# plainerman/DiffDock-Pocket

Hardware: AMD Instinct MI355X
Metric: ligand poses/sec (40 samples x 20 steps) on 3dpf (higher is better)
Workload: dtype f32 (fc and G products: fp16 hi/lo split of both operands on v_mfma_f32_16x16x32_f16 - the row-stationary conv kernel - and v_mfma_f32_32x32x16_f16, fp32 accumulate; G between its two kernels as fp16 hi + continuation byte = 19 significant bits; the exact fp32 MFMA form is timed in other_workloads)

## Files before the change

diffdock_pocket_amd/_lib.py:

```python
from __future__ import annotations

import ctypes as C
import os

HERE = os.path.dirname(os.path.abspath(__file__))
LIB_PATH = os.environ.get("DDP_HIP_LIB", os.path.join(HERE, "libddp_hip.so"))

DDP_MAX_TASKS, DDP_MAX_BLOCKS, DDP_MAX_SEGS, DDP_MAX_NS, DDP_EDGE_TILE = 9, 4, 3, 64, 64
F_SCALAR_S0, F_DOT, F_SCALAR_S1, F_VEC_S0, F_CROSS = range(5)
FS = 68

DDP_MAX_GEMM_BATCH = 16
DDP_EVAL_MAX_ATOMS = 1024
DDP_MINIMIZE_MAX_ATOMS, DDP_MINIMIZE_MAX_TORSIONS = 512, 4096
DDP_MINIMIZE_FLEX_MAX_MOVING, DDP_MINIMIZE_FLEX_MAX_BONDS, DDP_MINIMIZE_FLEX_MAX_STATE_BYTES = 256, 256, 47040
DDP_PAIRWISE_MAX_SAMPLES, DDP_CLUSTER_MAX_SAMPLES = 32768, 1024
EXPORTS = ["ddp_conv_messages", "ddp_conv_rows", "ddp_stage_a_gh", "ddp_stage_a_gh3", "ddp_segment_reduce", "ddp_edge_featurize", "ddp_edge_featurize_jobs", "ddp_torsion_sh", "ddp_stage_a", "ddp_stage_a_h2",
           "ddp_pose_update", "ddp_sidechain_update", "ddp_sde_update", "ddp_radius_count", "ddp_radius_fill", "ddp_knn", "ddp_group_by_key", "ddp_node_linear", "ddp_scan_jobs", "ddp_mark_jobs", "ddp_rowcopy_jobs", "ddp_select_jobs",
           "ddp_gather_rows", "ddp_clean_pair_maps", "ddp_flex_mark", "ddp_fallback_rowmap", "ddp_step_prologue", "ddp_trrot_head", "ddp_tor_head", "ddp_radius_search_jobs", "ddp_group_by_key_jobs", "ddp_set_occupancy_shaping", "ddp_pose_rmsd", "ddp_pose_contacts", "ddp_pose_pairwise_rmsd", "ddp_pose_cluster", "ddp_traj_record", "ddp_svgd_tau", "ddp_svgd_pairs", "ddp_svgd_rows", "ddp_refine_energy", "ddp_refine_direction", "ddp_refine_accept", "ddp_pose_score", "ddp_pose_minimize", "ddp_pose_minimize_flex", "ddp_pocket_occupancy", "ddp_pocket_buriedness", "ddp_pocket_label", "ddp_abi_version", "ddp_last_error", "ddp_source_hash"]


class Seg(C.Structure):
    _fields_ = [("kind", C.c_int32), ("in_off", C.c_int32), ("count", C.c_int32)]


class Block(C.Structure):
    _fields_ = [("U", C.c_int32), ("n", C.c_int32), ("C", C.c_int32), ("out_off", C.c_int32), ("tile0", C.c_int32),
                ("ntiles", C.c_int32), ("nsub", C.c_int32), ("ups", C.c_int32), ("nseg", C.c_int32),
                ("seg", Seg * DDP_MAX_SEGS), ("g_slot", C.c_int32), ("g_col0", C.c_int32)]


class RoleSeg(C.Structure):
    _fields_ = [("block", C.c_int32), ("tile0", C.c_int32), ("tstride", C.c_int32), ("count", C.c_int32), ("round", C.c_int32)]


DDP_CONV32_WAVES, DDP_MAX_ROLE_SEGS = 4, 2


class ConvShape(C.Structure):
    _fields_ = [("f_in", C.c_int32), ("hid", C.c_int32), ("kp1", C.c_int32), ("hp", C.c_int32), ("hs", C.c_int32),
                ("nct1", C.c_int32), ("d_out", C.c_int32), ("nblocks", C.c_int32), ("fbuf_floats", C.c_int32),
                ("g_cols", C.c_int32 * 2), ("blk", Block * DDP_MAX_BLOCKS), ("nrounds", C.c_int32),
                ("nrole", C.c_int32 * DDP_CONV32_WAVES), ("role", (RoleSeg * DDP_MAX_ROLE_SEGS) * DDP_CONV32_WAVES)]


class ConvTask(C.Structure):
    _fields_ = [("x_src", C.c_void_p), ("ldx_src", C.c_int32), ("n_edges", C.c_int32), ("src", C.c_void_p),
                ("eid", C.c_void_p), ("sh", C.c_void_p), ("seg_ptr", C.c_void_p * DDP_MAX_SEGS),
                ("seg_idx", C.c_void_p * DDP_MAX_SEGS), ("seg_ld", C.c_int32 * DDP_MAX_SEGS),
                ("seg_n", C.c_int32 * DDP_MAX_SEGS), ("w1p", C.c_void_p), ("b1p", C.c_void_p), ("w2p", C.c_void_p),
                ("b2p", C.c_void_p), ("msg", C.c_void_p), ("g", C.c_void_p * 2),
                ("pos", C.c_void_p), ("n_edges_dev", C.c_void_p), ("w1h", C.c_void_p), ("w2h", C.c_void_p), ("h2_range_flag", C.c_void_p),
                ("wsh", C.c_void_p), ("bsp", C.c_void_p), ("gh", C.c_void_p * 2), ("gh_fmt", C.c_int32), ("rows_form", C.c_int32), ("rows_bias_k", C.c_int32), ("rows_seg0", C.c_int32), ("rows_seg1", C.c_int32), ("rows_nts", C.c_int32)]


class ReduceSrc(C.Structure):
    _fields_ = [("msg", C.c_void_p), ("rowptr", C.c_void_p), ("bn_scale", C.c_void_p), ("bn_shift", C.c_void_p),
                ("n_edges", C.c_int32), ("rowmap", C.c_void_p), ("n_edges_dev", C.c_void_p)]


DDP_MAX_NODE_JOBS, DDP_MAX_NODE_CAT = 8, 16
DDP_MAX_LIST_JOBS = 12
_P, _I = C.c_void_p, C.c_int32


class ScanJob(C.Structure):
    _fields_ = [("n", _I), ("n_dev", _P), ("flag", _P), ("val", _P), ("rowptr", _P), ("base", _I), ("excl", _P), ("excl2", _P),
                ("list", _P), ("total", _P)]


class MarkJob(C.Structure):
    _fields_ = [("idx", _P), ("n", _I), ("n_dev", _P), ("mask", _P)]


class RowcopyJob(C.Structure):
    _fields_ = [("n_rows", _I), ("keep", _P), ("old_rowptr", _P), ("new_rowptr", _P), ("inp", _P * 3), ("out", _P * 3)]


class SelectJob(C.Structure):
    _fields_ = [("n", _I), ("n_dev", _P), ("mask_a", _P), ("idx_a", _P), ("mask_b", _P), ("idx_b", _P), ("out_idx", _P),
                ("pay", _P * 4), ("pay_add", _I * 4), ("out", _P * 4), ("total", _P), ("block_count", _P), ("block_off", _P)]


class RadiusJob(C.Structure):
    _fields_ = [("x", _P), ("x_ptr", _P), ("y", _P), ("y_batch", _P), ("ny", _I), ("r", C.c_float), ("max_neighbors", _I),
                ("flags", _I), ("graph_div", _P), ("counts", _P), ("offsets", _P), ("base", _I), ("total", _P), ("out_query", _P),
                ("out_x", _P), ("capacity", _I), ("overflow", _P)]


class SdeArgs(C.Structure):
    _fields_ = [("score", _P * 4), ("z", _P * 4), ("out", _P * 4), ("n", _I * 4)]


class SvgdArgs(C.Structure):
    _fields_ = [("pos", _P), ("n", _I), ("n_lig", _I), ("n_tor", _I), ("dihedrals", _P), ("score", _P * 3), ("upd", _P * 3), ("gdt", _P),
                ("weight", C.c_float), ("w_rep", C.c_float), ("w_rot", C.c_float), ("w_tor", C.c_float), ("svgd_only", _I),
                ("tau", _P), ("tr_diff", _P), ("rot_diff", _P), ("tor_diff", _P), ("dist", _P)]


class RefineArgs(C.Structure):
    _fields_ = [("n_samples", _I), ("n", _I), ("m", _I), ("rec_stride", _I), ("n_tor", _I), ("pos", _P), ("anchor", _P), ("lig_radii", _P),
                ("rec", _P), ("rec_radii", _P), ("self_pairs", _P), ("overlap", C.c_double), ("restraint", C.c_double), ("energy", _P),
                ("grad", _P), ("bonds", _P), ("mask_rotate", _P), ("step", _P), ("tr", _P), ("rot", _P), ("tor", _P), ("trial", _P),
                ("trial_energy", _P), ("trial_grad", _P), ("accepted", _P), ("grow", C.c_double), ("shrink", C.c_double),
                ("step_max", C.c_double)]


class ScoreArgs(C.Structure):
    _fields_ = [("n_samples", _I), ("n", _I), ("m", _I), ("rec_stride", _I), ("pos", _P), ("lig_radii", _P), ("lig_flags", _P), ("rec", _P),
                ("rec_radii", _P), ("rec_flags", _P), ("self_pairs", _P), ("cutoff", C.c_double), ("gauss_offset", C.c_double),
                ("gauss_width", C.c_double), ("hydrophobic_good", C.c_double), ("hydrophobic_bad", C.c_double), ("hbond_good", C.c_double),
                ("hbond_bad", C.c_double), ("w_gauss", C.c_double), ("w_repulsion", C.c_double), ("w_hydrophobic", C.c_double),
                ("w_hbond", C.c_double), ("tor_divisor", C.c_double), ("energy", _P), ("grad", _P)]


class MinimizeArgs(C.Structure):
    _fields_ = [("n_samples", _I), ("n", _I), ("m", _I), ("rec_stride", _I), ("n_tor", _I), ("iterations", _I), ("pos", _P), ("anchor", _P),
                ("lig_radii", _P), ("lig_flags", _P), ("rec", _P), ("rec_radii", _P), ("rec_flags", _P), ("self_pairs", _P), ("bonds", _P),
                ("mask_rotate", _P), ("cutoff", C.c_double), ("gauss_offset", C.c_double), ("gauss_width", C.c_double),
                ("hydrophobic_good", C.c_double), ("hydrophobic_bad", C.c_double), ("hbond_good", C.c_double), ("hbond_bad", C.c_double),
                ("w_gauss", C.c_double), ("w_repulsion", C.c_double), ("w_hydrophobic", C.c_double), ("w_hbond", C.c_double),
                ("restraint", C.c_double), ("grow", C.c_double), ("shrink", C.c_double), ("step_max", C.c_double), ("step", _P),
                ("accepted", _P), ("energy_in", _P), ("energy_out", _P), ("history", _P), ("grad", _P)]


class MinimizeFlexArgs(C.Structure):
    _fields_ = MinimizeArgs._fields_ + [("rec_anchor", _P), ("n_mov", _I), ("n_sc", _I), ("n_sub", _I), ("reserved", _I), ("mov", _P),
                                        ("sc_edge_idx", _P), ("sc_sub", _P), ("sc_map", _P), ("sc_pairs", _P),
                                        ("restraint_sc", C.c_double), ("grad_mov", _P)]


def flex_state_bytes(n: int, n_mov: int, n_sc: int) -> int:
    return 89 * n + 81 * n_mov + 4 * n_sc


class GroupJob(C.Structure):
    _fields_ = [("key", _P), ("n_items", _I), ("n_items_dev", _P), ("n_keys", _I), ("pay", _P * 3), ("rowptr", _P), ("perm", _P),
                ("out_key", _P), ("out", _P * 3), ("key_map", _P), ("scratch", _P)]



DDP_MAX_FEATURIZE_JOBS = 8


class FeaturizeJob(C.Structure):
    _fields_ = [("pos_a", _P), ("ia", _P), ("pos_b", _P), ("ib", _P), ("n_edges", _I), ("n_edges_dev", _P), ("offset", _P), ("k_rbf", _I),
                ("coeff", C.c_float), ("pre", _P), ("pre_idx", _P), ("ld_pre", _I), ("pre2", _P), ("n_pre2", _I), ("ld_pre2", _I),
                ("w1d", _P), ("w2", _P), ("b2", _P), ("ns", _I), ("out", _P), ("sh", _P)]


class _BondJob(C.Structure):
    _fields_ = [("pos", _P), ("b0", _P), ("b1", _P), ("n", _I), ("mid", _P), ("vec", _P)]


class _CopyJob(C.Structure):
    _fields_ = [("src", _P), ("dst", _P), ("n", _I)]


class PrologueArgs(C.Structure):
    _fields_ = [("t", _P * 4), ("t_stride", _I * 4), ("sig_min", C.c_float * 4), ("sig_max", C.c_float * 4), ("sigma", _P * 4),
                ("n_graphs", _I), ("cut", _P), ("cut_mul", C.c_float), ("cut_add", C.c_float), ("graph_emb", _P), ("sd", _I),
                ("emb_scale", C.c_float), ("freq", _P), ("lig_pos", _P), ("graph_ptr", _P), ("center", _P),
                ("bonds", _BondJob * 2), ("copy", _CopyJob * 2)]


class TrRotArgs(C.Structure):
    _fields_ = [("gp", _P), ("ld_gp", _I), ("n_graphs", _I), ("ns", _I), ("sd", _I), ("graph_emb", _P), ("w1", _P * 2), ("b1", _P * 2),
                ("w2", _P * 2), ("b2", _P * 2), ("sigma", _P * 2), ("so3_table", _P), ("so3_n", _I), ("so3_lo", C.c_float),
                ("so3_span", C.c_float), ("out", _P * 2)]


class TorArgs(C.Structure):
    _fields_ = [("h", _P), ("ld_h", _I), ("n_bonds", _I), ("ns", _I), ("w1", _P), ("w2", _P), ("sigma", _P), ("graph_of_bond", _P),
                ("torus_table", _P), ("torus_n", _I), ("torus_lo", C.c_float), ("torus_span", C.c_float), ("out", _P)]


class NodeJob(C.Structure):
    _fields_ = [("n_rows", C.c_int32), ("cat", C.c_void_p), ("ld_cat", C.c_int32), ("n_cat", C.c_int32), ("table", C.c_void_p),
                ("feat_off", C.c_int32 * DDP_MAX_NODE_CAT), ("emb_dim", C.c_int32), ("emb_mode", C.c_int32),
                ("dense", C.c_void_p * 2), ("ld_dense", C.c_int32 * 2), ("n_dense", C.c_int32 * 2),
                ("t", C.c_void_p), ("t_stride", C.c_int32), ("scale", C.c_float), ("freq", C.c_void_p),
                ("sig_emb", C.c_void_p), ("ld_sig", C.c_int32), ("sd", C.c_int32), ("sig_out", C.c_void_p), ("ld_sig_out", C.c_int32),
                ("w", C.c_void_p), ("bias", C.c_void_p),
                ("out", C.c_void_p), ("ld_out", C.c_int32), ("ncols", C.c_int32), ("zero_to", C.c_int32),
                ("add", C.c_void_p), ("ld_add", C.c_int32)]


def g_ld(hid: int, gcols: int) -> int:
    return (((hid + 3) // 4 * 4 + 1) * gcols + 31) // 32 * 32


class DdpError(RuntimeError):
    pass


_lib = None


def load():
    global _lib
    if _lib is not None:
        return _lib
    if not os.path.exists(LIB_PATH):
        raise DdpError(f"{LIB_PATH} not found: build it with `python -m diffdock_pocket_amd.build` "
                       f"(hipcc --offload-arch=gfx950); there is no fallback path")
    lib = C.CDLL(LIB_PATH)
    for name in EXPORTS:
        if not hasattr(lib, name):
            raise DdpError(f"{LIB_PATH} does not export {name}")
    lib.ddp_abi_version.restype = C.c_int
    lib.ddp_last_error.restype = C.c_char_p
    lib.ddp_conv_messages.argtypes = [C.POINTER(ConvShape), C.POINTER(ConvTask), C.c_int, C.c_void_p]
    lib.ddp_conv_messages.restype = C.c_int
    lib.ddp_conv_rows.argtypes = lib.ddp_conv_messages.argtypes
    lib.ddp_conv_rows.restype = C.c_int
    lib.ddp_segment_reduce.argtypes = [C.c_void_p, C.c_int, C.c_int, C.c_int, C.POINTER(ReduceSrc), C.c_int, C.c_int,
                                       C.c_int, C.c_int, C.c_void_p]
    lib.ddp_segment_reduce.restype = C.c_int
    lib.ddp_edge_featurize.argtypes = [C.c_void_p, C.c_void_p, C.c_void_p, C.c_void_p, C.c_int, C.c_void_p, C.c_void_p, C.c_int,
                                       C.c_float, C.c_void_p, C.c_void_p, C.c_int, C.c_void_p, C.c_int, C.c_int, C.c_void_p,
                                       C.c_void_p, C.c_void_p, C.c_int, C.c_void_p, C.c_void_p, C.c_void_p]
    lib.ddp_edge_featurize.restype = C.c_int
    lib.ddp_edge_featurize_jobs.argtypes = [C.POINTER(FeaturizeJob), C.c_int, C.c_void_p]
    lib.ddp_edge_featurize_jobs.restype = C.c_int
    lib.ddp_torsion_sh.argtypes = [C.c_void_p, C.c_void_p, C.c_void_p, C.c_int, C.c_void_p, C.c_void_p, C.c_void_p, C.c_int, C.c_int,
                                   C.c_void_p, C.c_void_p, C.c_int, C.c_void_p, C.c_void_p]
    lib.ddp_torsion_sh.restype = C.c_int
    lib.ddp_stage_a.argtypes = [C.c_void_p, C.c_int, C.c_int, C.c_void_p, C.c_void_p, C.c_int, C.POINTER(C.c_int32), C.c_int,
                                C.c_void_p, C.c_void_p, C.c_int, C.c_int, C.c_void_p, C.c_int, C.c_void_p]
    lib.ddp_stage_a.restype = C.c_int
    lib.ddp_stage_a_h2.argtypes = lib.ddp_stage_a.argtypes[:-1] + [C.c_void_p, C.c_void_p]
    lib.ddp_stage_a_h2.restype = C.c_int
    lib.ddp_stage_a_gh.argtypes = lib.ddp_stage_a_h2.argtypes[:-1] + [C.c_void_p, C.c_void_p]
    lib.ddp_stage_a_gh.restype = C.c_int
    lib.ddp_stage_a_gh3.argtypes = lib.ddp_stage_a_gh.argtypes
    lib.ddp_stage_a_gh3.restype = C.c_int
    lib.ddp_set_occupancy_shaping.argtypes = [C.c_int, C.c_int]
    lib.ddp_set_occupancy_shaping.restype = C.c_int
    lib.ddp_pose_update.argtypes = [C.c_void_p, C.c_int, C.c_int, C.c_void_p, C.c_void_p, C.c_void_p, C.c_int, C.c_void_p,
                                    C.c_void_p, C.c_void_p, C.c_void_p]
    lib.ddp_pose_update.restype = C.c_int
    lib.ddp_sidechain_update.argtypes = [C.c_void_p, C.c_int, C.c_int, C.c_void_p, C.c_int, C.c_void_p, C.c_void_p, C.c_void_p,
                                         C.c_void_p, C.c_void_p]
    lib.ddp_sidechain_update.restype = C.c_int
    lib.ddp_radius_count.argtypes = [C.c_void_p, C.c_void_p, C.c_void_p, C.c_void_p, C.c_int, C.c_float, C.c_int, C.c_int,
                                     C.c_void_p, C.c_void_p]
    lib.ddp_radius_count.restype = C.c_int
    lib.ddp_radius_fill.argtypes = [C.c_void_p, C.c_void_p, C.c_void_p, C.c_void_p, C.c_int, C.c_float, C.c_int, C.c_int,
                                    C.c_void_p, C.c_void_p, C.c_void_p, C.c_void_p]
    lib.ddp_radius_fill.restype = C.c_int
    lib.ddp_knn.argtypes = [C.c_void_p, C.c_void_p, C.c_void_p, C.c_int, C.c_int, C.c_void_p, C.c_void_p]
    lib.ddp_knn.restype = C.c_int
    lib.ddp_group_by_key.argtypes = [C.c_void_p, C.c_int, C.c_int] + [C.c_void_p] * 11
    lib.ddp_group_by_key.restype = C.c_int
    for name, job in (("ddp_scan_jobs", ScanJob), ("ddp_mark_jobs", MarkJob), ("ddp_rowcopy_jobs", RowcopyJob),
                      ("ddp_select_jobs", SelectJob), ("ddp_radius_search_jobs", RadiusJob), ("ddp_group_by_key_jobs", GroupJob)):
        getattr(lib, name).argtypes = [C.POINTER(job), C.c_int, C.c_void_p]
        getattr(lib, name).restype = C.c_int
    lib.ddp_sde_update.argtypes = [C.c_void_p, C.POINTER(SdeArgs), C.c_void_p]
    lib.ddp_sde_update.restype = C.c_int
    lib.ddp_gather_rows.argtypes = [C.c_void_p, C.c_int, C.c_void_p, C.c_int, C.c_void_p, C.c_void_p, C.c_int, C.c_int, C.c_void_p]
    lib.ddp_gather_rows.restype = C.c_int
    lib.ddp_clean_pair_maps.argtypes = [C.c_void_p, C.c_void_p, C.c_void_p, C.c_void_p, C.c_int, C.c_int, C.c_int, C.c_int, C.c_void_p,
                                        C.c_void_p, C.c_void_p]
    lib.ddp_clean_pair_maps.restype = C.c_int
    lib.ddp_flex_mark.argtypes = [C.c_void_p, C.c_void_p, C.c_int, C.c_void_p, C.c_void_p, C.c_int, C.c_int, C.c_int, C.c_int, C.c_int,
                                  C.c_void_p, C.c_void_p]
    lib.ddp_flex_mark.restype = C.c_int
    lib.ddp_fallback_rowmap.argtypes = [C.c_void_p, C.c_void_p, C.c_void_p, C.c_void_p, C.c_int, C.c_int, C.c_void_p, C.c_void_p]
    lib.ddp_fallback_rowmap.restype = C.c_int
    for name, st in (("ddp_step_prologue", PrologueArgs), ("ddp_trrot_head", TrRotArgs), ("ddp_tor_head", TorArgs)):
        getattr(lib, name).argtypes = [C.POINTER(st), C.c_void_p]
        getattr(lib, name).restype = C.c_int
    lib.ddp_node_linear.argtypes = [C.POINTER(NodeJob), C.c_int, C.c_void_p]
    lib.ddp_node_linear.restype = C.c_int
    lib.ddp_pose_rmsd.argtypes = [C.c_void_p, C.c_int, C.c_int, C.c_void_p, C.c_int, C.c_void_p, C.c_int, C.c_void_p, C.c_int,
                                  C.c_void_p, C.c_void_p, C.c_void_p]
    lib.ddp_pose_rmsd.restype = C.c_int
    lib.ddp_pose_contacts.argtypes = [C.c_void_p, C.c_int, C.c_int, C.c_void_p, C.c_void_p, C.c_int, C.c_int, C.c_void_p, C.c_float,
                                      C.c_void_p, C.c_void_p, C.c_void_p]
    lib.ddp_pose_contacts.restype = C.c_int
    lib.ddp_pose_pairwise_rmsd.argtypes = [C.c_void_p, C.c_int, C.c_int, C.c_void_p, C.c_int, C.c_void_p, C.c_int, C.c_void_p, C.c_void_p]
    lib.ddp_pose_pairwise_rmsd.restype = C.c_int
    lib.ddp_pose_cluster.argtypes = [C.c_void_p, C.c_int, C.c_void_p, C.c_float, C.c_void_p, C.c_void_p, C.c_void_p, C.c_void_p, C.c_void_p]
    lib.ddp_pose_cluster.restype = C.c_int
    lib.ddp_traj_record.argtypes = [C.c_void_p, C.c_int, C.c_int, C.c_void_p, C.c_void_p, C.c_int, C.c_void_p, C.c_int, C.c_void_p,
                                    C.c_int, C.c_void_p, C.c_void_p]
    lib.ddp_traj_record.restype = C.c_int
    for name in ("ddp_svgd_tau", "ddp_svgd_pairs", "ddp_svgd_rows"):
        getattr(lib, name).argtypes = [C.POINTER(SvgdArgs), C.c_void_p]
        getattr(lib, name).restype = C.c_int
    for name in ("ddp_refine_energy", "ddp_refine_direction", "ddp_refine_accept"):
        getattr(lib, name).argtypes = [C.POINTER(RefineArgs), C.c_void_p]
        getattr(lib, name).restype = C.c_int
    lib.ddp_pose_score.argtypes = [C.POINTER(ScoreArgs), C.c_void_p]
    lib.ddp_pose_score.restype = C.c_int
    lib.ddp_pose_minimize.argtypes = [C.POINTER(MinimizeArgs), C.c_void_p]
    lib.ddp_pose_minimize.restype = C.c_int
    lib.ddp_pose_minimize_flex.argtypes = [C.POINTER(MinimizeFlexArgs), C.c_void_p]
    lib.ddp_pose_minimize_flex.restype = C.c_int
    lib.ddp_pocket_occupancy.argtypes = [C.c_void_p, C.c_void_p, C.c_int, C.c_float, C.c_float, C.c_float, C.c_float, C.c_int, C.c_int, C.c_int,
                                         C.c_void_p, C.c_void_p]
    lib.ddp_pocket_occupancy.restype = C.c_int
    lib.ddp_pocket_buriedness.argtypes = [C.c_void_p, C.c_int, C.c_int, C.c_int, C.c_double, C.c_double, C.c_int, C.c_void_p, C.c_void_p,
                                          C.c_void_p]
    lib.ddp_pocket_buriedness.restype = C.c_int
    lib.ddp_pocket_label.argtypes = [C.c_void_p, C.c_int, C.c_int, C.c_int, C.c_void_p, C.c_void_p]
    lib.ddp_pocket_label.restype = C.c_int
    if lib.ddp_abi_version() != 17:
        raise DdpError("libddp_hip.so ABI version mismatch")
    lib.ddp_source_hash.restype = C.c_char_p
    if "DDP_HIP_LIB" not in os.environ:
        from .build import source_hash
        have, want = lib.ddp_source_hash().decode(), source_hash()
        if have != want:
            raise DdpError(f"{LIB_PATH} was built from other sources (library {have}, tree {want}): rebuild it with "
                           f"`python -m diffdock_pocket_amd.build`")
    _lib = lib
    return lib


def check(rc, what):
    if rc != 0:
        raise DdpError(f"{what} failed (rc={rc}): {load().ddp_last_error().decode()}")
```

diffdock_pocket_amd/csrc/ddp_gemm.hip:

```cpp
#include <hip/hip_runtime.h>
#include <stdint.h>
#include <type_traits>
#include <stdlib.h>

#include "ddp_hip.h"
#include "ddp_internal.h"

typedef float f32x2 __attribute__((ext_vector_type(2)));
typedef float f32x4 __attribute__((ext_vector_type(4)));

#define DDP_GEMM_THREADS 256
#define DDP_GEMM_ROWS 128

struct GemmOffs {
  int off[DDP_MAX_GEMM_BATCH];
};

template <int KT, int CPL>
__global__ __launch_bounds__(DDP_GEMM_THREADS, 2) void ddp_stage_a_kernel(const float* __restrict__ x, int ldx, int nrows,
                                                                           const int32_t* __restrict__ rows,
                                                                           const int32_t* __restrict__ nrows_dev, int out_rows,
                                                                           const GemmOffs offs, const float* __restrict__ w,
                                                                           int k, int ncols, float* __restrict__ out, int ldo) {
  constexpr int KP = (KT > 0) ? KT / 2 : 32;
// ... 225 lines not shown

template <int KT>
__global__ __launch_bounds__(DDP_GEMM_THREADS, 2) void ddp_stage_a_x3_kernel(const float* __restrict__ x, int ldx, int nrows,
                                                                              const int32_t* __restrict__ rows,
                                                                              const int32_t* __restrict__ nrows_dev, int out_rows,
                                                                              int mrows, const GemmOffs offs,
                                                                              const __bf16* __restrict__ w3, int ncols,
                                                                              float* __restrict__ out, int ldo) {
  if (nrows_dev) nrows = min(nrows, *nrows_dev);
  if ((int)blockIdx.y * mrows >= nrows) return;
  constexpr int KP = (KT + 15) / 16 * 16, NS = KP / 16, CT = DDP_SA3_CT;
  constexpr int XS = KP + 8;
  constexpr int NV = (32 * KT / 4 + DDP_GEMM_THREADS - 1) / DDP_GEMM_THREADS;
  constexpr int TS = 36;
  constexpr int NM = NS * 6;
  __shared__ __attribute__((aligned(16))) __bf16 xt[2][3][32 * XS];
  __shared__ __attribute__((aligned(16))) float st[4][2][32 * TS];
  const int z = (int)blockIdx.z, tid = (int)threadIdx.x;
  const int wave = tid >> 6, lane = tid & 63, r = lane & 31, hh = lane >> 5;
  const int col0 = ((int)blockIdx.x * 4 + wave) * (32 * CT);
  bf16x8 wr[CT][3][NS];
#pragma unroll
  for (int t = 0; t < CT; ++t) {
    const int c = min(col0 + 32 * t + r, ncols - 1);
#pragma unroll
    for (int p = 0; p < 3; ++p)
#pragma unroll
      for (int s2 = 0; s2 < NS; ++s2)
        wr[t][p][s2] = *reinterpret_cast<const bf16x8*>(w3 + (((((size_t)z * 3 + p) * NS + s2) * 2 + hh) * ncols + c) * 8);
  }
  if constexpr (KP > KT) {
    for (int i = tid; i < 2 * 3 * 32 * (KP - KT); i += DDP_GEMM_THREADS) {
      const int kk = i % (KP - KT), rr = (i / (KP - KT)) % 32, bp = i / ((KP - KT) * 32);
      xt[bp / 3][bp % 3][rr * XS + KT + kk] = (__bf16)0.f;
    }
  }
  const float* __restrict__ xb = x + offs.off[z];
  for (int R0 = (int)blockIdx.y * mrows; R0 < nrows; R0 += (int)gridDim.y * mrows) {
  const int R1 = min(nrows, R0 + mrows);
  const bool al4 = ((ldx | offs.off[z]) & 3) == 0 && (reinterpret_cast<size_t>(x) & 15) == 0;
  f32x4 xv[NV];
  auto fetch = [&](int row0) {
#pragma unroll
    for (int v = 0; v < NV; ++v) {
      const int i = tid + v * DDP_GEMM_THREADS;
      const int rr = min(i / (KT / 4), 31), q = i % (KT / 4);
      const int ri = min(row0 + rr, nrows - 1);
      const float* __restrict__ p = xb + (size_t)(rows ? rows[ri] : ri) * ldx + 4 * q;
      if (al4)
        xv[v] = *reinterpret_cast<const f32x4*>(p);
      else
        xv[v] = f32x4{p[0], p[1], p[2], p[3]};
    }
  };
  auto park = [&](int buf) {
#pragma unroll
    for (int v = 0; v < NV; ++v) {
      const int i = tid + v * DDP_GEMM_THREADS;
      if (i < 32 * (KT / 4)) {
        const int rr = i / (KT / 4), q = i % (KT / 4);
        bf16x4 h, m, l;
#pragma unroll
        for (int e = 0; e < 4; ++e) {
          const float f = xv[v][e];
          h[e] = (__bf16)f;
          const float r1 = f - (float)h[e];
          m[e] = (__bf16)r1;
          l[e] = (__bf16)(r1 - (float)m[e]);
        }
        *reinterpret_cast<bf16x4*>(&xt[buf][0][rr * XS + 4 * q]) = h;
        *reinterpret_cast<bf16x4*>(&xt[buf][1][rr * XS + 4 * q]) = m;
        *reinterpret_cast<bf16x4*>(&xt[buf][2][rr * XS + 4 * q]) = l;
      }
    }
  };
  float* pend_ob = nullptr;
  int pend_c0 = 0, pend_rows = 0, pend_buf = 0, pbuf = 0;
  int pend_ri[4] = {0, 0, 0, 0};
  f32x4 dv = {0.f, 0.f, 0.f, 0.f};
  auto drain_read = [&](int p) {
    if (pend_ob) dv = *reinterpret_cast<const f32x4*>(&st[wave][pend_buf][(8 * p + (lane >> 3)) * TS + 4 * (lane & 7)]);
  };
  auto drain_store = [&](int p) {
    if (pend_ob) {
      const int rr = 8 * p + (lane >> 3), c = pend_c0 + 4 * (lane & 7);
      if (rr < pend_rows && c < ncols) *reinterpret_cast<f32x4*>(&pend_ob[(size_t)pend_ri[p] * ldo + c]) = dv;
    }
  };
  fetch(R0);
  park(0);
  __syncthreads();
  int buf = 0;
  for (int row0 = R0; row0 < R1; row0 += 32, buf ^= 1) {
    const bool more = row0 + 32 < R1;
    if (more) fetch(row0 + 32);
    bf16x8 a[3][NS];
#pragma unroll
    for (int p = 0; p < 3; ++p)
#pragma unroll
      for (int s2 = 0; s2 < NS; ++s2) a[p][s2] = *reinterpret_cast<const bf16x8*>(&xt[buf][p][r * XS + 16 * s2 + 8 * hh]);
    float* __restrict__ ob = out + (size_t)z * out_rows * ldo;
    int blk_ri[4];
#pragma unroll
    for (int p = 0; p < 4; ++p) {
      const int ri = min(row0 + 8 * p + (lane >> 3), R1 - 1);
      blk_ri[p] = rows ? rows[ri] : ri;
    }
#pragma unroll
    for (int t = 0; t < CT; ++t) {
      f32x16 acc;
#pragma unroll
      for (int i = 0; i < 16; ++i) acc[i] = 0.f;
#pragma unroll
      for (int m = 0; m < NM; ++m) {
        constexpr int PA[6] = {2, 0, 1, 1, 0, 0}, PB[6] = {0, 2, 1, 0, 1, 0};
        const int pr = m / NS, s2 = m % NS;
        acc = __builtin_amdgcn_mfma_f32_32x32x16_bf16(a[PA[pr]][s2], wr[t][PB[pr]][s2], acc, 0, 0, 0);
        static_assert(NM / 4 >= 3 && NM % 4 == 0, "quarter schedule");
        if (m % (NM / 4) == 0) drain_read(m / (NM / 4));
        if (m % (NM / 4) == 2) drain_store(m / (NM / 4));
      }
      float* tl = st[wave][pbuf];
#pragma unroll
      for (int i = 0; i < 16; ++i) tl[((i & 3) + 8 * (i >> 2) + 4 * hh) * TS + r] = acc[i];
      pend_ob = ob;
#pragma unroll
      for (int p = 0; p < 4; ++p) pend_ri[p] = blk_ri[p];
      pend_c0 = col0 + 32 * t;
      pend_rows = R1 - row0;
      pend_buf = pbuf;
      pbuf ^= 1;
    }
    if (more) park(buf ^ 1);
    __syncthreads();
  }
#pragma unroll
  for (int p = 0; p < 4; ++p) {
    drain_read(p);
    drain_store(p);
  }
  __syncthreads();
  }
}

typedef _Float16 h8 __attribute__((ext_vector_type(8)));
typedef _Float16 h4 __attribute__((ext_vector_type(4)));
#ifndef DDP_SAH_CT_GH
#define DDP_SAH_CT_GH 4
#endif
#ifndef DDP_SAH_CT
#define DDP_SAH_CT 4
#endif

template <int KT, bool GH = false, bool G3 = false>
__global__ __launch_bounds__(DDP_GEMM_THREADS, 2) void ddp_stage_a_h2_kernel(const float* __restrict__ x, int ldx, int nrows,
                                                                              const int32_t* __restrict__ rows,
                                                                              const int32_t* __restrict__ nrows_dev, int out_rows,
                                                                              int mrows, const GemmOffs offs,
                                                                              const _Float16* __restrict__ wh, int ncols,
                                                                              float* __restrict__ out, int ldo, int32_t* range_flag,
                                                                              const int32_t* __restrict__ gh_dest = nullptr) {
  if (nrows_dev) nrows = min(nrows, *nrows_dev);
  if ((int)blockIdx.y * mrows >= nrows) return;
  constexpr int KP = (KT + 15) / 16 * 16, NS = KP / 16, CT = GH ? DDP_SAH_CT_GH : DDP_SAH_CT;
  constexpr int XS = KP + 8;
  constexpr int NV = (32 * KT / 4 + DDP_GEMM_THREADS - 1) / DDP_GEMM_THREADS;
  constexpr int TS = 36;
  constexpr int RS3 = 392;
  __shared__ __attribute__((aligned(16))) _Float16 xt[2][2][32 * XS];
  __shared__ __attribute__((aligned(16))) float st[G3 ? 1 : 4][2][G3 ? 4 : 32 * TS];
  __shared__ __attribute__((aligned(16))) char g3t[G3 ? 4 : 1][G3 ? 32 * RS3 : 16];
  const int z = (int)blockIdx.z, tid = (int)threadIdx.x;
  const int wave = tid >> 6, lane = tid & 63, r = lane & 31, hh = lane >> 5;
  const int col0 = ((int)blockIdx.x * 4 + wave) * (32 * CT);
  h8 wr[CT][2][NS];
#pragma unroll
  for (int t = 0; t < CT; ++t) {
    const int c = min(col0 + 32 * t + r, ncols - 1);
#pragma unroll
    for (int p = 0; p < 2; ++p)
#pragma unroll
      for (int s2 = 0; s2 < NS; ++s2)
        wr[t][p][s2] = *reinterpret_cast<const h8*>(wh + (((((size_t)z * 2 + p) * NS + s2) * 2 + hh) * ncols + c) * 8);
  }
  if constexpr (KP > KT) {
    for (int i = tid; i < 2 * 2 * 32 * (KP - KT); i += DDP_GEMM_THREADS) {
      const int kk = i % (KP - KT), rr = (i / (KP - KT)) % 32, bp = i / ((KP - KT) * 32);
      xt[bp / 2][bp % 2][rr * XS + KT + kk] = (_Float16)0.f;
    }
  }
  const float* __restrict__ xb = x + offs.off[z];
  float* __restrict__ ob = out + (size_t)z * out_rows * ldo;
  int cq[CT];
#pragma unroll
  for (int t = 0; t < CT; ++t) cq[t] = max(0, min(4 * (lane & 7), ncols - 4 - (col0 + 32 * t)));
  int gh_o[CT][2];
  bool gh_sp[CT];
  float gh_max = 0.f;
#pragma unroll
  for (int t = 0; t < CT; ++t) {
    gh_o[t][0] = gh_o[t][1] = 0;
    gh_sp[t] = false;
    if constexpr (GH) {
      const int g = min(col0 + 32 * t + 8 * (lane & 3), ncols - 8) >> 3;
      const int32_t* __restrict__ d = gh_dest + ((size_t)z * (ncols >> 3) + g) * 2;
      gh_o[t][0] = d[0] & ~3;
      gh_o[t][1] = d[1];
      gh_sp[t] = (d[0] & 1) != 0;
    }
  }
  unsigned sp3 = 0u;
  int g3_rr[3] = {0, 0, 0}, g3_pc[3] = {0, 0, 0};
  if constexpr (G3) {
    const int g = min(col0 + 8 * (lane & 15), ncols - 8) >> 3;
    sp3 = (unsigned)__ballot((gh_dest[((size_t)z * (ncols >> 3) + g) * 2] & 1) != 0) & 0xffffu;
#pragma unroll
    for (int j = 0; j < 3; ++j) {
      g3_rr[j] = (64 * j + lane) / 24;
      g3_pc[j] = (64 * j + lane) % 24;
    }
  }
  for (int R0 = (int)blockIdx.y * mrows; R0 < nrows; R0 += (int)gridDim.y * mrows) {
  const int R1 = min(nrows, R0 + mrows);
  const bool al4 = ((ldx | offs.off[z]) & 3) == 0 && (reinterpret_cast<size_t>(x) & 15) == 0;
  f32x4 xv[NV];
  auto fetch = [&](int row0) {
#pragma unroll
    for (int v = 0; v < NV; ++v) {
      const int i = tid + v * DDP_GEMM_THREADS;
      const int rr = min(i / (KT / 4), 31), q = i % (KT / 4);
      const int ri = min(row0 + rr, nrows - 1);
      const float* __restrict__ p = xb + (size_t)(rows ? rows[ri] : ri) * ldx + 4 * q;
      if (al4)
        xv[v] = *reinterpret_cast<const f32x4*>(p);
      else
        xv[v] = f32x4{p[0], p[1], p[2], p[3]};
    }
  };
  auto park = [&](int buf) {
#pragma unroll
    for (int v = 0; v < NV; ++v) {
      const int i = tid + v * DDP_GEMM_THREADS;
      if (i < 32 * (KT / 4)) {
        const int rr = i / (KT / 4), q = i % (KT / 4);
        h4 h, l;
#pragma unroll
        for (int e = 0; e < 4; ++e) {
          const float f = GH ? xv[v][e] * (float)DDP_GH_SX : xv[v][e];
          if (!(fabsf(f) <= 65504.f) && range_flag) *range_flag = 1;
          h[e] = (_Float16)f;
          l[e] = (_Float16)(GH ? f - (float)h[e] : (f - (float)h[e]) * 2048.f);
        }
        *reinterpret_cast<h4*>(&xt[buf][0][rr * XS + 4 * q]) = h;
        *reinterpret_cast<h4*>(&xt[buf][1][rr * XS + 4 * q]) = l;
      }
    }
  };
  size_t pend_off[4] = {0, 0, 0, 0};
  int pend_lds[4] = {0, 0, 0, 0};
  bool pend_sp = false;
  int pbuf = 0;
  f32x4 dv = {0.f, 0.f, 0.f, 0.f};
  f32x4 dv2 = {0.f, 0.f, 0.f, 0.f};
  auto gh_read = [&](const float* pt, int p) {
    if (p & 1) {
      dv = dv2;
      return;
    }
    typedef float f32x8 __attribute__((ext_vector_type(8)));
    const f32x4 a = *reinterpret_cast<const f32x4*>(&pt[pend_lds[p]]), b = *reinterpret_cast<const f32x4*>(&pt[pend_lds[p] + 4]);
    const f32x8 f = {a[0], a[1], a[2], a[3], b[0], b[1], b[2], b[3]};
    const h8 hi = __builtin_convertvector(f, h8);
    const f32x8 rest = f - __builtin_convertvector(hi, f32x8);
    const h8 lo = __builtin_convertvector(rest, h8);
    const float m8 = fmaxf(fmaxf(fmaxf(fabsf(f[0]), fabsf(f[1])), fmaxf(fabsf(f[2]), fabsf(f[3]))), fmaxf(fmaxf(fabsf(f[4]), fabsf(f[5])), fmaxf(fabsf(f[6]), fabsf(f[7]))));
    gh_max = fmaxf(gh_max, pend_sp ? m8 : 0.f);
    const f32x4 vh = __builtin_bit_cast(f32x4, hi), vl = __builtin_bit_cast(f32x4, lo);
#pragma unroll
    for (int e = 0; e < 4; ++e) {
      dv[e] = pend_sp ? vh[e] : a[e];
      dv2[e] = pend_sp ? vl[e] : b[e];
    }
  };
  auto block = [&](auto drain_tag, int t, const h8 (&a)[2][NS], const int (&blk_ri)[4], int nr) {
    constexpr bool DRAIN = decltype(drain_tag)::value;
    f32x16 am, ac;
#pragma unroll
    for (int i = 0; i < 16; ++i) { am[i] = 0.f; ac[i] = 0.f; }
    const float* pt = st[wave][pbuf ^ 1];
#pragma unroll
    for (int s2 = 0; s2 < NS; ++s2) {
      if constexpr (DRAIN && NS == 4) {
        if constexpr (GH)
          gh_read(pt, s2);
        else
          dv = *reinterpret_cast<const f32x4*>(&pt[pend_lds[s2]]);
      }
      if constexpr (GH) {
        am = __builtin_amdgcn_mfma_f32_32x32x16_f16(wr[t][0][s2], a[0][s2], am, 0, 0, 0);
        am = __builtin_amdgcn_mfma_f32_32x32x16_f16(wr[t][1][s2], a[0][s2], am, 0, 0, 0);
        am = __builtin_amdgcn_mfma_f32_32x32x16_f16(wr[t][0][s2], a[1][s2], am, 0, 0, 0);
      } else {
        am = __builtin_amdgcn_mfma_f32_32x32x16_f16(a[0][s2], wr[t][0][s2], am, 0, 0, 0);
        ac = __builtin_amdgcn_mfma_f32_32x32x16_f16(a[0][s2], wr[t][1][s2], ac, 0, 0, 0);
        ac = __builtin_amdgcn_mfma_f32_32x32x16_f16(a[1][s2], wr[t][0][s2], ac, 0, 0, 0);
      }
      if constexpr (DRAIN && NS == 4) {
        {
          *reinterpret_cast<f32x4*>(&ob[pend_off[s2]]) = dv;
        }
      }
    }
    if constexpr (DRAIN && NS != 4) {
#pragma unroll
      for (int p = 0; p < 4; ++p) {
        if constexpr (GH)
          gh_read(pt, p);
        else
          dv = *reinterpret_cast<const f32x4*>(&pt[pend_lds[p]]);
        *reinterpret_cast<f32x4*>(&ob[pend_off[p]]) = dv;
      }
    }
    float* tl = st[wave][pbuf];
    if constexpr (GH) {
#pragma unroll
      for (int q4 = 0; q4 < 4; ++q4)
        *reinterpret_cast<f32x4*>(&tl[r * TS + 8 * q4 + 4 * hh]) = f32x4{am[4 * q4], am[4 * q4 + 1], am[4 * q4 + 2], am[4 * q4 + 3]};
    } else {
#pragma unroll
      for (int i = 0; i < 16; ++i) tl[((i & 3) + 8 * (i >> 2) + 4 * hh) * TS + r] = am[i] + ac[i] * (1.f / 2048.f);
    }
    if constexpr (GH) {
#if defined(DDP_GH_ABL) && DDP_GH_ABL == 1
      pend_sp = false;
#else
      pend_sp = gh_sp[t];
#endif
#pragma unroll
      for (int p = 0; p < 4; ++p) {
        const int rr = min(16 * (p >> 1) + (lane >> 2), nr - 1);
        pend_lds[p] = rr * TS + 8 * (lane & 3);
        pend_off[p] = (size_t)blk_ri[p >> 1] * ldo + gh_o[t][p & 1];
      }
    } else {
#pragma unroll
      for (int p = 0; p < 4; ++p) {
        const int rr = min(8 * p + (lane >> 3), nr - 1);
        pend_lds[p] = rr * TS + cq[t];
        pend_off[p] = (size_t)blk_ri[p] * ldo + (col0 + 32 * t + cq[t]);
      }
    }
    pbuf ^= 1;
  };
  auto block3 = [&](int t, const h8 (&a)[2][NS]) {
    f32x16 am;
#pragma unroll
    for (int i = 0; i < 16; ++i) am[i] = 0.f;
#pragma unroll
    for (int s2 = 0; s2 < NS; ++s2) {
      am = __builtin_amdgcn_mfma_f32_32x32x16_f16(wr[t][0][s2], a[0][s2], am, 0, 0, 0);
      am = __builtin_amdgcn_mfma_f32_32x32x16_f16(wr[t][1][s2], a[0][s2], am, 0, 0, 0);
      am = __builtin_amdgcn_mfma_f32_32x32x16_f16(wr[t][0][s2], a[1][s2], am, 0, 0, 0);
    }
    char* tl = g3t[G3 ? wave : 0] + r * RS3 + 96 * t;
#pragma unroll
    for (int q = 0; q < 4; ++q) {
      const bool sp = ((sp3 >> (4 * t + q)) & 1u) != 0u;
      const float v0 = am[4 * q], v1 = am[4 * q + 1], v2 = am[4 * q + 2], v3 = am[4 * q + 3];
      gh_max = fmaxf(gh_max, sp ? fmaxf(fmaxf(fabsf(v0), fabsf(v1)), fmaxf(fabsf(v2), fabsf(v3))) : 0.f);
      const uint32_t b0 = __builtin_bit_cast(uint32_t, v0) + 0x10u, b1 = __builtin_bit_cast(uint32_t, v1) + 0x10u;
      const uint32_t b2 = __builtin_bit_cast(uint32_t, v2) + 0x10u, b3 = __builtin_bit_cast(uint32_t, v3) + 0x10u;
      typedef __fp16 pk2 __attribute__((ext_vector_type(2)));
      const pk2 h01 = __builtin_amdgcn_cvt_pkrtz(__builtin_bit_cast(float, b0), __builtin_bit_cast(float, b1));
      const pk2 h23 = __builtin_amdgcn_cvt_pkrtz(__builtin_bit_cast(float, b2), __builtin_bit_cast(float, b3));
      const uint32_t lo = ((b0 >> 5) & 0xffu) | (((b1 >> 5) & 0xffu) << 8) | (((b2 >> 5) & 0xffu) << 16) | ((b3 >> 5) << 24);
      typedef uint32_t u32x2 __attribute__((ext_vector_type(2)));
      u32x2 w8;
      w8[0] = sp ? __builtin_bit_cast(uint32_t, h01) : __builtin_bit_cast(uint32_t, v0);
      w8[1] = sp ? __builtin_bit_cast(uint32_t, h23) : __builtin_bit_cast(uint32_t, v1);
      *reinterpret_cast<u32x2*>(tl + 24 * q + 8 * hh) = w8;
      *reinterpret_cast<uint32_t*>(tl + 24 * q + 16 + 4 * hh) = sp ? lo : __builtin_bit_cast(uint32_t, v2);
    }
  };
  auto drain3 = [&](int myrow, int nr) {
    __builtin_amdgcn_fence(__ATOMIC_RELEASE, "wavefront");
    __builtin_amdgcn_wave_barrier();
    const char* img = g3t[G3 ? wave : 0];
    float* __restrict__ oc = ob + 6 * (col0 >> 3);
#pragma unroll
    for (int p = 0; p < 4; ++p)
#pragma unroll
      for (int j = 0; j < 3; ++j) {
        const int rl = min(8 * p + g3_rr[j], nr - 1);
        typedef uint32_t u32x2 __attribute__((ext_vector_type(2)));
        const u32x2 lo8 = *reinterpret_cast<const u32x2*>(img + rl * RS3 + 16 * g3_pc[j]);
        const u32x2 hi8 = *reinterpret_cast<const u32x2*>(img + rl * RS3 + 16 * g3_pc[j] + 8);
        const int ri = __shfl(myrow, rl);
        typedef uint32_t u32x4 __attribute__((ext_vector_type(4)));
        *reinterpret_cast<u32x4*>(oc + (size_t)ri * ldo + 4 * g3_pc[j]) = u32x4{lo8[0], lo8[1], hi8[0], hi8[1]};
      }
    __builtin_amdgcn_wave_barrier();
  };
  fetch(R0);
  park(0);
  __syncthreads();
  int buf = 0;
  bool first = true;
  for (int row0 = R0; row0 < R1; row0 += 32, buf ^= 1) {
    const bool more = row0 + 32 < R1;
    if (more) fetch(row0 + 32);
    h8 a[2][NS];
#pragma unroll
    for (int p = 0; p < 2; ++p)
#pragma unroll
      for (int s2 = 0; s2 < NS; ++s2) a[p][s2] = *reinterpret_cast<const h8*>(&xt[buf][p][r * XS + 16 * s2 + 8 * hh]);
    int blk_ri[4];
#pragma unroll
    for (int p = 0; p < 4; ++p) {
      const int ri = min(row0 + (GH ? 16 * (p & 1) + (lane >> 2) : 8 * p + (lane >> 3)), R1 - 1);
      blk_ri[p] = rows ? rows[ri] : ri;
    }
    const int nr = R1 - row0;
    if constexpr (G3) {
      if (col0 < ncols) {
        const int ri = min(row0 + r, R1 - 1);
        const int myrow = rows ? rows[ri] : ri;
#pragma unroll
        for (int t = 0; t < CT; ++t) block3(t, a);
        drain3(myrow, nr);
      }
      if (more) park(buf ^ 1);
      __syncthreads();
      continue;
    }
#pragma unroll
    for (int t = 0; t < CT; ++t) {
      if (col0 + 32 * t >= ncols) continue;
      if (t == 0 && first)
        block(std::false_type{}, t, a, blk_ri, nr);
      else
        block(std::true_type{}, t, a, blk_ri, nr);
      first = false;
    }
    if (more) park(buf ^ 1);
    __syncthreads();
  }
  if (!first) {
    const float* pt = st[wave][pbuf ^ 1];
#pragma unroll
    for (int p = 0; p < 4; ++p) {
      if constexpr (GH)
        gh_read(pt, p);
      else
        dv = *reinterpret_cast<const f32x4*>(&pt[pend_lds[p]]);
      *reinterpret_cast<f32x4*>(&ob[pend_off[p]]) = dv;
    }
  }
  __syncthreads();
  }
  if constexpr (GH) {
    if (!(gh_max <= 65504.f) && range_flag) *range_flag = 1;
  }
}

static int stage_a_impl(const float* x, int ldx, int nrows, const int32_t* rows, const int32_t* nrows_dev, int out_rows,
                        const int32_t* offs, int nbatch, const float* w, const void* w_bf16x3, const void* w_h2, int k, int ncols, float* out,
                        int ldo, int32_t* range_flag, void* stream, const int32_t* gh_dest = nullptr, int gh_fmt = 0) {
  if (!rows) out_rows = nrows;
  if (out_rows < 1 && nrows > 0) return ddp_fail(DDP_EINVAL, "ddp_stage_a: out_rows");
  if (nbatch < 0 || nbatch > DDP_MAX_GEMM_BATCH) return ddp_fail(DDP_ELIMIT, "ddp_stage_a: nbatch > DDP_MAX_GEMM_BATCH");
  if (k < 2 || k > 64 || (k & 1)) return ddp_fail(DDP_ELIMIT, "ddp_stage_a: K must be even and in [2, 64]");
  if (ncols < 1 || nrows < 0 || (ldo < ncols && !(gh_dest && gh_fmt == 1 && ldo >= (ncols / 8) * 6)))
    return ddp_fail(DDP_EINVAL, "ddp_stage_a: ncols / nrows / ldo");
  if (gh_dest && gh_fmt == 1 && ((ncols & 127) != 0 || (ldo & 31) != 0))
    return ddp_fail(DDP_EINVAL, "ddp_stage_a_gh3: ncols % 128 == 0 (a wave's four column blocks), ldo % 32 == 0 (whole 128-byte lines)");
  if (nbatch == 0 || nrows == 0) return 0;
  if (!x || !offs || !w || !out) return ddp_fail(DDP_EINVAL, "ddp_stage_a: null argument");
  if ((reinterpret_cast<size_t>(x) & 3) || (reinterpret_cast<size_t>(out) & 7))
    return ddp_fail(DDP_EINVAL, "ddp_stage_a: x must be 4-byte aligned, out 8-byte aligned");
  GemmOffs O;
  for (int i = 0; i < DDP_MAX_GEMM_BATCH; ++i) O.off[i] = (i < nbatch) ? offs[i] : 0;
  hipStream_t s = (hipStream_t)stream;
  const int nry = (nrows + DDP_GEMM_ROWS - 1) / DDP_GEMM_ROWS;
#define DDP_GEMM_LAUNCH(KT, CPL)                                                                                 \
  hipLaunchKernelGGL((ddp_stage_a_kernel<KT, CPL>), dim3((ncols + CPL * DDP_GEMM_THREADS - 1) / (CPL * DDP_GEMM_THREADS), nry, nbatch), \
                     dim3(DDP_GEMM_THREADS), 0, s, x, ldx, nrows, rows, nrows_dev, out_rows, O, w, k, ncols, out, ldo)
  const bool wide = ((ncols | ldo) & 3) == 0 && ncols >= 4 * DDP_GEMM_THREADS && (reinterpret_cast<size_t>(out) & 15) == 0;
#define DDP_GEMM_MFMA(KT)                                                                                        \
  hipLaunchKernelGGL((ddp_stage_a_mfma_kernel<KT>), dim3((ncols + 128 * DDP_SA_CT - 1) / (128 * DDP_SA_CT), gy, nbatch), \
                     dim3(DDP_GEMM_THREADS), 0, s, x, ldx, nrows, rows, nrows_dev, out_rows, mrows, O, w, ncols, out, ldo)
  const bool listed = rows && nrows_dev;
  int mrows = listed ? (nrows >= 16384 ? 256 : 128) : (nrows >= 8192 ? DDP_GEMM_MROWS : nrows >= 384 ? 256 : 64);
  int gy = (nrows + mrows - 1) / mrows;
  if (listed && gy > 96) gy = 96;
#ifdef DDP_SA_TUNE
  if (nrows < 8192 || listed) {
    if (const char* e = getenv("DDP_SA_MROWS")) mrows = atoi(e);
    gy = (nrows + mrows - 1) / mrows;
    const char* c = getenv("DDP_SA_GYCAP");
    const int cap = c ? atoi(c) : 96;
    if (listed && gy > cap) gy = cap;
  }
#endif
  static const bool no_mfma = getenv("DDP_STAGE_A_VALU") != nullptr;
  if (gh_dest) {
    if (!(w_h2 && wide && (k == 60 || k == 32 || k == 24 || k == 16) && (reinterpret_cast<size_t>(w_h2) & 15) == 0 && (ncols & 31) == 0 &&
          (reinterpret_cast<size_t>(gh_dest) & 7) == 0))
      return ddp_fail(DDP_EINVAL, "ddp_stage_a_gh: plane output needs the h2 path (w_h2, k in {60, 32, 24, 16}) and ncols % 32 == 0");
    const dim3 grid((ncols + 128 * DDP_SAH_CT_GH - 1) / (128 * DDP_SAH_CT_GH), gy, nbatch);
    const int pad = ddp_shape_stage_a_pad;
    static int pad_have[8] = {0, 0, 0, 0, 0, 0, 0, 0};
#define DDP_GEMM_GH(KT, I)                                                                                       \
    {                                                                                                            \
      if (pad > 0) {                                                                                             \
        const hipError_t ep = (gh_fmt == 1) ? ddp_need_lds(reinterpret_cast<const void*>(ddp_stage_a_h2_kernel<KT, true, true>), pad, &pad_have[4 + I]) \
                                            : ddp_need_lds(reinterpret_cast<const void*>(ddp_stage_a_h2_kernel<KT, true>), pad, &pad_have[I]); \
        if (ep != hipSuccess) return ddp_fail_hip(ep, "hipFuncSetAttribute(stage A)");                           \
      }                                                                                                          \
      if (gh_fmt == 1)                                                                                           \
        hipLaunchKernelGGL((ddp_stage_a_h2_kernel<KT, true, true>), grid, dim3(DDP_GEMM_THREADS), pad, s, x, ldx, nrows, rows, nrows_dev, out_rows, mrows, O, \
                           reinterpret_cast<const _Float16*>(w_h2), ncols, out, ldo, range_flag, gh_dest);       \
      else                                                                                                       \
        hipLaunchKernelGGL((ddp_stage_a_h2_kernel<KT, true>), grid, dim3(DDP_GEMM_THREADS), pad, s, x, ldx, nrows, rows, nrows_dev, out_rows, mrows, O, \
                           reinterpret_cast<const _Float16*>(w_h2), ncols, out, ldo, range_flag, gh_dest);       \
    }
    switch (k) {
      case 60: DDP_GEMM_GH(60, 0); break;
      case 32: DDP_GEMM_GH(32, 1); break;
      case 24: DDP_GEMM_GH(24, 2); break;
      default: DDP_GEMM_GH(16, 3); break;
    }
#undef DDP_GEMM_GH
    const hipError_t eg = hipGetLastError();
    if (eg != hipSuccess) return ddp_fail_hip(eg, "ddp_stage_a_gh launch");
    return 0;
  }
  if (w_h2 && wide && (k == 60 || k == 32 || k == 24 || k == 16) && !no_mfma && (reinterpret_cast<size_t>(w_h2) & 15) == 0) {
    const dim3 grid((ncols + 128 * DDP_SAH_CT - 1) / (128 * DDP_SAH_CT), gy, nbatch);
#define DDP_GEMM_H2(KT)                                                                                          \
    hipLaunchKernelGGL((ddp_stage_a_h2_kernel<KT>), grid, dim3(DDP_GEMM_THREADS), 0, s, x, ldx, nrows, rows, nrows_dev, out_rows, mrows, O, \
                       reinterpret_cast<const _Float16*>(w_h2), ncols, out, ldo, range_flag)
    switch (k) {
      case 60: DDP_GEMM_H2(60); break;
      case 32: DDP_GEMM_H2(32); break;
      case 24: DDP_GEMM_H2(24); break;
      default: DDP_GEMM_H2(16); break;
    }
#undef DDP_GEMM_H2
    const hipError_t eh = hipGetLastError();
    if (eh != hipSuccess) return ddp_fail_hip(eh, "ddp_stage_a (h2) launch");
    return 0;
  }
  if (w_bf16x3 && wide && (k == 60 || k == 32) && !no_mfma && (reinterpret_cast<size_t>(w_bf16x3) & 15) == 0) {
    const dim3 grid((ncols + 128 * DDP_SA3_CT - 1) / (128 * DDP_SA3_CT), gy, nbatch);
    if (k == 60)
      hipLaunchKernelGGL((ddp_stage_a_x3_kernel<60>), grid, dim3(DDP_GEMM_THREADS), 0, s, x, ldx, nrows, rows, nrows_dev, out_rows, mrows, O,
                         reinterpret_cast<const __bf16*>(w_bf16x3), ncols, out, ldo);
    else
      hipLaunchKernelGGL((ddp_stage_a_x3_kernel<32>), grid, dim3(DDP_GEMM_THREADS), 0, s, x, ldx, nrows, rows, nrows_dev, out_rows, mrows, O,
                         reinterpret_cast<const __bf16*>(w_bf16x3), ncols, out, ldo);
    const hipError_t e3 = hipGetLastError();
    if (e3 != hipSuccess) return ddp_fail_hip(e3, "ddp_stage_a (bf16x3) launch");
    return 0;
  }
  if (ncols >= 512 && !no_mfma && (k == 60 || k == 64 || k == 32 || k == 24 || k == 16)) {
    switch (k) {
      case 60: DDP_GEMM_MFMA(60); break;
      case 64: DDP_GEMM_MFMA(64); break;
      case 32: DDP_GEMM_MFMA(32); break;
      case 24: DDP_GEMM_MFMA(24); break;
      default: DDP_GEMM_MFMA(16); break;
    }
  } else
  switch (k) {
    case 60: if (wide) DDP_GEMM_LAUNCH(60, 4); else DDP_GEMM_LAUNCH(60, 2); break;
    case 32: DDP_GEMM_LAUNCH(32, 2); break;
    case 24: DDP_GEMM_LAUNCH(24, 2); break;
    case 16: DDP_GEMM_LAUNCH(16, 2); break;
    default: DDP_GEMM_LAUNCH(0, 2); break;
  }
#undef DDP_GEMM_LAUNCH
#undef DDP_GEMM_MFMA
  const hipError_t err = hipGetLastError();
  if (err != hipSuccess) return ddp_fail_hip(err, "ddp_stage_a launch");
  return 0;
}

extern "C" int ddp_stage_a(const float* x, int ldx, int nrows, const int32_t* rows, const int32_t* nrows_dev, int out_rows,
                           const int32_t* offs, int nbatch, const float* w, const void* w_bf16x3, int k, int ncols, float* out, int ldo,
                           void* stream) {
  return stage_a_impl(x, ldx, nrows, rows, nrows_dev, out_rows, offs, nbatch, w, w_bf16x3, nullptr, k, ncols, out, ldo, nullptr, stream);
}

extern "C" int ddp_stage_a_h2(const float* x, int ldx, int nrows, const int32_t* rows, const int32_t* nrows_dev, int out_rows,
                              const int32_t* offs, int nbatch, const float* w, const void* w_h2, int k, int ncols, float* out, int ldo,
                              int32_t* range_flag, void* stream) {
  return stage_a_impl(x, ldx, nrows, rows, nrows_dev, out_rows, offs, nbatch, w, nullptr, w_h2, k, ncols, out, ldo, range_flag, stream);
}

extern "C" int ddp_stage_a_gh(const float* x, int ldx, int nrows, const int32_t* rows, const int32_t* nrows_dev, int out_rows,
                              const int32_t* offs, int nbatch, const float* w, const void* w_h2, int k, int ncols, float* out, int ldo,
                              int32_t* range_flag, const int32_t* dest, void* stream) {
  if (!dest) return ddp_fail(DDP_EINVAL, "ddp_stage_a_gh: dest");
  return stage_a_impl(x, ldx, nrows, rows, nrows_dev, out_rows, offs, nbatch, w, nullptr, w_h2, k, ncols, out, ldo, range_flag, stream, dest);
}

extern "C" int ddp_stage_a_gh3(const float* x, int ldx, int nrows, const int32_t* rows, const int32_t* nrows_dev, int out_rows,
                               const int32_t* offs, int nbatch, const float* w, const void* w_h2, int k, int ncols, float* out, int ldo,
                               int32_t* range_flag, const int32_t* dest, void* stream) {
  if (!dest) return ddp_fail(DDP_EINVAL, "ddp_stage_a_gh3: dest");
  return stage_a_impl(x, ldx, nrows, rows, nrows_dev, out_rows, offs, nbatch, w, nullptr, w_h2, k, ncols, out, ldo, range_flag, stream, dest, 1);
}
```

diffdock_pocket_amd/csrc/ddp_misc.hip:

```cpp
#include <hip/hip_runtime.h>
#include <stdlib.h>
#include <stdint.h>

#include "ddp_hip.h"
#include "ddp_internal.h"

typedef float f32x4 __attribute__((ext_vector_type(4)));

struct ReduceLaunch {
  ddp_reduce_src_t src[3];
  int nsrc;
};

__global__ void ddp_segment_reduce_kernel(float* __restrict__ x, int ldx, int n_nodes, int d_out, ReduceLaunch L,
                                          int accumulate, int n_rep, int rep_stride) {
  const int node = blockIdx.x;
  const int ch = threadIdx.x;
  if (ch >= d_out) return;
  float* dst = x + (size_t)node * ldx + ch;
  float total = (accumulate && n_rep <= 1) ? *dst : 0.f;
  int p0[3], p1[3];
#pragma unroll
  for (int k = 0; k < 3; ++k) {
    const bool on = k < L.nsrc;
    p0[k] = on ? L.src[k].rowptr[node] : 0;
    p1[k] = on ? L.src[k].rowptr[node + 1] : 0;
  }
#pragma unroll
  for (int k = 0; k < 3; ++k) {
    if (k < L.nsrc && !(L.src[k].n_edges_dev && *L.src[k].n_edges_dev <= 0)) {
      const ddp_reduce_src_t& s = L.src[k];
      const float* __restrict__ m = s.msg + ch;
      const int32_t* __restrict__ rm = s.rowmap;
      float sum = 0.f;
      for (int p = p0[k]; p < p1[k]; p += 8) {
        float v[8];
        int row[8];
#pragma unroll
        for (int i = 0; i < 8; ++i) {
          const int q = min(p + i, p1[k] - 1);
          row[i] = rm ? rm[q] : q;
        }
#pragma unroll
        for (int i = 0; i < 8; ++i) v[i] = m[(size_t)row[i] * d_out];
#pragma unroll
        for (int i = 0; i < 8; ++i)
          if (p + i < p1[k]) sum += v[i];
      }
      const int cnt = p1[k] - p0[k];
      const float mean = sum / (float)(cnt > 1 ? cnt : 1);
      total += mean * s.bn_scale[ch] + s.bn_shift[ch];
    }
  }
  if (n_rep <= 1) {
    *dst = total;
  } else {
    for (int g = 0; g < n_rep; ++g) {
      float* d = dst + (size_t)g * rep_stride * ldx;
      *d = *d + total;
    }
  }
}

typedef float red4 __attribute__((ext_vector_type(4)));
__global__ __launch_bounds__(256) void ddp_segment_reduce4_kernel(float* __restrict__ x, int ldx, int n_nodes, int d_out, ReduceLaunch L,
                                                                  int accumulate, int n_rep, int rep_stride) {
  const int nq = d_out >> 2;
  const long long item = (long long)blockIdx.x * 256 + threadIdx.x;
  const int node = (int)(item / nq), ch = 4 * (int)(item - (long long)node * nq);
  if (node >= n_nodes) return;
  float* dst = x + (size_t)node * ldx + ch;
  red4 total = (accumulate && n_rep <= 1) ? *reinterpret_cast<const red4*>(dst) : red4{0.f, 0.f, 0.f, 0.f};
  int p0[3], p1[3];
#pragma unroll
  for (int k = 0; k < 3; ++k) {
    const bool on = k < L.nsrc;
    p0[k] = on ? L.src[k].rowptr[node] : 0;
    p1[k] = on ? L.src[k].rowptr[node + 1] : 0;
  }
#pragma unroll
  for (int k = 0; k < 3; ++k) {
    if (k < L.nsrc && !(L.src[k].n_edges_dev && *L.src[k].n_edges_dev <= 0)) {
      const ddp_reduce_src_t& s = L.src[k];
      const float* __restrict__ m = s.msg + ch;
      const int32_t* __restrict__ rm = s.rowmap;
      red4 sum = {0.f, 0.f, 0.f, 0.f};
      for (int p = p0[k]; p < p1[k]; p += 8) {
        red4 v[8];
        int row[8];
#pragma unroll
        for (int i = 0; i < 8; ++i) {
          const int q = min(p + i, p1[k] - 1);
          row[i] = rm ? rm[q] : q;
        }
#pragma unroll
        for (int i = 0; i < 8; ++i) v[i] = *reinterpret_cast<const red4*>(m + (size_t)row[i] * d_out);
#pragma unroll
        for (int i = 0; i < 8; ++i)
          if (p + i < p1[k]) sum += v[i];
      }
      const int cnt = p1[k] - p0[k];
      const float den = (float)(cnt > 1 ? cnt : 1);
      const red4 sc = *reinterpret_cast<const red4*>(s.bn_scale + ch), sh = *reinterpret_cast<const red4*>(s.bn_shift + ch);
#pragma unroll
      for (int c = 0; c < 4; ++c) total[c] += (sum[c] / den) * sc[c] + sh[c];
    }
  }
  if (n_rep <= 1) {
    *reinterpret_cast<red4*>(dst) = total;
  } else {
    for (int g = 0; g < n_rep; ++g) {
      red4* d = reinterpret_cast<red4*>(dst + (size_t)g * rep_stride * ldx);
      *d = *d + total;
    }
  }
}

extern "C" int ddp_segment_reduce(float* x, int ldx, int n_nodes, int d_out, const ddp_reduce_src_t* srcs, int nsrc,
                                  int accumulate, int n_rep, int rep_stride, void* stream) {
  if (!x || (!srcs && nsrc > 0)) return ddp_fail(DDP_EINVAL, "ddp_segment_reduce: null argument");
  if (nsrc < 0 || nsrc > 3) return ddp_fail(DDP_ELIMIT, "ddp_segment_reduce: nsrc > 3");
  if (d_out < 1 || d_out > 1024) return ddp_fail(DDP_ELIMIT, "ddp_segment_reduce: d_out");
  if (n_nodes <= 0) return 0;
  ReduceLaunch L;
  L.nsrc = 0;
  for (int i = 0; i < nsrc; ++i)
    if (srcs[i].n_edges > 0) L.src[L.nsrc++] = srcs[i];
  if (L.nsrc == 0 && (accumulate || n_rep > 1)) return 0;
  if (n_rep > 1 && rep_stride < n_nodes) return ddp_fail(DDP_EINVAL, "ddp_segment_reduce: rep_stride < n_nodes");
  bool wide = ((d_out | ldx) & 3) == 0 && (reinterpret_cast<size_t>(x) & 15) == 0;
  for (int i = 0; i < L.nsrc; ++i)
    wide = wide && ((reinterpret_cast<size_t>(L.src[i].msg) | reinterpret_cast<size_t>(L.src[i].bn_scale) | reinterpret_cast<size_t>(L.src[i].bn_shift)) & 15) == 0;
  static const bool narrow_only = getenv("DDP_REDUCE_NARROW") != nullptr;
  if (wide && !narrow_only) {
    const long long items = (long long)n_nodes * (d_out >> 2);
    hipLaunchKernelGGL(ddp_segment_reduce4_kernel, dim3((unsigned)((items + 255) / 256)), dim3(256), 0, (hipStream_t)stream, x, ldx, n_nodes,
                       d_out, L, accumulate, n_rep, rep_stride);
  } else {
    const int threads = ((d_out + 63) / 64) * 64;
    hipLaunchKernelGGL(ddp_segment_reduce_kernel, dim3(n_nodes), dim3(threads), 0, (hipStream_t)stream, x, ldx, n_nodes,
                       d_out, L, accumulate, n_rep, rep_stride);
  }
  hipError_t err = hipGetLastError();
  if (err != hipSuccess) return ddp_fail_hip(err, "ddp_segment_reduce launch");
  return 0;
}

#define EF_NS 64
__global__ __launch_bounds__(256) void ddp_edge_featurize_kernel(
    const float* __restrict__ pos_a, const int* __restrict__ ia, const float* __restrict__ pos_b,
    const int* __restrict__ ib, int n_edges, const int* __restrict__ n_edges_dev, const float* __restrict__ offset, int k_rbf,
    float coeff, const float* __restrict__ pre, const int* __restrict__ pre_idx, int ld_pre, const float* __restrict__ pre2,
    int n_pre2, int ld_pre2, const float* __restrict__ w1d, const float* __restrict__ w2, const float* __restrict__ b2, int ns,
    float* __restrict__ out, float* __restrict__ sh) {
  if (n_edges_dev) n_edges = min(n_edges, *n_edges_dev);
  extern __shared__ __attribute__((aligned(16))) float smem[];
  float* s_w1 = smem;
  float* s_w2 = s_w1 + k_rbf * EF_NS;
  float* s_b2 = s_w2 + EF_NS * EF_NS;
  float* s_off = s_b2 + EF_NS;
  float* s_out = s_off + ((k_rbf + 3) & ~3);
  const int tid = threadIdx.x;
  for (int i = tid; i < k_rbf * EF_NS; i += 256) s_w1[i] = w1d[i];
  for (int i = tid; i < EF_NS * EF_NS; i += 256) s_w2[i] = w2[i];
  if (tid < EF_NS) s_b2[tid] = b2[tid];
  for (int i = tid; i < k_rbf; i += 256) s_off[i] = offset[i];
  __syncthreads();

  const int wave = tid >> 6, lane = tid & 63;
  float* my_out = s_out + wave * 64 * 65;
  for (int base = blockIdx.x * 256; base < n_edges; base += gridDim.x * 256) {
    const int e = base + tid;
    const bool live = e < n_edges;
    const int ec = live ? e : n_edges - 1;
    const int a = ia[ec], b = ib[ec];
    const float vx = pos_b[3 * b] - pos_a[3 * a], vy = pos_b[3 * b + 1] - pos_a[3 * a + 1],
                vz = pos_b[3 * b + 2] - pos_a[3 * a + 2];
    const float d = sqrtf(vx * vx + vy * vy + vz * vz);
    const float inv = 1.7320508075688772f / fmaxf(d, 1e-12f);
    if (live) reinterpret_cast<f32x4*>(sh)[e] = f32x4{1.0f, vx * inv, vy * inv, vz * inv};

    float hid[EF_NS];
    const float* prow = pre + (size_t)pre_idx[ec] * ld_pre;
#pragma unroll
    for (int j = 0; j < EF_NS; ++j) hid[j] = (j < ns) ? prow[j] : 0.f;
    if (ec < n_pre2) {
      const float* p2 = pre2 + (size_t)ec * ld_pre2;
#pragma unroll
      for (int j = 0; j < EF_NS; ++j)
        if (j < ns) hid[j] = hid[j] + p2[j];
    }
    for (int k = 0; k < k_rbf; ++k) {
      const float t = d - s_off[k];
      const float rb = expf(coeff * (t * t));
      const f32x4* wrow = reinterpret_cast<const f32x4*>(s_w1 + k * EF_NS);
#pragma unroll
      for (int j4 = 0; j4 < EF_NS / 4; ++j4) {
        const f32x4 w = wrow[j4];
        hid[4 * j4 + 0] += rb * w[0];
        hid[4 * j4 + 1] += rb * w[1];
        hid[4 * j4 + 2] += rb * w[2];
        hid[4 * j4 + 3] += rb * w[3];
      }
    }
#pragma unroll
    for (int oc = 0; oc < EF_NS / 16; ++oc) {
      float o[16];
#pragma unroll
      for (int q = 0; q < 16; ++q) o[q] = s_b2[16 * oc + q];
#pragma unroll
      for (int j = 0; j < EF_NS; ++j) {
        const float hj = fmaxf(hid[j], 0.f);
        const f32x4* wrow = reinterpret_cast<const f32x4*>(s_w2 + j * EF_NS + 16 * oc);
#pragma unroll
        for (int q4 = 0; q4 < 4; ++q4) {
          const f32x4 w = wrow[q4];
          o[4 * q4 + 0] += hj * w[0];
          o[4 * q4 + 1] += hj * w[1];
          o[4 * q4 + 2] += hj * w[2];
          o[4 * q4 + 3] += hj * w[3];
        }
      }
#pragma unroll
      for (int q = 0; q < 16; ++q) my_out[lane * 65 + 16 * oc + q] = o[q];
    }
    __builtin_amdgcn_wave_barrier();
    const int ebase = base + wave * 64;
    for (int i = lane; i < 64 * ns; i += 64) {
      const int row = i / ns, col = i - row * ns;
      if (ebase + row < n_edges) out[(size_t)(ebase + row) * ns + col] = my_out[row * 65 + col];
    }
    __builtin_amdgcn_wave_barrier();
  }
}

typedef float ef_f32x16 __attribute__((ext_vector_type(16)));
#define EF_HS 68
struct FeatLaunch {
  int njobs;
  int blk_start[DDP_MAX_FEATURIZE_JOBS + 1];
  ddp_featurize_job_t job[DDP_MAX_FEATURIZE_JOBS];
};

__global__ __launch_bounds__(256) void ddp_edge_featurize_mfma_kernel(const FeatLaunch L) {
  int j = 0;
  while (j + 1 < L.njobs && (int)blockIdx.x >= L.blk_start[j + 1]) ++j;
  const ddp_featurize_job_t& J = L.job[j];
  const int blk = (int)blockIdx.x - L.blk_start[j], nblk = L.blk_start[j + 1] - L.blk_start[j];
  const float* __restrict__ pos_a = J.pos_a;
  const int* __restrict__ ia = J.ia;
  const float* __restrict__ pos_b = J.pos_b;
  const int* __restrict__ ib = J.ib;
  const float* __restrict__ offset = J.offset;
  const float* __restrict__ pre = J.pre;
  const int* __restrict__ pre_idx = J.pre_idx;
  const float* __restrict__ pre2 = J.pre2;
  const float* __restrict__ w1d = J.w1d;
  const float* __restrict__ w2 = J.w2;
  const float* __restrict__ b2 = J.b2;
  float* __restrict__ out = J.out;
  float* __restrict__ sh = J.sh;
  const int k_rbf = J.k_rbf, ld_pre = J.ld_pre, n_pre2 = J.n_pre2, ld_pre2 = J.ld_pre2, ns = J.ns;
  const float coeff = J.coeff;
  int n_edges = J.n_edges;
  if (J.n_edges_dev) n_edges = min(n_edges, *J.n_edges_dev);
  if (blk * 128 >= n_edges) return;
  extern __shared__ __attribute__((aligned(16))) float smem[];
  float* s_w1 = smem;
  float* s_w2 = s_w1 + k_rbf * EF_NS;
  float* s_b2 = s_w2 + EF_NS * EF_NS;
  float* s_off = s_b2 + EF_NS;
  float* s_h = s_off + 64;
  const int tid = threadIdx.x;
  for (int i = tid; i < k_rbf * EF_NS; i += 256) {
    const int k = i / EF_NS, c = i - k * EF_NS;
    s_w1[(((k >> 3) * 2 + ((k >> 2) & 1)) * EF_NS + c) * 4 + (k & 3)] = w1d[i];
  }
  for (int i = tid; i < EF_NS * EF_NS; i += 256) {
    const int k = i / EF_NS, c = i - k * EF_NS;
    s_w2[(((k >> 3) * 2 + ((k >> 2) & 1)) * EF_NS + c) * 4 + (k & 3)] = w2[i];
  }
  if (tid < EF_NS) s_b2[tid] = b2[tid];
  for (int i = tid; i < k_rbf; i += 256) s_off[i] = offset[i];
  __syncthreads();

  const int wave = tid >> 6, lane = tid & 63, r = lane & 31, hh = lane >> 5;
  float* my_h = s_h + wave * 32 * EF_HS;
  const f32x4* w1q = reinterpret_cast<const f32x4*>(s_w1);
  const f32x4* w2q = reinterpret_cast<const f32x4*>(s_w2);
  const int nm1 = k_rbf >> 3;
  for (int base = (blk * 4 + wave) * 32; base < n_edges; base += nblk * 128) {
    const int e = base + r;
    const int ec = min(e, n_edges - 1);
// ... 185 lines not shown
```

diffdock_pocket_amd/engine.py:

```python
from __future__ import annotations

import ctypes as C
from collections.abc import Mapping
from types import SimpleNamespace
from typing import Dict, List, Optional

import math

import torch

from . import _lib as L
from . import graph as G
from . import launch as K
from . import packing as P
from . import packing as P_
from .graph import EdgeView

SRC_TYPE = {0: "l", 1: "r", 2: "a", 3: "a", 4: "l", 5: "r", 6: "r", 7: "l", 8: "a"}
RECV_TYPE = {0: "l", 1: "l", 2: "l", 3: "a", 4: "a", 5: "a", 6: "r", 7: "r", 8: "r"}
RECV_OF = {"a": (3, 4, 5), "r": (6, 7, 8)}
ORDER = {"l": [0, 2, 1], "a": [3, 4, 5], "r": [6, 8, 7]}
_DROP_SELF = 1


# ... 480 lines not shown
                    K.rowcopy_jobs(copies)
                    F.pruned[l] = pl
                    rows_mask = {"a": i32z(Na), "r": i32z(Nr)}
                    marks = []
                    for k in range(9):
                        rt, st_ = RECV_TYPE[k], SRC_TYPE[k]
                        if st_ == "l" or k == 2 or k not in F.fact or (rt != "l" and not act[rt]):
                            continue
                        vw = pl.get(k, c[k])
                        if vw.n_edges > 0:
                            marks.append(K.mark_job(rows_mask[st_], vw.src, vw.n_edges, vw.cnt))
                    nxt = None
                    if l != layers[-1]:
                        nxt = {"a": need["a"].clone(), "r": need["r"].clone()}
                        for k in range(9):
                            rt, st_ = RECV_TYPE[k], SRC_TYPE[k]
                            if st_ == "l" or (rt != "l" and not act[rt]):
                                continue
                            vw = pl.get(k, c[k])
                            if vw.n_edges > 0:
                                marks.append(K.mark_job(nxt[st_], vw.src, vw.n_edges, vw.cnt))
                    K.mark_jobs(marks)
                    lists = {}
                    scans = []
                    for t in ("a", "r"):
                        rows = i32e(n_of[t])
                        scans.append(K.scan_job(n_of[t], flag=rows_mask[t], lst=rows, total=cnt[f"rows{l}_{t}"]))
                        lists[t] = (rows, cnt[f"rows{l}_{t}"])
                    K.scan_jobs(scans)
                    F.rows_a[l] = lists
                    if nxt is not None:
                        need = nxt
                gj = []
                for l, pl in F.pruned.items():
                    for k, v in pl.items():
                        if k in F.fact:
                            n_keys = n_of[SRC_TYPE[k]]
                            w = SimpleNamespace(rp=i32e(n_keys + 1), perm=i32e(v.n_edges), key=i32e(v.n_edges), o0=i32e(v.n_edges), o1=i32e(v.n_edges))
                            gj.append(K.group_job(v.src, v.n_edges, n_keys, [v.recv, v.eid], w.rp, w.perm, w.key, [w.o0, w.o1],
                                                  i32e(n_keys + v.n_edges), n_dev=v.cnt))
                            F.pruned_so.setdefault(l, {})[k] = EdgeView(v.n_edges, w.o0, w.key, w.o1, pos=w.perm, cnt=v.cnt)
                K.group_jobs(gj)
                F.keep.append(gj)

        def flex0():
            F.flex0 = None
            fx = getattr(F, "flex_static", None)
            kk = m.atom_max_neighbors if m.atom_max_neighbors else 32
            if (fx is not None and m.share_flex_layer0 and S.num_flex > 0 and not dbg and 0 not in F.pruned and L_ >= 2
                    and 3 in F.fact and 5 in F.fact and E_aa == Na * kk and E_aa % B == 0 and E_aa >= m.plan_min_edges
                    and E_aa * m.ns >= m.flex_share_min_work):
                na, e_ar, nr = fx
                e0 = E_aa // B
                qdirty, dirty, need_r = i32z(Na), i32z(Na), i32z(Nr)
                K.flex_mark(c[3].src, c[3].recv, E_aa, e0, na, na, qdirty, pos=F.apos, a_too=True, ref_list=True)
                K.flex_mark(c[3].recv, c[3].src, E_aa, e0, na, na, dirty, flag=qdirty, a_too=True, ref_list=True)
                K.flex_mark(c[8].recv, c[8].src, c[8].n_edges, e_ar, nr, na, need_r, pos=F.apos)
                scans, copies, pl, rowmaps = [], [], {}, {}
                for k, need, n in ((3, dirty, Na), (5, dirty, Na), (8, need_r, Nr)):
                    full = c[k]
                    v = EdgeView(full.n_edges, i32e(full.n_edges), i32e(full.n_edges), i32e(full.n_edges), rowptr=i32e(n + 1), cnt=cnt[f"fx_{k}"])
                    scans.append(K.scan_job(n, flag=need, rowptr=full.rowptr, excl=v.rowptr, total=cnt[f"fx_{k}"]))
                    copies.append(K.rowcopy_job(n, need, full.rowptr, v.rowptr, [full.recv, full.src, full.eid], [v.recv, v.src, v.eid]))
                    pl[k] = v
                K.scan_jobs(scans)
                K.rowcopy_jobs(copies)
                for k, need, n_per in ((3, dirty, na), (5, dirty, na), (8, need_r, nr)):
                    rowmaps[k] = i32e(c[k].n_edges)
                    K.fallback_rowmap(need, c[k].recv, c[k].rowptr, pl[k].rowptr, c[k].n_edges, n_per, rowmaps[k])
                rows_mask = {"a": i32z(Na), "r": i32z(Nr)}
                marks = [K.mark_job(rows_mask["a"], pl[3].src, pl[3].n_edges, pl[3].cnt),
                         K.mark_job(rows_mask["r"], pl[5].src, pl[5].n_edges, pl[5].cnt)]
                if 1 in F.fact and c[1].n_edges > 0:
                    marks.append(K.mark_job(rows_mask["r"], c[1].src, c[1].n_edges, c[1].cnt))
                K.mark_jobs(marks)
                lists, scans = {}, []
                for t in ("a", "r"):
                    rows = i32e(n_of[t])
                    scans.append(K.scan_job(n_of[t], flag=rows_mask[t], lst=rows, total=cnt[f"rows0_{t}"]))
                    lists[t] = (rows, cnt[f"rows0_{t}"])
                K.scan_jobs(scans)
                gj, pso = [], {}
                for k in (3, 5):
                    v = pl[k]
                    n_keys = n_of[SRC_TYPE[k]]
                    w = SimpleNamespace(rp=i32e(n_keys + 1), perm=i32e(v.n_edges), key=i32e(v.n_edges), o0=i32e(v.n_edges), o1=i32e(v.n_edges))
                    gj.append(K.group_job(v.src, v.n_edges, n_keys, [v.recv, v.eid], w.rp, w.perm, w.key, [w.o0, w.o1],
                                          i32e(n_keys + v.n_edges), n_dev=v.cnt))
                    pso[k] = EdgeView(v.n_edges, w.o0, w.key, w.o1, pos=w.perm, cnt=v.cnt)
                K.group_jobs(gj)
                F.keep.append(gj)
                F.pruned[0], F.pruned_so[0], F.rows_a[0] = pl, pso, lists
                F.flex0 = SimpleNamespace(dirty=dirty, need_r=need_r, rowmaps=rowmaps, na=na, e0=e0)

        def clean1():
            if (m.share_clean_layer1 and (3 in F.shared0 or F.flex0 is not None) and 3 in so and L_ >= 4 and E_aa > 0
                    and E_aa >= m.plan_min_edges and not dbg and 1 not in F.pruned):
                if F.flex0 is not None:
                    n0, e0 = F.flex0.na, F.flex0.e0
                    F.touched_l1 = F.touched + F.flex0.dirty
                else:
                    n0, e0, _ = F.shared0[3]
                    F.touched_l1 = F.touched
                so3 = so[3]
                d = SimpleNamespace(recv=i32e(E_aa), src=i32e(E_aa), eid=i32e(E_aa), pos=i32e(E_aa))
                K.select_jobs([K.select_job(E_aa, F.touched_l1, so3.recv, F.touched_l1, so3.src, [so3.recv, so3.src, so3.eid, so3.pos],
                                            [d.recv, d.src, d.eid, d.pos], cnt["dirty"], i32e(2 * ((E_aa + 2047) // 2048) + 1))])
                so_d = EdgeView(E_aa, d.recv, d.src, d.eid, pos=d.pos, cnt=cnt["dirty"])
                mask, rows_d = i32z(Na), i32e(Na)
                K.mark_jobs([K.mark_job(mask, d.src, E_aa, cnt["dirty"])])
                K.scan_jobs([K.scan_job(Na, flag=mask, lst=rows_d, total=cnt["rows_dirty"])])
                rowmap, rows_v = i32e(E_aa), i32e(n0)
                K.clean_pair_maps(F.touched_l1, c[3].recv, c[3].src, E_aa, e0, B, n0, rowmap, rows_v, rowptr=c[3].rowptr if F.flex0 is not None else None)
                so_v = m._cached(f"so_v{e0}", (so3.pos,), lambda: G.SourceOrder(e0, so3.recv[:e0], so3.src[:e0], so3.eid[:e0], (so3.pos[:e0] + E_aa).contiguous()))
                F.clean1 = SimpleNamespace(so_d=so_d, rows_d=rows_d, rows_d_cnt=cnt["rows_dirty"], rowmap=rowmap, so_v=so_v, rows_v=rows_v,
                                           E=E_aa, e0=e0, n0=n0)

        if side is not None and S.num_flex > 0 and m.fork_lists_flex:
            side(prune)
            flex0()
            clean1()
        elif side is not None and S.num_flex == 0:
            side(lambda: (prune(), flex0(), clean1()))
        else:
            prune()
            flex0()
            clean1()

    def _exact(self, F):
        vals = F.cnt.values()
        by_ptr = {F.cnt.block[i:i + 1].data_ptr(): vals[k] for k, i in F.cnt.index.items()}

        def cut(v):
            if v is None or v.cnt is None:
                return v
            n = by_ptr[v.cnt.data_ptr()]
            return EdgeView(n, v.recv[:n], v.src[:n], v.eid[:n], v.rowptr, v.pos[:n] if v.pos is not None else None, None)

        F.c = {k: cut(v) for k, v in F.c.items()}
        F.so = {k: cut(v) for k, v in F.so.items()}
        F.pruned = {l: {k: cut(v) for k, v in pl.items()} for l, pl in F.pruned.items()}
        F.pruned_so = {l: {k: cut(v) for k, v in pl.items()} for l, pl in F.pruned_so.items()}
        for h in (F.tor, F.sc):
            if h is not None:
                h.csr = cut(h.csr)
        if F.clean1 is not None:
            F.clean1.so_d = cut(F.clean1.so_d)
        F.exact = by_ptr

    def _conv_path(self, conv, dev) -> K.ConvPath:
        return K.conv_path(conv.packed_g(dev), self.m.rows_all_or_none(dev))

    def _stage_a(self, l, convs, x, n_rows, rows=None, rows_cnt=None, dense_rows=None):
        m = self.m
        paths = {self._conv_path(conv, x.device) for _, conv in convs}
        if len(paths) != 1:
            raise L.DdpError("the convs of one stage-A launch run through different conv paths")
        path = paths.pop()
        key = (l, tuple(k for k, _ in convs), path.rows)
        st = m._stage_a_stacks.get(key)
        if st is None or st.W.device != x.device:
            st = m._stage_a_stacks[key] = K.stage_a_stack([(k, conv.packed_g(x.device)) for k, conv in convs], convs[0][1].spec_g.hid, path)
        h2 = m.stage_a_h2 and K.CONV_H2 and not m.stage_a_bf16x3
        st.prepare(m.stage_a_h2, m.stage_a_bf16x3)
        Gall = torch.empty((len(st.meta), n_rows, st.ld), device=x.device, dtype=torch.float32)
        prof = K.profiler(hbm=True)
        if prof is not None:
            e0, e1 = torch.cuda.Event(enable_timing=True), torch.cuda.Event(enable_timing=True)
            e0.record()
        n_list = n_rows if rows is None else int(rows.shape[0])
        K.stage_a(x, n_list, st, Gall, rows=rows, rows_cnt=rows_cnt, out_rows=n_rows, h2=h2, x3=m.stage_a_bf16x3)
        if prof is not None:
            e1.record()
            row_bytes = 4.0 * len(st.meta) * (st.ld + st.W.shape[1])

            def nbytes(n_list=n_list, rows_cnt=rows_cnt, row_bytes=row_bytes, wn=st.W.numel()):
                n = n_list if rows_cnt is None else min(n_list, int(rows_cnt.item()))
                return row_bytes * n + 4.0 * wn
            prof.hbm.setdefault("ddp_stage_a_h2_kernel" if (st.path.rows or h2) else "ddp_stage_a_mfma_kernel", []).append((e0, e1, nbytes))
        return {(k, slot): Gall[i] for i, (k, slot, _) in enumerate(st.meta)}

    def _layers(self, S, F, dev, mark):
        m = self.m
        ns, L_, B, ldx = m.ns, m.num_conv_layers, S.B, m._ldx
        Nl, Nr, Na = S.Nl, S.Nr, S.Na
        c, so = F.c, F.so
        xl, xr, xa = F.xl, F.xr, F.xa
        e, sh = F.e, F.sh
        arr = {0: (xl, xl, "ll"), 1: (xl, xr, "lr"), 2: (xl, xa, "la"), 3: (xa, xa, "aa"), 4: (xa, xl, "la"), 5: (xa, xr, "ar"),
               6: (xr, xr, "rr"), 7: (xr, xl, "lr"), 8: (xr, xa, "ar")}
        nodes = {"l": (xl, Nl), "a": (xa, Na), "r": (xr, Nr)}
        dbg = m.debug_conv_outputs
        exact = getattr(F, "exact", None)
        prof_on = K.profiler() is not None
        plain = m.before_layers is not None
        fork = self._fork(dev) if (m.concurrent_small_batches and Na <= m.concurrent_max_atoms and not plain) else None
        pipelined = (fork is None and m.overlap_direct_conv and not plain and dbg is None and m.section_timer is None and L_ >= 2
                     and F.fact == {0, 1, 2, 3, 4, 5, 6, 7})
        side = self._fork(dev) if pipelined else None
        lists_fork = getattr(F, "lists_fork", None)

        def join_lists():
            nonlocal lists_fork
            if lists_fork is not None:
                lists_fork.join(only=4)
                lists_fork = None
        if not pipelined and fork is None:
            join_lists()

        def plan(l):
            P = SimpleNamespace(l=l, spec=m._layer_specs[l], spec_g=m._layer_specs_g[l], gmap={}, keep=[], msgs={})
            do_atom = m.flexible_sidechains or l != L_ - 1
            P.active = active = {"l": True, "a": do_atom, "r": do_atom and l != L_ - 1}
            P.shared = shared = F.shared0 if l == 0 else {}
            pl, pl_so = F.pruned.get(l, {}), F.pruned_so.get(l, {})
            P.c1 = c1 = F.clean1 if (l == 1 and F.clean1 is not None and active["a"]) else None
            P.per, P.groups = per, groups = {}, {}
            for k in range(9):
                rt, st_ = RECV_TYPE[k], SRC_TYPE[k]
                if not active[rt]:
                    continue
                csr, so_k = c[k], so.get(k) if k in F.fact else None
                x_src = arr[k][1]
                rows = ("all", None, None, nodes[st_][1])
                if k in pl:
                    csr, so_k = pl[k], pl_so.get(k)
                    if st_ != "l":
                        r_, rc = F.rows_a[l][st_]
                        rows = (f"pr{l}", r_, rc, nodes[st_][1])
                elif k in shared:
                    n0, e0, ns0 = shared[k]
                    csr = csr.prefix(e0, n0)
                    so_k = so_k.prefix(e0) if so_k is not None else None
                    x_src = x_src[:ns0]
                    rows = ("g0", None, None, ns0)
                elif k == 2 and so_k is not None:
                    rows = ("near", F.near_rows, F.cnt["near"], Na)
                    if exact is not None:
                        rows = ("near", F.near_rows[:exact[F.cnt["near"].data_ptr()]], None, Na)
                elif l in F.pruned and st_ != "l" and so_k is not None:
                    r_, rc = F.rows_a[l][st_]
                    rows = (f"pr{l}", r_, rc, nodes[st_][1])
                if exact is not None and rows[2] is not None:
                    rows = (rows[0], rows[1][:exact[rows[2].data_ptr()]], None, rows[3])
                per[k] = (csr, so_k, x_src)
                if so_k is not None and csr.n_edges > 0 and not (k == 3 and c1 is not None):
                    groups.setdefault((st_, rows[0]), (x_src, rows, []))[2].append((k, m.conv_layers[9 * l + k]))
            return P

        def node_bytes(l, k):
            d_in = P_.irreps_dim(P_.irreps_muls(ns, m.nv, l))
            return 4.0 * (nodes[SRC_TYPE[k]][1] * d_in + nodes[RECV_TYPE[k]][1] * m._layer_specs[l].d_out)

        def stage_a(P, which, forked=None):
            l = P.l
            for gi, ((st_, gid), (x_src, rows, convs)) in enumerate(P.groups.items()):
                if st_ not in which:
                    continue
                if forked is not None and gi > 0:
                    P.gmap.update(forked.run((gi - 1) % 3, lambda: self._stage_a(l, convs, x_src, rows[3], rows=rows[1], rows_cnt=rows[2])))
                else:
                    P.gmap.update(self._stage_a(l, convs, x_src, rows[3], rows=rows[1], rows_cnt=rows[2]))
            if forked is not None:
                for i_ in range(3):
                    forked.join(only=i_)
            c1 = P.c1
            if c1 is not None and "a" in which:
                conv3 = m.conv_layers[9 * l + 3]
                rows_d, rows_dc = c1.rows_d, c1.rows_d_cnt
                if exact is not None:
                    rows_d, rows_dc = rows_d[:exact[rows_dc.data_ptr()]], None
                P.g_d = self._stage_a(l, [(3, conv3)], xa, Na, rows=rows_d, rows_cnt=rows_dc)
                P.x_clean = torch.empty((c1.n0, ldx), device=dev)
                K.gather_rows(xa, c1.rows_v, c1.n0, P.x_clean, ldx)
                P.g_v = self._stage_a(l, [(3, conv3)], P.x_clean, c1.n0)
                P.keep += [P.g_d, P.g_v, P.x_clean]

        def direct_tasks(P):
            l, spec = P.l, P.spec
            direct = [(k, csr, x_src) for k, (csr, so_k, x_src) in P.per.items() if not (so_k is not None or (k == 3 and P.c1 is not None))]
            live = [(k, csr, x_src) for k, csr, x_src in direct if csr.n_edges > 0]
            split_cap = max(1, L.DDP_MAX_TASKS // max(1, len(live)))
            packs = direct_packs([(m.conv_layers[9 * l + k], max(1, min(m.direct_rows_max_split, split_cap, -(-256 // max(1, -(-csr.n_edges // 128))))))
                                  for k, csr, _ in live], dev)
            tasks, nb_d = [], 0.0
            for k, csr, x_src in direct:
                P.msgs[k] = (torch.empty((csr.n_edges, spec.d_out), device=dev), csr, m.conv_layers[9 * l + k].packed(dev))
            for (k, csr, x_src), pks in zip(live, packs):
                x_recv, _, ek = arr[k]
                if prof_on:
                    nb_d += node_bytes(l, k)
                segs = [(e[ek], csr.eid, ns, ns), (x_recv, csr.recv, ldx, ns), (x_src, csr.src, ldx, ns)]
                for i_, pk in enumerate(pks):
                    t_ = K.make_task(pk, K.conv_path(pk), x_src, ldx, csr, sh[ek], segs, P.msgs[k][0])
                    if i_:
                        t_._count = (0, None)
                    tasks.append(t_)
            P.tasks, P.nb_d = tasks, nb_d
            return tasks

        def launch_direct(P):
            K.launch_convs(P.spec, P.tasks, node_bytes=P.nb_d, tag=f"layer{P.l}")

        def launch_factorised(P, which="lar"):
            l, spec, c1 = P.l, P.spec, P.c1
            tasks_g, nb_g = [], 0.0
            for k, (csr, so_k, x_src) in P.per.items():
                if k in P.msgs or SRC_TYPE[k] not in which:
                    continue
                x_recv, _, ek = arr[k]
                conv = m.conv_layers[9 * l + k]
                pkc = conv.packed(dev)
                e_base, sh_k = e[ek], sh[ek]
                if k == 3 and c1 is not None:
                    msg = torch.empty((c1.E + c1.e0, spec.d_out), device=dev)
                    P.msgs[k] = (msg, csr, pkc, c1.rowmap)
                    pkg, path = conv.packed_g(dev), self._conv_path(conv, dev)
                    sd_ = c1.so_d
                    if sd_.n_edges > 0:
                        segs = [(e_base, sd_.eid, ns, ns), (x_recv, sd_.recv, ldx, ns), (xa, sd_.src, ldx, ns)]
                        tasks_g.append(K.make_task(pkg, path, xa, ldx, sd_, sh_k, segs, msg, g=[P.g_d.get((3, s_)) for s_ in (0, 1)]))
                    sv = c1.so_v
                    segs = [(e_base, sv.eid, ns, ns), (P.x_clean, sv.recv, ldx, ns), (P.x_clean, sv.src, ldx, ns)]
                    tasks_g.append(K.make_task(pkg, path, P.x_clean, ldx, sv, sh_k, segs, msg, g=[P.g_v.get((3, s_)) for s_ in (0, 1)]))
                    continue
                msg = torch.empty((csr.n_edges, spec.d_out), device=dev)
                P.msgs[k] = (msg, csr, pkc)
                if csr.n_edges == 0:
                    continue
                if prof_on:
                    nb_g += node_bytes(l, k)
                segs = [(e_base, so_k.eid, ns, ns), (x_recv, so_k.recv, ldx, ns), (x_src, so_k.src, ldx, ns)]
                tasks_g.append(K.make_task(conv.packed_g(dev), self._conv_path(conv, dev), x_src, ldx, so_k, sh_k, segs, msg,
                                           g=[P.gmap.get((k, s_)) for s_ in (0, 1)]))
            P.tasks_g = getattr(P, "tasks_g", []) + tasks_g
            if tasks_g:
                K.launch_convs(P.spec_g, tasks_g, flops_spec=spec, node_bytes=nb_g, tag=f"layer{l}")

        def fix_rowmaps(P):
            if P.l == 0 and F.flex0 is not None:
                for k, rm in F.flex0.rowmaps.items():
                    if k in P.msgs:
                        P.msgs[k] = (P.msgs[k][0], c[k], P.msgs[k][2], rm)

        def means(P, types):
            spec, shared = P.spec, P.shared
            for rt in types:
                if not P.active[rt]:
                    continue
                x, n = nodes[rt]
                own = [P.msgs[k] for k in ORDER[rt] if k not in shared]
                if own:
                    K.launch_reduce(x, ldx, n, spec.d_out, own, accumulate=True)
                com = [P.msgs[k] for k in ORDER[rt] if k in shared]
                if com:
                    n0 = shared[[k for k in ORDER[rt] if k in shared][0]][0]
                    K.launch_reduce(x, ldx, n0, spec.d_out, com, accumulate=True, n_rep=B, rep_stride=n0)

        if pipelined:
            P = plan(0)
            direct_tasks(P)
            if P.tasks:
                side.run(1, lambda P=P: launch_direct(P))
            stage_a(P, "lar")
            def atom_g_bytes(Pn):
                tot = 0
                for (st_, _gid), (_x, rows_, convs_) in (Pn.groups.items() if m.rows_all_or_none(dev) else ()):
                    if st_ != "a":
                        continue
                    for _k, conv_ in convs_:
                        tot += rows_[3] * 4 * sum(ld_ for ld_ in (conv_.packed_g(dev).gh_ld or []) if ld_ is not None)
                return tot
            for l in range(L_):
                nxt = plan(l + 1) if l + 1 < L_ else None
                launch_factorised(P)
                join_lists()
                fix_rowmaps(P)
                side.join(only=1)
                side.join(only=0)
                ev_r, ev_l, ev_sr, ev_sl = (torch.cuda.Event() for _ in range(4))

                def rec_chain(P=P, nxt=nxt, ev_r=ev_r, ev_sr=ev_sr):
                    means(P, "r")
                    ev_r.record()
                    if nxt is not None:
                        stage_a(nxt, "r")
                        ev_sr.record()

                def lig_chain(P=P, nxt=nxt, ev_l=ev_l, ev_sl=ev_sl):
                    means(P, "l")
                    ev_l.record()
                    if nxt is not None:
                        stage_a(nxt, "l")
                        ev_sl.record()
                side.run(3, rec_chain)
                side.run(2, lig_chain)
                means(P, "a")
                if nxt is not None:
                    direct_tasks(nxt)
                    if nxt.tasks:
                        def direct_next(nxt=nxt, ev_r=ev_r):
                            torch.cuda.current_stream(dev).wait_event(ev_r)
                            launch_direct(nxt)
                        side.run(1, direct_next)
                    if bool(getattr(m, "split_rows_launch", False)) and atom_g_bytes(nxt) >= m.split_rows_min_g_bytes:
                        def early(nxt=nxt, evs=(ev_r, ev_l, ev_sr, ev_sl)):
                            st_ = torch.cuda.current_stream(dev)
                            for ev in evs:
                                st_.wait_event(ev)
                            if getattr(m, "shape_early_rows", False):
                                K.occupancy_shaping(82 * 1024, 0)
                                try:
                                    launch_factorised(nxt, "rl")
                                finally:
                                    K.occupancy_shaping(0, 0)
                                return
                            launch_factorised(nxt, "rl")
                        side.run(0, early)
                    stage_a(nxt, "a")
                side.join(only=2)
                side.join(only=3)
                F.keep.append((P.keep, P.per, P.msgs, P.tasks, P.tasks_g, P.gmap, ev_r))
                P = nxt
            side.join()
            mark("reduce")
# ... 149 lines not shown
```

diffdock_pocket_amd/launch.py:

```python
from __future__ import annotations

import ctypes as C
import os
from dataclasses import dataclass
from typing import Dict, List, NamedTuple, Optional, Sequence

import torch
from torch import nn

from . import _lib as L
from . import packing as P
from .graph import EdgeView


def require_hip(t: torch.Tensor):
    if not t.is_cuda:
        raise L.DdpError("the MI355X score model runs on a HIP device only (no CPU/eager fallback); "
                         "move the batch to cuda:<n>")
    L.load()


def stream():
    return C.c_void_p(torch._C._cuda_getCurrentRawStream(torch._C._cuda_getDevice()))

# ... 227 lines not shown
        L.check(lib.ddp_conv_rows(C.byref(shape), arr, len(tasks), stream()), "ddp_conv_rows")
    else:
        L.check(lib.ddp_conv_messages(C.byref(shape), arr, len(tasks), stream()), "ddp_conv_messages")
    if prof is not None:
        e1.record()
        h2 = P.h2_steps(spec) > 0 and all(t._path.h2 for t in tasks)
        prof.record_conv(e0, e1, spec, flops_spec, [t._count for t in tasks], node_bytes, tag, h2,
                         rows=(2 if path.rows_form == 1 else 1) if path.rows else 0)


def launch_reduce(x, ldx, n_nodes, d_out, sources, accumulate=True, n_rep=1, rep_stride=0):
    lib = L.load()
    arr = (L.ReduceSrc * max(len(sources), 1))()
    for i, src_ in enumerate(sources):
        msg, view, pk = src_[:3]
        arr[i].msg, arr[i].rowptr = msg.data_ptr(), view.rowptr.data_ptr()
        arr[i].bn_scale, arr[i].bn_shift, arr[i].n_edges = pk.bn_scale.data_ptr(), pk.bn_shift.data_ptr(), view.n_edges
        arr[i].rowmap = src_[3].data_ptr() if (len(src_) > 3 and src_[3] is not None) else 0
        arr[i].n_edges_dev = _p(view.cnt)
    prof = profiler(hbm=True)
    if prof is not None:
        e0, e1 = torch.cuda.Event(enable_timing=True), torch.cuda.Event(enable_timing=True)
        e0.record()
    L.check(lib.ddp_segment_reduce(ptr(x), ldx, n_nodes, d_out, arr, len(sources), 1 if accumulate else 0, n_rep, rep_stride,
                                   stream()), "ddp_segment_reduce")
    if prof is not None:
        e1.record()
        views = [s_[1] for s_ in sources]

        def nbytes(views=views, d_out=d_out, n_nodes=n_nodes, n_rep=n_rep):
            ne = sum(v.n_edges if v.cnt is None else min(v.n_edges, int(v.cnt.item())) for v in views)
            return 4.0 * d_out * (ne + 2 * n_nodes * max(n_rep, 1))
        wide = (d_out % 4 == 0 and ldx % 4 == 0 and x.data_ptr() % 16 == 0 and not os.environ.get("DDP_REDUCE_NARROW")
                and all(s_[0].data_ptr() % 16 == 0 and s_[2].bn_scale.data_ptr() % 16 == 0 and s_[2].bn_shift.data_ptr() % 16 == 0 for s_ in sources))
        prof.hbm.setdefault("ddp_segment_reduce4_kernel" if wide else "ddp_segment_reduce_kernel", []).append((e0, e1, nbytes))


class EdgeMLPPack:

    def __init__(self, seq: nn.Sequential, rbf_slice: slice, device):
        W1, b1, W2, b2 = seq[0].weight.detach(), seq[0].bias.detach(), seq[3].weight.detach(), seq[3].bias.detach()
        ns = W1.shape[0]
        k = rbf_slice.stop - rbf_slice.start
        w1d = torch.zeros(k, 64, device=device)
        w1d[:, :ns] = W1[:, rbf_slice].t()
        w2 = torch.zeros(64, 64, device=device)
        w2[:ns, :ns] = W2.t()
        b2p = torch.zeros(64, device=device)
        b2p[:ns] = b2
        self.w1d, self.w2, self.b2, self.ns, self.k = w1d.contiguous(), w2.contiguous(), b2p, ns, k
        self.W1, self.b1 = W1, b1


def edge_featurize(pack: EdgeMLPPack, dist, pos_a, ia, pos_b, ib, pre, pre_idx, pre2=None, n_edges=None, cnt=None):
    lib = L.load()
    E = int(ia.shape[0]) if n_edges is None else int(n_edges)
    dev = pos_a.device
    out = torch.empty((E, pack.ns), device=dev, dtype=torch.float32)
    sh = torch.empty((E, 4), device=dev, dtype=torch.float32)
    if E == 0:
        return out, sh
    if pre.stride(1) != 1:
        pre = pre.contiguous()
    n2 = 0 if pre2 is None else int(pre2.shape[0])
    L.check(lib.ddp_edge_featurize(ptr(pos_a), ptr(ia), ptr(pos_b), ptr(ib), E, ptr(cnt), ptr(dist.offset), pack.k,
                                   C.c_float(dist.coeff), ptr(pre), ptr(pre_idx), pre.stride(0),
                                   ptr(pre2) if n2 else None, n2, pre2.stride(0) if n2 else 0, ptr(pack.w1d),
                                   ptr(pack.w2), ptr(pack.b2), pack.ns, ptr(out), ptr(sh), stream()),
            "ddp_edge_featurize")
    return out, sh


def edge_featurize_jobs(calls):
    if any(a[0].k % 8 or not 8 <= a[0].k <= 64 for a, _ in calls) or len(calls) > L.DDP_MAX_FEATURIZE_JOBS:
        return [edge_featurize(*a, **kw) for a, kw in calls]
    jobs, outs, keep = [], [], []
    for (pack, dist, pos_a, ia, pos_b, ib, pre, pre_idx), kw in calls:
        pre2, n_edges, cnt = kw.get("pre2"), kw.get("n_edges"), kw.get("cnt")
        E = int(ia.shape[0]) if n_edges is None else int(n_edges)
        out = torch.empty((E, pack.ns), device=pos_a.device, dtype=torch.float32)
        sh = torch.empty((E, 4), device=pos_a.device, dtype=torch.float32)
        outs.append((out, sh))
        if E == 0:
            continue
        if pre.stride(1) != 1:
            pre = pre.contiguous()
        n2 = 0 if pre2 is None else int(pre2.shape[0])
        j = L.FeaturizeJob()
        j.pos_a, j.ia, j.pos_b, j.ib, j.n_edges, j.n_edges_dev = _p(pos_a), _p(ia), _p(pos_b), _p(ib), E, _p(cnt)
        j.offset, j.k_rbf, j.coeff = _p(dist.offset), pack.k, float(dist.coeff)
        j.pre, j.pre_idx, j.ld_pre = _p(pre), _p(pre_idx), pre.stride(0)
        j.pre2, j.n_pre2, j.ld_pre2 = (_p(pre2) if n2 else 0), n2, (pre2.stride(0) if n2 else 0)
        j.w1d, j.w2, j.b2, j.ns, j.out, j.sh = _p(pack.w1d), _p(pack.w2), _p(pack.b2), pack.ns, _p(out), _p(sh)
        jobs.append(j)
        keep.append((pre, pre2, ia, ib, pre_idx))
    if jobs:
        arr = (L.FeaturizeJob * len(jobs))(*jobs)
        L.check(L.load().ddp_edge_featurize_jobs(arr, len(jobs), stream()), "ddp_edge_featurize_jobs")
    return outs


@dataclass
class StageAStack:
    W: torch.Tensor
    meta: list
    offs: object
    path: ConvPath
    gh: Optional[torch.Tensor]
    ld: int
    Wh: Optional[torch.Tensor] = None
    W3: Optional[torch.Tensor] = None

    def prepare(self, h2: bool, x3: bool) -> "StageAStack":
        if (h2 or self.path.rows) and self.Wh is None:
            self.Wh = P.split_h2(self.W, unified_scale=P.GH_SW) if self.path.rows else P.split_h2(self.W)
        if x3 and not self.path.rows and self.W3 is None:
            self.W3 = P.split_bf16x3(self.W)
        return self


def stage_a_stack(packs, hid: int, path: ConvPath) -> StageAStack:
    Ws, meta, ghs, lds = [], [], [], set()
    for key, pk in packs:
        for slot in (0, 1):
            if pk.wg[slot] is None:
                continue
            meta.append((key, slot, pk.g_in_off[slot]))
            Ws.append(pk.wgh[slot] if path.rows else pk.wg[slot])
            if path.rows:
                ghs.append(pk.gh_groups[slot])
                lds.add(pk.gh_ld[slot])
    assert len(lds) <= 1, "the convs of one stage-A launch write G rows of one length"
    W = torch.stack(Ws).contiguous()
    gh = torch.stack([P.gh_dest_table(ws, (hid + 7) // 8, W.shape[2], fmt=path.gh_fmt) for ws in ghs]).contiguous().to(W.device) if path.rows else None
    return StageAStack(W, meta, (C.c_int32 * len(meta))(*[mm[2] for mm in meta]), path, gh, lds.pop() if lds else W.shape[2])


def stage_a(x, n_rows, st: StageAStack, out, rows=None, rows_cnt=None, out_rows=None, h2=False, x3=False):
    lib = L.load()
    nb, n_in, ncols = st.W.shape
    if nb > L.DDP_MAX_GEMM_BATCH:
        raise L.DdpError("more (conv, slot) pairs per source array than DDP_MAX_GEMM_BATCH")
    if n_rows == 0:
        return
    args = (x.data_ptr(), x.stride(0), n_rows, ptr(rows), ptr(rows_cnt), out_rows if out_rows is not None else n_rows, st.offs, nb,
            st.W.data_ptr())
    if st.path.rows:
        fn, name = (lib.ddp_stage_a_gh3, "ddp_stage_a_gh3") if st.path.gh_fmt == 1 else (lib.ddp_stage_a_gh, "ddp_stage_a_gh")
        L.check(fn(*args, ptr(st.Wh), n_in, ncols, out.data_ptr(), st.ld, ptr(_RANGE_FLAG), st.gh.data_ptr(), stream()), name)
    elif h2:
        L.check(lib.ddp_stage_a_h2(*args, ptr(st.Wh), n_in, ncols, out.data_ptr(), ncols, ptr(_RANGE_FLAG), stream()), "ddp_stage_a_h2")
    else:
        L.check(lib.ddp_stage_a(*args, ptr(st.W3 if x3 else None), n_in, ncols, out.data_ptr(), ncols, stream()), "ddp_stage_a")


def _hold(j, *objs):
    j._keep = objs
    return j


def _run_jobs(fn, cls, jobs, what):
    lib = L.load()
    for i in range(0, len(jobs), L.DDP_MAX_LIST_JOBS):
        part = jobs[i:i + L.DDP_MAX_LIST_JOBS]
        arr = (cls * len(part))(*part)
        L.check(getattr(lib, fn)(arr, len(part), stream()), what)


def scan_job(n, flag=None, val=None, rowptr=None, base=0, excl=None, excl2=None, lst=None, total=None, n_dev=None) -> L.ScanJob:
    j = L.ScanJob()
    j.n, j.n_dev, j.flag, j.val, j.rowptr, j.base = n, _p(n_dev), _p(flag), _p(val), _p(rowptr), base
    j.excl, j.excl2, j.list, j.total = _p(excl), _p(excl2), _p(lst), _p(total)
    return _hold(j, flag, val, rowptr, excl, excl2, lst, total, n_dev)


def scan_jobs(jobs: Sequence[L.ScanJob]):
    _run_jobs("ddp_scan_jobs", L.ScanJob, list(jobs), "ddp_scan_jobs")


def mark_job(mask, idx, n, n_dev=None) -> L.MarkJob:
    j = L.MarkJob()
    j.idx, j.n, j.n_dev, j.mask = _p(idx), n, _p(n_dev), _p(mask)
    return _hold(j, idx, n_dev, mask)


def mark_jobs(jobs: Sequence[L.MarkJob]):
    _run_jobs("ddp_mark_jobs", L.MarkJob, list(jobs), "ddp_mark_jobs")


def rowcopy_job(n_rows, keep, old_rowptr, new_rowptr, ins, outs) -> L.RowcopyJob:
    j = L.RowcopyJob()
    j.n_rows, j.keep, j.old_rowptr, j.new_rowptr = n_rows, _p(keep), _p(old_rowptr), _p(new_rowptr)
    for k, (a, b) in enumerate(zip(ins, outs)):
        j.inp[k], j.out[k] = _p(a), _p(b)
    return _hold(j, keep, old_rowptr, new_rowptr, list(ins), list(outs))


def rowcopy_jobs(jobs: Sequence[L.RowcopyJob]):
    _run_jobs("ddp_rowcopy_jobs", L.RowcopyJob, list(jobs), "ddp_rowcopy_jobs")


def select_job(n, mask_a, idx_a, mask_b, idx_b, pays, outs, total, scratch, out_idx=None, n_dev=None, pay_add=None) -> L.SelectJob:
    j = L.SelectJob()
    nb = (n + 2047) // 2048
    j.n, j.n_dev, j.mask_a, j.idx_a, j.mask_b, j.idx_b, j.out_idx = n, _p(n_dev), _p(mask_a), _p(idx_a), _p(mask_b), _p(idx_b), _p(out_idx)
    for k, (a, b) in enumerate(zip(pays, outs)):
        j.pay[k], j.out[k] = _p(a), _p(b)
        j.pay_add[k] = 0 if pay_add is None else pay_add[k]
    j.total = _p(total)
    j.block_count, j.block_off = scratch.data_ptr(), scratch.data_ptr() + 4 * nb
    return _hold(j, n_dev, mask_a, idx_a, mask_b, idx_b, out_idx, list(pays), list(outs), total, scratch)


def select_jobs(jobs: Sequence[L.SelectJob]):
    _run_jobs("ddp_select_jobs", L.SelectJob, list(jobs), "ddp_select_jobs")


def radius_job(x, x_ptr, y, y_batch, r, cap, flags, counts, offsets=None, base=0, total=None, out_query=None, out_x=None,
               capacity=0, graph_div=None, overflow=None) -> L.RadiusJob:
    j = L.RadiusJob()
    j.x, j.x_ptr, j.y, j.y_batch, j.ny = x.data_ptr(), x_ptr.data_ptr(), y.data_ptr(), y_batch.data_ptr(), int(y.shape[0])
    j.r, j.max_neighbors, j.flags, j.graph_div = float(r), int(cap), int(flags), _p(graph_div)
    j.counts, j.offsets, j.base, j.total = _p(counts), _p(offsets), int(base), _p(total)
    j.out_query, j.out_x, j.capacity, j.overflow = _p(out_query), _p(out_x), int(capacity), _p(overflow)
    return _hold(j, x, x_ptr, y, y_batch, graph_div, counts, offsets, total, out_query, out_x, overflow)


def radius_search_jobs(jobs: Sequence[L.RadiusJob]):
    _run_jobs("ddp_radius_search_jobs", L.RadiusJob, list(jobs), "ddp_radius_search_jobs")


def group_job(key, n_items, n_keys, pays, rowptr, perm=None, out_key=None, outs=(), scratch=None, n_dev=None, key_map=None) -> L.GroupJob:
    j = L.GroupJob()
    j.key, j.n_items, j.n_items_dev, j.n_keys = _p(key), n_items, _p(n_dev), n_keys
    for k, a in enumerate(pays):
        j.pay[k] = _p(a)
    j.rowptr, j.perm, j.out_key, j.key_map, j.scratch = _p(rowptr), _p(perm), _p(out_key), _p(key_map), _p(scratch)
    for k, a in enumerate(outs):
        j.out[k] = _p(a)
    return _hold(j, key, n_dev, list(pays), rowptr, perm, out_key, list(outs), key_map, scratch)


def group_jobs(jobs: Sequence[L.GroupJob]):
    _run_jobs("ddp_group_by_key_jobs", L.GroupJob, list(jobs), "ddp_group_by_key_jobs")


def gather_rows(x, idx, n, out, ncols, n_dev=None):
    lib = L.load()
    if n > 0:
        L.check(lib.ddp_gather_rows(x.data_ptr(), x.stride(0), idx.data_ptr(), n, ptr(n_dev), out.data_ptr(), out.stride(0), ncols,
                                    stream()), "ddp_gather_rows")


def flex_mark(a, b, n_edges, e0, n_a_per_graph, n_b_per_graph, mark, pos=None, flag=None, a_too=False, ref_list=False):
    L.check(L.load().ddp_flex_mark(ptr(pos), ptr(flag), n_b_per_graph, ptr(a), ptr(b), n_edges, e0, n_a_per_graph, int(a_too), int(ref_list),
                                   ptr(mark), stream()), "ddp_flex_mark")


def fallback_rowmap(mark, recv, old_rowptr, new_rowptr, n_edges, n_recv_per_graph, rowmap):
    L.check(L.load().ddp_fallback_rowmap(ptr(mark), ptr(recv), ptr(old_rowptr), ptr(new_rowptr), n_edges, n_recv_per_graph, ptr(rowmap),
                                         stream()), "ddp_fallback_rowmap")


def clean_pair_maps(touched, recv, src, n_edges, e0, n_graphs, n0, rowmap, rows_v, rowptr=None):
    lib = L.load()
    L.check(lib.ddp_clean_pair_maps(touched.data_ptr(), recv.data_ptr(), src.data_ptr(), ptr(rowptr), n_edges, e0, n_graphs, n0,
                                    rowmap.data_ptr(), rows_v.data_ptr(), stream()), "ddp_clean_pair_maps")


def _eval_arg(t, dtype, dev, what):
    if t.device != dev or t.dtype != dtype or not t.is_contiguous():
        raise L.DdpError(f"{what}: expected a contiguous {dtype} tensor on {dev}, got {t.dtype} on {t.device}")


def pose_rmsd(pred, ref, perms, sel=None, rmsd=None, best=None):
    dev = pred.device
    S, n, P = pred.shape[0], perms.shape[0], perms.shape[1]
    for t, dt, w in ((pred, torch.float32, "pred"), (ref, torch.float32, "ref"), (perms, torch.int32, "perms")):
        _eval_arg(t, dt, dev, f"pose_rmsd {w}")
    if sel is not None:
        _eval_arg(sel, torch.int32, dev, "pose_rmsd sel")
        if sel.shape != (n,):
            raise L.DdpError("pose_rmsd: sel must have one entry per perms row")
    elif n > pred.shape[1]:
        raise L.DdpError("pose_rmsd: more perms rows than pred rows")
    if pred.dim() != 3 or pred.shape[2] != 3 or ref.dim() != 2 or ref.shape[1] != 3 or perms.dim() != 2:
        raise L.DdpError("pose_rmsd: pred [S, rows, 3], ref [n_ref, 3], perms [n, P]")
    rmsd = torch.empty(S, dtype=torch.float32, device=dev) if rmsd is None else rmsd
    best = torch.empty(S, dtype=torch.int32, device=dev) if best is None else best
    if S == 0:
        return rmsd, best
    L.check(L.load().ddp_pose_rmsd(pred.data_ptr(), S, pred.shape[1] * 3, _p(sel), n, ref.data_ptr(), ref.shape[0], perms.data_ptr(), P,
                                   rmsd.data_ptr(), best.data_ptr(), stream()), "ddp_pose_rmsd")
    return rmsd, best


def pose_contacts(lig, lig_radii, rec, rec_radii, ref_centroid, overlap=0.4, out=None):
    dev = lig.device
    S, n = lig.shape[0], lig.shape[1]
    for t, w in ((lig, "lig"), (lig_radii, "lig_radii"), (rec, "rec"), (rec_radii, "rec_radii"), (ref_centroid, "ref_centroid")):
        _eval_arg(t, torch.float32, dev, f"pose_contacts {w}")
    if lig.dim() != 3 or lig.shape[2] != 3 or rec.dim() not in (2, 3) or rec.shape[-1] != 3:
        raise L.DdpError("pose_contacts: lig [S, n, 3], rec [m, 3] or [S, m, 3]")
    m = rec.shape[-2]
    if rec.dim() == 3 and rec.shape[0] != S:
        raise L.DdpError("pose_contacts: a per-sample receptor needs one row block per sample")
# ... 320 lines not shown
```

diffdock_pocket_amd/score_model.py:

```python
from __future__ import annotations

import math
import os
from typing import Dict, List, Optional

import numpy as np
import torch
from torch import nn

from . import _lib as L
from . import graph as G
from . import launch as K
from . import packing as P
from .synthetic import LIG_FEATURE_DIMS, REC_ATOM_FEATURE_DIMS, REC_RESIDUE_FEATURE_DIMS

ASSETS = os.path.join(os.path.dirname(os.path.abspath(__file__)), "assets")


class GaussianSmearing(nn.Module):

    def __init__(self, start=0.0, stop=5.0, num_gaussians=50):
        super().__init__()
        offset = torch.linspace(start, stop, num_gaussians)
        self.coeff = -0.5 / (offset[1] - offset[0]).item() ** 2
# ... 267 lines not shown
_EdgeMLPPack, _edge_featurize = K.EdgeMLPPack, K.edge_featurize
_make_task, _launch_convs, _launch_reduce = K.make_task, K.launch_convs, K.launch_reduce


class _EncoderPack:

    def __init__(self, enc, dev):
        tabs = [e.weight.detach().float() for e in enc.atom_embedding_list]
        self.table = torch.cat(tabs, 0).contiguous().to(dev)
        self.feat_off = [0]
        for t in tabs[:-1]:
            self.feat_off.append(self.feat_off[-1] + t.shape[0])
        self.n_cat, self.emb_dim = len(tabs), tabs[0].shape[1]
        self.old = isinstance(enc, OldAtomEncoder)
        if self.old:
            self.has_lm = enc.lm_embedding_type is not None
            self.n_scalar = enc.num_scalar_features
            if self.n_scalar > 0:
                self.w1, self.b1 = enc.linear.weight.detach().float().t().contiguous().to(dev), enc.linear.bias.detach().float().to(dev)
            if self.has_lm:
                lin = enc.lm_embedding_layer
                self.w2, self.b2 = lin.weight.detach().float().t().contiguous().to(dev), lin.bias.detach().float().to(dev)
        else:
            self.has_extra = enc.additional_features_dim > 0
            if self.has_extra:
                lin = enc.additional_features_embedder
                self.w, self.b = lin.weight.detach().float().t().contiguous().to(dev), lin.bias.detach().float().to(dev)


def _node_job(n_rows, out, ncols, w, bias, zero_to=0, cat=None, pack=None, emb_mode=0, dense=(), sigma=None, sig_out=None, add=None):
    j = L.NodeJob()
    j.n_rows, j.out, j.ld_out, j.ncols, j.zero_to = n_rows, out.data_ptr(), out.stride(0), ncols, zero_to
    j.w, j.bias = w.data_ptr(), (bias.data_ptr() if bias is not None else 0)
    if cat is not None and emb_mode:
        j.cat, j.ld_cat, j.n_cat, j.table, j.emb_dim, j.emb_mode = cat.data_ptr(), cat.stride(0), pack.n_cat, pack.table.data_ptr(), pack.emb_dim, emb_mode
        for f, o in enumerate(pack.feat_off):
            j.feat_off[f] = o
    for d, (ten, c0, n) in enumerate(dense):
        j.dense[d], j.ld_dense[d], j.n_dense[d] = ten.data_ptr() + 4 * c0, ten.stride(0), n
    if sigma is not None and sigma[0] == "t":
        _, t, scale, freq, sd = sigma
        j.t, j.t_stride, j.scale, j.freq, j.sd = t.data_ptr(), (t.stride(0) if t.numel() > 1 else 0), scale, freq.data_ptr(), sd
    elif sigma is not None:
        j.sig_emb, j.ld_sig, j.sd = sigma[1].data_ptr(), sigma[1].stride(0), sigma[1].shape[1]
    if sig_out is not None:
        j.sig_out, j.ld_sig_out = sig_out.data_ptr(), sig_out.stride(0)
    if add is not None:
        j.add, j.ld_add = add.data_ptr(), add.stride(0)
    return j


def _launch_node_jobs(jobs):
    lib = L.load()
    for i in range(0, len(jobs), L.DDP_MAX_NODE_JOBS):
        part = jobs[i:i + L.DDP_MAX_NODE_JOBS]
        arr = (L.NodeJob * len(part))(*part)
        L.check(lib.ddp_node_linear(arr, len(part), _stream()), "ddp_node_linear")


class TensorProductScoreModel(nn.Module):
    def __init__(self, t_to_sigma, device, timestep_emb_func, in_lig_edge_features=4, sigma_embed_dim=32, sh_lmax=2,
                 ns=16, nv=4, num_conv_layers=2, lig_max_radius=5, rec_max_radius=30, cross_max_distance=250,
                 center_max_distance=30, distance_embed_dim=32, cross_distance_embed_dim=32, no_torsion=False,
                 scale_by_sigma=True, norm_by_sigma=True, use_second_order_repr=False, batch_norm=True,
                 dynamic_max_cross=False, dropout=0.0, smooth_edges=False, odd_parity=False,
                 separate_noise_schedule=False, lm_embedding_type=False, confidence_mode=False,
                 confidence_dropout=0, confidence_no_batchnorm=False,
                 asyncronous_noise_schedule=False, affinity_prediction=False, parallel=1,
                 parallel_aggregators="mean max min std", num_confidence_outputs=1, fixed_center_conv=False,
                 atom_max_neighbors=None,
                 no_aminoacid_identities=False, flexible_sidechains=False, include_miscellaneous_atoms=False,
                 use_old_atom_encoder=False):
        super().__init__()
        unsupported = {"sh_lmax != 1": sh_lmax != 1, "use_second_order_repr": use_second_order_repr,
                       "odd_parity": odd_parity,
                       "separate_noise_schedule": separate_noise_schedule,
                       "asyncronous_noise_schedule": asyncronous_noise_schedule,
                       "affinity_prediction": affinity_prediction, "parallel > 1": parallel != 1,
                       "include_miscellaneous_atoms": include_miscellaneous_atoms}
        bad = [k for k, v in unsupported.items() if v]
        if bad:
            raise NotImplementedError("MI355X score model: unsupported configuration: " + ", ".join(bad))
        assert (not no_aminoacid_identities) or (lm_embedding_type is None), "no language model emb without identities"
        if num_conv_layers < 1:
            raise NotImplementedError("num_conv_layers >= 1 required")
        self.t_to_sigma = t_to_sigma
        self.device = device
        self.timestep_emb_func = timestep_emb_func
        self.in_lig_edge_features = in_lig_edge_features
        self.sigma_embed_dim = sigma_embed_dim
        self.lig_max_radius, self.rec_max_radius = lig_max_radius, rec_max_radius
        self.cross_max_distance, self.dynamic_max_cross = cross_max_distance, dynamic_max_cross
        self.center_max_distance = center_max_distance
        self.distance_embed_dim, self.cross_distance_embed_dim = distance_embed_dim, cross_distance_embed_dim
        self.ns, self.nv = ns, nv
        self.scale_by_sigma, self.norm_by_sigma = scale_by_sigma, norm_by_sigma
        self.no_torsion = no_torsion
        self.num_conv_layers = num_conv_layers
        self.fixed_center_conv = fixed_center_conv
        self.atom_max_neighbors = atom_max_neighbors
        self.no_aminoacid_identities = no_aminoacid_identities
        self.flexible_sidechains = flexible_sidechains
        self.confidence_mode = bool(confidence_mode)
        self.smooth_edges = bool(smooth_edges)

        enc = OldAtomEncoder if use_old_atom_encoder else AtomEncoder
        sd, dd, cd = sigma_embed_dim, distance_embed_dim, cross_distance_embed_dim
        self.lig_node_embedding = enc(ns, LIG_FEATURE_DIMS, sd)
        self.lig_edge_embedding = _mlp(in_lig_edge_features + sd + dd, ns, ns, dropout)
        self.rec_node_embedding = enc(ns, REC_RESIDUE_FEATURE_DIMS, sd, lm_embedding_type=lm_embedding_type)
        self.rec_edge_embedding = _mlp(sd + dd, ns, ns, dropout)
        self.atom_node_embedding = enc(ns, REC_ATOM_FEATURE_DIMS, sd)
        self.atom_edge_embedding = _mlp(sd + dd, ns, ns, dropout)
        self.lr_edge_embedding = _mlp(sd + cd, ns, ns, dropout)
        self.ar_edge_embedding = _mlp(sd + dd, ns, ns, dropout)
        self.la_edge_embedding = _mlp(sd + cd, ns, ns, dropout)
        self.lig_distance_expansion = GaussianSmearing(0.0, lig_max_radius, dd)
        self.rec_distance_expansion = GaussianSmearing(0.0, rec_max_radius, dd)
        self.cross_distance_expansion = GaussianSmearing(0.0, cross_max_distance, cd)

        def out_blocks(m):
            return [(mul, dim, s) for mul, dim, s in ((m[0], 1, True), (m[1], 3, False), (m[2], 3, False), (m[3], 1, False))
                    if mul > 0]

        convs = []
        self._layer_specs, self._layer_specs_g = [], []
        self.factorize_min_degree = 3.0
        self.prune_last_receptor_layer = True
        self.share_layer0 = True
        self.share_clean_layer1 = True
        self.share_flex_layer0 = True
        self.flex_share_min_work = 2_000_000
        self.plan_min_edges = 0
        self._static_cache = {}
        self.before_layers = None
        self.cache_slot = 0
        self._stage_a_stacks = {}
        self.section_timer = None
        self.check_weight_values = True
        self.range_check_in_forward = True
        self.la_capacity_per_atom = 128
        self.concurrent_small_batches = True
        self.concurrent_max_atoms = 16000
        self.fork_small_means = True
        self.overlap_direct_conv = True
        self.split_rows_launch = True
        self.shape_early_rows = False
        self.split_rows_min_g_bytes = 3.0e9
        self.fork_front = True
        self.fork_lists_flex = True
        self.concurrent_heads = True
        self.stage_a_bf16x3 = False
        self.stage_a_h2 = True
        self._overflow_flag = None
        self.exact_sizes = False
        self.debug_conv_outputs = None
        for i in range(num_conv_layers):
            mi, mo = P.irreps_muls(ns, nv, i), P.irreps_muls(ns, nv, i + 1)
            spec = P.faster_tp_spec(mi, mo, 3 * ns)
            spec_g = P.faster_tp_spec(mi, mo, 3 * ns, factorized=True)
            self._layer_specs.append(spec)
            self._layer_specs_g.append(spec_g)
            for _ in range(9):
                convs.append(TensorProductConvLayer(spec, out_blocks(mo), batch_norm=batch_norm, dropout=dropout,
                                                    spec_g=spec_g))
        self.conv_layers = nn.ModuleList(convs)
        m_final = P.irreps_muls(ns, nv, num_conv_layers)
        self._d_final = P.irreps_dim(m_final)
        self._ldx = (P.irreps_dim(P.irreps_muls(ns, nv, num_conv_layers)) + 3) // 4 * 4

        if self.confidence_mode:
            conf_in = (2 * ns if num_conv_layers >= 3 else ns) * (2 if flexible_sidechains else 1)
            bn = (lambda: nn.Identity()) if confidence_no_batchnorm else (lambda: nn.BatchNorm1d(ns))
            self.confidence_predictor = nn.Sequential(
                nn.Linear(conf_in, ns), bn(), nn.ReLU(), nn.Dropout(confidence_dropout),
                nn.Linear(ns, ns), bn(), nn.ReLU(), nn.Dropout(confidence_dropout),
                nn.Linear(ns, num_confidence_outputs))
        else:
            self.center_distance_expansion = GaussianSmearing(0.0, center_max_distance, dd)
            self.center_edge_embedding = _mlp(dd + sd, ns, ns, dropout)
            self.final_conv = TensorProductConvLayer(P.faster_tp_spec(m_final, (0, 2, 2, 0), 2 * ns),
                                                     [(2, 3, False), (2, 3, False)], batch_norm=batch_norm, dropout=dropout)
            self.tr_final_layer = nn.Sequential(nn.Linear(1 + sd, ns), nn.Dropout(dropout), nn.ReLU(), nn.Linear(ns, 1))
            self.rot_final_layer = nn.Sequential(nn.Linear(1 + sd, ns), nn.Dropout(dropout), nn.ReLU(), nn.Linear(ns, 1))
            tor_blocks = [(ns, 1, False), (ns, 1, True)]
            if not no_torsion:
                self.final_edge_embedding = _mlp(dd, ns, ns, dropout)
                self.tor_bond_conv = TensorProductConvLayer(P.torsion_tp_spec(m_final, ns, 3 * ns), tor_blocks,
                                                            batch_norm=batch_norm, dropout=dropout)
                self.tor_final_layer = nn.Sequential(nn.Linear(2 * ns, ns, bias=False), nn.Tanh(), nn.Dropout(dropout),
                                                     nn.Linear(ns, 1, bias=False))
            if flexible_sidechains:
                self.sidechain_final_edge_embedding = _mlp(dd, ns, ns, dropout)
                self.sc_tor_bond_conv = TensorProductConvLayer(P.torsion_tp_spec(m_final, ns, 3 * ns), tor_blocks,
                                                               batch_norm=batch_norm, dropout=dropout)
                self.sc_tor_final_layer = nn.Sequential(nn.Linear(2 * ns, ns, bias=False), nn.Tanh(), nn.Dropout(dropout),
                                                        nn.Linear(ns, 1, bias=False))
        with np.load(os.path.join(ASSETS, "score_norm_tables.npz")) as z:
            self._so3_table = torch.from_numpy(z["so3_exp_score_norms"]).float()
            self._torus_table = torch.from_numpy(z["torus_score_norm"]).float()
        self._edge_packs: Dict[str, _EdgeMLPPack] = {}
        self.last_stats: Dict[str, float] = {}
        self.rows_mfma16, self.g_planes3, self.direct_rows = rows_defaults()
        self.direct_rows_max_split = int(os.environ.get("DDP_DIRECT_SPLIT", "6"))

    _IGNORED_PREFIXES = ("final_tp_tor.", "final_tp_sc_tor.", "tor_bond_conv.tp.", "sc_tor_bond_conv.tp.")

    def load_state_dict(self, state_dict, strict=True, **kw):
        sd = {k: v for k, v in state_dict.items() if not k.startswith(self._IGNORED_PREFIXES)}
        out = super().load_state_dict(sd, strict=strict, **kw)
        self.invalidate_packed()
        return out

    def _shared_receptor_side(self, B, rec, atom, rpos, apos, lay_r, lay_a, rr, ar, aa, atoms=True):
        out = {3: None, 5: None, 6: None, 8: None}
        if B < 2 or not (lay_r.uniform and lay_a.uniform):
            return out
        nr, na = lay_r.nmax, lay_a.nmax

        def same_rows(t, n):
            v = t.reshape(B, n, -1)
            return bool((v == v[:1]).all())

        def same_edges(ei, n0, n1):
            E = ei.shape[1]
            if E == 0 or E % B:
                return 0
            e = E // B
            off = torch.arange(B, device=ei.device).unsqueeze(1)
            a, b = ei[0].reshape(B, e) - off * n0, ei[1].reshape(B, e) - off * n1
            ok = (a == a[:1]).all() & (b == b[:1]).all() & (a >= 0).all() & (a < n0).all() & (b >= 0).all() & (b < n1).all()
            return e if bool(ok) else 0

        rec_same = same_rows(rec.x, nr) and same_rows(rpos, nr)
        atom_same = atoms is True and same_rows(atom.x, na) and same_rows(apos, na)
        if rec_same:
            e = same_edges(rr, nr, nr)
            out[6] = (nr, e, nr) if e else None
        if atoms == "static" and rec_same and same_rows(atom.x, na):
            e = same_edges(ar, na, nr)
            out["flex"] = (na, e, nr) if e else None
        if atom_same:
            e = same_edges(aa, na, na)
            out[3] = (na, e, na) if e else None
        if rec_same and atom_same:
            e = same_edges(ar, na, nr)
            if e:
                out[5], out[8] = (na, e, nr), (nr, e, na)
        return out

    def _weight_tensors(self):
        ts = self.__dict__.get("_weight_tensors_")
        if ts is None:
            ts = self.__dict__["_weight_tensors_"] = list(self.parameters()) + list(self.buffers())
        return ts

    def _weights_version(self):
        return sum(t._version for t in self._weight_tensors())

    def _weights_fingerprint(self):
        ts = [t.detach() for t in self._weight_tensors() if t.is_floating_point() and t.numel() > 0]
        if not ts:
            return ()
        parts = torch._foreach_norm(ts, 1) + torch._foreach_norm(ts, 2)
        return tuple(torch.stack([p.double() for p in parts]).tolist())

    def _refresh_weight_caches(self):
        wv = self._weights_version()
        fp = self._weights_fingerprint() if self.check_weight_values else self.__dict__.get("_weights_seen_fp")
        if self.__dict__.get("_weights_seen") != wv or self.__dict__.get("_weights_seen_fp") != fp:
            self.invalidate_packed()
            self._weights_seen = wv
            self._weights_seen_fp = fp if self.check_weight_values else self._weights_fingerprint()

    def overflow_flag(self, dev):
        if self._overflow_flag is None:
            self._overflow_flag = torch.zeros(2, dtype=torch.int32).pin_memory()
        return self._overflow_flag

    def check_overflow(self, range_too=True):
        if self._overflow_flag is None:
            return
        trunc, rng = int(self._overflow_flag[0]) != 0, range_too and int(self._overflow_flag[1]) != 0
        if not (trunc or rng):
            return
        if range_too:
            self._overflow_flag.zero_()
        else:
            self._overflow_flag[0] = 0
        msgs = []
        if rng:
            msgs.append("a node feature / edge feature / fc activation / G value outside the fp16 range (|v| > 65504, or NaN) reached the fp16 "
                        "hi/lo split kernels of an earlier forward whose scores were consumed without the range check (a hand-driven "
                        "Sampler.step sequence without Sampler.check_overflow): they are not to be trusted - model.conv_h2 = False runs the "
                        "exact fp32 MFMA form")
        if trunc:
            msgs.append(f"a ligand atom had more than la_capacity_per_atom = {self.la_capacity_per_atom} pocket atoms within lig_max_radius: "
                        f"the ligand<-atom edge list of an earlier forward was truncated; raise the capacity")
        raise L.DdpError("; ".join(msgs))

    def range_flag_raised(self, clear=True):
        if self._overflow_flag is None or int(self._overflow_flag[1]) == 0:
            return False
        if clear:
            self._overflow_flag[1] = 0
        return True
# ... 258 lines not shown
```

include/ddp_hip.h:

```cpp
#ifndef DDP_HIP_H
#define DDP_HIP_H

#include <stdint.h>

#ifdef __cplusplus
extern "C" {
#endif

#define DDP_ABI_VERSION 17
#define DDP_EINVAL (-1)
#define DDP_ELIMIT (-2)

#define DDP_MAX_TASKS 9
#define DDP_MAX_BLOCKS 4
#define DDP_MAX_SEGS 3
#define DDP_MAX_NS 64
#define DDP_EDGE_TILE 64

enum ddp_feat_kind {
  DDP_F_SCALAR_S0 = 0,
  DDP_F_DOT = 1,
  DDP_F_SCALAR_S1 = 2,
  DDP_F_VEC_S0 = 3,
  DDP_F_CROSS = 4
// ... 57 lines not shown
  const float* w1p;
  const float* b1p;
  const float* w2p;
  const float* b2p;
  float* msg;
  const float* g[2];
  const int32_t* pos;
  const int32_t* n_edges_dev;
  const void* w1h;
  const void* w2h;
  int32_t* h2_range_flag;
  const void* wsh;
  const float* bsp;
  const void* gh[2];
  int32_t gh_fmt;
  int32_t rows_form;
  int32_t rows_bias_k;
  int32_t rows_seg0, rows_seg1, rows_nts;
} ddp_conv_task_t;
#define DDP_ROWS_SX 16
#define DDP_ROWS_SW 256
#define DDP_ROWS_SH 16
#define DDP_ROWS_SG 32
#define DDP_ROWS_KPERM(ks, hh, i) (32 * ((ks) >> 1) + ((8 * ((ks) & 1) + (i)) & 3) + 8 * ((8 * ((ks) & 1) + (i)) >> 2) + 4 * (hh))
#define DDP_ROWS16_POS(j) (16 * (((j) & 7) >> 2) + 4 * ((j) >> 3) + ((j) & 3))
#define DDP_GH3_LD(hid, gcp) ((((((hid) + 7) / 8) * (gcp) + ((gcp) + 5) / 6 + 15) / 16) * 96)
#define DDP_GH_LD(hid, gcp) ((((((hid) + 7) / 8) * 8 + 1) * (gcp) + 31) / 32 * 32)
int ddp_conv_messages(const ddp_conv_shape_t* shape, const ddp_conv_task_t* tasks, int ntasks, void* stream);

int ddp_conv_rows(const ddp_conv_shape_t* shape, const ddp_conv_task_t* tasks, int ntasks, void* stream);

typedef struct {
  const float* msg;
  const int32_t* rowptr;
  const float* bn_scale;
  const float* bn_shift;
  int32_t n_edges;
  const int32_t* rowmap;
  const int32_t* n_edges_dev;
} ddp_reduce_src_t;
int ddp_segment_reduce(float* x, int ldx, int n_nodes, int d_out, const ddp_reduce_src_t* srcs, int nsrc,
                       int accumulate, int n_rep, int rep_stride, void* stream);

int ddp_edge_featurize(const float* pos_a, const int32_t* ia, const float* pos_b, const int32_t* ib, int n_edges,
                       const int32_t* n_edges_dev, const float* offset, int k_rbf, float coeff, const float* pre,
                       const int32_t* pre_idx, int ld_pre, const float* pre2, int n_pre2, int ld_pre2, const float* w1d,
                       const float* w2, const float* b2, int ns, float* out, float* sh, void* stream);

#define DDP_MAX_FEATURIZE_JOBS 8
typedef struct {
  const float* pos_a;
  const int32_t* ia;
  const float* pos_b;
  const int32_t* ib;
  int32_t n_edges;
  const int32_t* n_edges_dev;
  const float* offset;
  int32_t k_rbf;
  float coeff;
  const float* pre;
  const int32_t* pre_idx;
  int32_t ld_pre;
  const float* pre2;
  int32_t n_pre2, ld_pre2;
  const float* w1d;
  const float* w2;
  const float* b2;
  int32_t ns;
  float* out;
  float* sh;
} ddp_featurize_job_t;
int ddp_edge_featurize_jobs(const ddp_featurize_job_t* jobs, int njobs, void* stream);

int ddp_torsion_sh(const float* sh_edge, const float* bond_vec, const int32_t* bond_of_edge, int n_edges,
                   const int32_t* n_edges_dev, float* out, const float* x, int ldx, int ns, const int32_t* b0,
                   const int32_t* b1, int n_bonds, float* bond_attr, void* stream);

typedef struct {
  const float* t[4];
  int32_t t_stride[4];
  float sig_min[4], sig_max[4];
  float* sigma[4];
  int32_t n_graphs;
  float* cut;
  float cut_mul, cut_add;
  float* graph_emb;
  int32_t sd;
  float emb_scale;
  const float* freq;
  const float* lig_pos;
  const int32_t* graph_ptr;
  float* center;
  struct {
    const float* pos;
    const int32_t* b0;
    const int32_t* b1;
    int32_t n;
    float* mid;
    float* vec;
  } bonds[2];
  struct {
    const int32_t* src;
    int32_t* dst;
    int32_t n;
  } copy[2];
} ddp_prologue_args_t;
int ddp_step_prologue(const ddp_prologue_args_t* args, void* stream);

typedef struct {
  const float* gp;
  int32_t ld_gp, n_graphs, ns, sd;
  const float* graph_emb;
  const float* w1[2];
  const float* b1[2];
  const float* w2[2];
  const float* b2[2];
  const float* sigma[2];
  const float* so3_table;
  int32_t so3_n;
  float so3_lo, so3_span;
  float* out[2];
} ddp_trrot_args_t;
int ddp_trrot_head(const ddp_trrot_args_t* args, void* stream);

typedef struct {
  const float* h;
  int32_t ld_h, n_bonds, ns;
  const float* w1;
  const float* w2;
  const float* sigma;
  const int32_t* graph_of_bond;
  const float* torus_table;
  int32_t torus_n;
  float torus_lo, torus_span;
  float* out;
} ddp_tor_args_t;
int ddp_tor_head(const ddp_tor_args_t* args, void* stream);

#define DDP_MAX_GEMM_BATCH 16
#define DDP_G_LD(hid, gcols) ((((((hid) + 3) / 4) * 4 + 1) * (gcols) + 31) / 32 * 32)
int ddp_stage_a(const float* x, int ldx, int nrows, const int32_t* rows, const int32_t* nrows_dev, int out_rows, const int32_t* offs,
                int nbatch, const float* w, const void* w_bf16x3, int k, int ncols, float* out, int ldo, void* stream);

int ddp_stage_a_h2(const float* x, int ldx, int nrows, const int32_t* rows, const int32_t* nrows_dev, int out_rows, const int32_t* offs,
                   int nbatch, const float* w, const void* w_h2, int k, int ncols, float* out, int ldo, int32_t* range_flag, void* stream);
int ddp_stage_a_gh(const float* x, int ldx, int nrows, const int32_t* rows, const int32_t* nrows_dev, int out_rows, const int32_t* offs,
                   int nbatch, const float* w, const void* w_h2, int k, int ncols, float* out, int ldo, int32_t* range_flag,
                   const int32_t* dest, void* stream);

int ddp_stage_a_gh3(const float* x, int ldx, int nrows, const int32_t* rows, const int32_t* nrows_dev, int out_rows, const int32_t* offs,
                    int nbatch, const float* w, const void* w_h2, int k, int ncols, float* out, int ldo, int32_t* range_flag,
                    const int32_t* dest, void* stream);

#define DDP_GH_SX 2

int ddp_set_occupancy_shaping(int rows_min_lds_bytes, int stage_a_lds_pad_bytes);

int ddp_pose_update(const float* pos_in, int n_samples, int n_atoms, const float* tr, const float* rot, const float* tor,
                    int n_tor, const int32_t* bonds, const uint8_t* mask_rotate, float* pos_out, void* stream);

int ddp_sidechain_update(const float* pos_in, int n_samples, int n_atoms, const float* angles, int n_bonds,
                         const int32_t* edge_idx, const int32_t* subcomponents, const int32_t* mapping, float* pos_out,
                         void* stream);

typedef struct {
  const float* score[4];
  const float* z[4];
  float* out[4];
  int32_t n[4];
} ddp_sde_args_t;
int ddp_sde_update(const float* coef, const ddp_sde_args_t* args, void* stream);

#define DDP_RADIUS_DROP_SELF 1
#define DDP_RADIUS_NEAREST 2
int ddp_radius_count(const float* x, const int32_t* x_ptr, const float* y, const int32_t* y_batch, int ny, float r,
                     int max_neighbors, int flags, int32_t* counts, void* stream);
int ddp_radius_fill(const float* x, const int32_t* x_ptr, const float* y, const int32_t* y_batch, int ny, float r,
                    int max_neighbors, int flags, const int32_t* offsets, int32_t* out_query, int32_t* out_x, void* stream);
int ddp_knn(const float* x, const int32_t* x_ptr, const int32_t* batch, int n, int k, int32_t* out_neighbors, void* stream);

int ddp_group_by_key(const int32_t* key, int n_items, int n_keys, const int32_t* pay0, const int32_t* pay1, const int32_t* pay2,
                     int32_t* rowptr, int32_t* perm, int32_t* out_key, int32_t* out0, int32_t* out1, int32_t* out2,
                     int32_t* scratch, void* stream);

#define DDP_MAX_LIST_JOBS 12

typedef struct {
  int32_t n;
  const int32_t* n_dev;
  const int32_t* flag;
  const int32_t* val;
  const int32_t* rowptr;
  int32_t base;
  int32_t* excl;
  int32_t* excl2;
  int32_t* list;
  int32_t* total;
} ddp_scan_job_t;
int ddp_scan_jobs(const ddp_scan_job_t* jobs, int njobs, void* stream);

typedef struct {
  const int32_t* idx;
  int32_t n;
  const int32_t* n_dev;
  int32_t* mask;
} ddp_mark_job_t;
int ddp_mark_jobs(const ddp_mark_job_t* jobs, int njobs, void* stream);

typedef struct {
  int32_t n_rows;
  const int32_t* keep;
  const int32_t* old_rowptr;
  const int32_t* new_rowptr;
  const int32_t* in[3];
  int32_t* out[3];
} ddp_rowcopy_job_t;
int ddp_rowcopy_jobs(const ddp_rowcopy_job_t* jobs, int njobs, void* stream);

typedef struct {
  int32_t n;
  const int32_t* n_dev;
  const int32_t* mask_a;
  const int32_t* idx_a;
  const int32_t* mask_b;
  const int32_t* idx_b;
  int32_t* out_idx;
  const int32_t* pay[4];
  int32_t pay_add[4];
  int32_t* out[4];
  int32_t* total;
  int32_t* block_count;
  int32_t* block_off;
} ddp_select_job_t;
int ddp_select_jobs(const ddp_select_job_t* jobs, int njobs, void* stream);

int ddp_gather_rows(const float* x, int ldx, const int32_t* idx, int n, const int32_t* n_dev, float* out, int ldo, int ncols,
                    void* stream);

int ddp_clean_pair_maps(const int32_t* touched, const int32_t* recv, const int32_t* src, const int32_t* rowptr, int n_edges, int e0,
                        int n_graphs, int n0, int32_t* rowmap, int32_t* rows_v, void* stream);

int ddp_flex_mark(const float* pos, const int32_t* flag, int n_b_per_graph, const int32_t* a, const int32_t* b, int n_edges, int e0,
                  int n_a_per_graph, int a_too, int ref_list, int32_t* mark, void* stream);
int ddp_fallback_rowmap(const int32_t* mark, const int32_t* recv, const int32_t* old_rowptr, const int32_t* new_rowptr, int n_edges,
                        int n_recv_per_graph, int32_t* rowmap, void* stream);

typedef struct {
  const float* x;
  const int32_t* x_ptr;
  const float* y;
  const int32_t* y_batch;
  int32_t ny;
  float r;
  int32_t max_neighbors;
  int32_t flags;
  const float* graph_div;
  int32_t* counts;
  int32_t* offsets;
  int32_t base;
  int32_t* total;
  int32_t* out_query;
  int32_t* out_x;
  int32_t capacity;
  int32_t* overflow;
} ddp_radius_job_t;
int ddp_radius_search_jobs(const ddp_radius_job_t* jobs, int njobs, void* stream);

typedef struct {
  const int32_t* key;
  int32_t n_items;
  const int32_t* n_items_dev;
  int32_t n_keys;
  const int32_t* pay[3];
  int32_t* rowptr;
  int32_t* perm;
  int32_t* out_key;
  int32_t* out[3];
  const int32_t* key_map;
  int32_t* scratch;
} ddp_group_job_t;
int ddp_group_by_key_jobs(const ddp_group_job_t* jobs, int njobs, void* stream);

#define DDP_MAX_NODE_JOBS 8
#define DDP_MAX_NODE_CAT 16
typedef struct {
  int32_t n_rows;
  const int32_t* cat;
  int32_t ld_cat, n_cat;
  const float* table;
  int32_t feat_off[DDP_MAX_NODE_CAT];
  int32_t emb_dim, emb_mode;
  const float* dense[2];
  int32_t ld_dense[2], n_dense[2];
  const float* t;
  int32_t t_stride;
  float scale;
  const float* freq;
  const float* sig_emb;
  int32_t ld_sig, sd;
  float* sig_out;
  int32_t ld_sig_out;
  const float* w;
  const float* bias;
  float* out;
  int32_t ld_out, ncols, zero_to;
  const float* add;
// ... 172 lines not shown
```

Measured before the change: 172.2.

## Batch multiple stage-A GEMM launches into one grouped jobs kernel

Adds a grouped stage-A kernel that takes a table of up to eight jobs as a kernel argument and maps a flat workgroup index to (job, bx, by, z). The Python layer collects the stage-A calls of a layer and issues them as one launch instead of several launches or forked streams. This targets launch overhead and the tail of small grids, and lets work from different groups fill the device at once. In exchange, every job must share k and the output format, each workgroup does a short linear job lookup, and the jobs are ordered by size on the host.

```diff
diff --git a/diffdock_pocket_amd/_lib.py b/diffdock_pocket_amd/_lib.py
--- a/diffdock_pocket_amd/_lib.py
+++ b/diffdock_pocket_amd/_lib.py
@@ -15,7 +15,7 @@
 DDP_MINIMIZE_MAX_ATOMS, DDP_MINIMIZE_MAX_TORSIONS = 512, 4096
 DDP_MINIMIZE_FLEX_MAX_MOVING, DDP_MINIMIZE_FLEX_MAX_BONDS, DDP_MINIMIZE_FLEX_MAX_STATE_BYTES = 256, 256, 47040
 DDP_PAIRWISE_MAX_SAMPLES, DDP_CLUSTER_MAX_SAMPLES = 32768, 1024
-EXPORTS = ["ddp_conv_messages", "ddp_conv_rows", "ddp_stage_a_gh", "ddp_stage_a_gh3", "ddp_segment_reduce", "ddp_edge_featurize", "ddp_edge_featurize_jobs", "ddp_torsion_sh", "ddp_stage_a", "ddp_stage_a_h2",
+EXPORTS = ["ddp_conv_messages", "ddp_conv_rows", "ddp_stage_a_gh", "ddp_stage_a_gh3", "ddp_segment_reduce", "ddp_edge_featurize", "ddp_edge_featurize_jobs", "ddp_torsion_sh", "ddp_stage_a", "ddp_stage_a_h2", "ddp_stage_a_jobs", "ddp_stage_a_jobs_plan",
            "ddp_pose_update", "ddp_sidechain_update", "ddp_sde_update", "ddp_radius_count", "ddp_radius_fill", "ddp_knn", "ddp_group_by_key", "ddp_node_linear", "ddp_scan_jobs", "ddp_mark_jobs", "ddp_rowcopy_jobs", "ddp_select_jobs",
            "ddp_gather_rows", "ddp_clean_pair_maps", "ddp_flex_mark", "ddp_fallback_rowmap", "ddp_step_prologue", "ddp_trrot_head", "ddp_tor_head", "ddp_radius_search_jobs", "ddp_group_by_key_jobs", "ddp_set_occupancy_shaping", "ddp_pose_rmsd", "ddp_pose_contacts", "ddp_pose_pairwise_rmsd", "ddp_pose_cluster", "ddp_traj_record", "ddp_svgd_tau", "ddp_svgd_pairs", "ddp_svgd_rows", "ddp_refine_energy", "ddp_refine_direction", "ddp_refine_accept", "ddp_pose_score", "ddp_pose_minimize", "ddp_pose_minimize_flex", "ddp_pocket_occupancy", "ddp_pocket_buriedness", "ddp_pocket_label", "ddp_abi_version", "ddp_last_error", "ddp_source_hash"]
 
@@ -147,6 +147,14 @@
     _fields_ = [("pos_a", _P), ("ia", _P), ("pos_b", _P), ("ib", _P), ("n_edges", _I), ("n_edges_dev", _P), ("offset", _P), ("k_rbf", _I),
                 ("coeff", C.c_float), ("pre", _P), ("pre_idx", _P), ("ld_pre", _I), ("pre2", _P), ("n_pre2", _I), ("ld_pre2", _I),
                 ("w1d", _P), ("w2", _P), ("b2", _P), ("ns", _I), ("out", _P), ("sh", _P)]
+
+
+DDP_MAX_STAGE_A_JOBS = 8
+
+
+class StageAJob(C.Structure):
+    _fields_ = [("x", _P), ("ldx", _I), ("nrows", _I), ("rows", _P), ("nrows_dev", _P), ("out_rows", _I), ("offs", _I * DDP_MAX_GEMM_BATCH),
+                ("nbatch", _I), ("w", _P), ("w_h2", _P), ("k", _I), ("ncols", _I), ("out", _P), ("ldo", _I), ("dest", _P), ("gh_fmt", _I)]
 
 
 class _BondJob(C.Structure):
@@ -235,6 +243,10 @@
     lib.ddp_stage_a_gh.restype = C.c_int
     lib.ddp_stage_a_gh3.argtypes = lib.ddp_stage_a_gh.argtypes
     lib.ddp_stage_a_gh3.restype = C.c_int
+    lib.ddp_stage_a_jobs.argtypes = [C.POINTER(StageAJob), C.c_int, C.c_void_p, C.c_void_p]
+    lib.ddp_stage_a_jobs.restype = C.c_int
+    lib.ddp_stage_a_jobs_plan.argtypes = [C.POINTER(StageAJob), C.c_int, C.POINTER(C.c_int32), C.POINTER(C.c_int32)]
+    lib.ddp_stage_a_jobs_plan.restype = C.c_int
     lib.ddp_set_occupancy_shaping.argtypes = [C.c_int, C.c_int]
     lib.ddp_set_occupancy_shaping.restype = C.c_int
     lib.ddp_pose_update.argtypes = [C.c_void_p, C.c_int, C.c_int, C.c_void_p, C.c_void_p, C.c_void_p, C.c_int, C.c_void_p,
diff --git a/diffdock_pocket_amd/csrc/ddp_gemm.hip b/diffdock_pocket_amd/csrc/ddp_gemm.hip
--- a/diffdock_pocket_amd/csrc/ddp_gemm.hip
+++ b/diffdock_pocket_amd/csrc/ddp_gemm.hip
@@ -401,16 +401,14 @@
 #define DDP_SAH_CT 4
 #endif
 
-template <int KT, bool GH = false, bool G3 = false>
-__global__ __launch_bounds__(DDP_GEMM_THREADS, 2) void ddp_stage_a_h2_kernel(const float* __restrict__ x, int ldx, int nrows,
-                                                                              const int32_t* __restrict__ rows,
-                                                                              const int32_t* __restrict__ nrows_dev, int out_rows,
-                                                                              int mrows, const GemmOffs offs,
-                                                                              const _Float16* __restrict__ wh, int ncols,
-                                                                              float* __restrict__ out, int ldo, int32_t* range_flag,
-                                                                              const int32_t* __restrict__ gh_dest = nullptr) {
+template <int KT, bool GH, bool G3>
+__device__ __forceinline__ void stage_a_h2_body(const float* __restrict__ x, int ldx, int nrows, const int32_t* __restrict__ rows,
+                                                const int32_t* __restrict__ nrows_dev, int out_rows, int mrows, const int off_z,
+                                                const _Float16* __restrict__ wh, int ncols, float* __restrict__ out, int ldo,
+                                                int32_t* range_flag, const int32_t* __restrict__ gh_dest, const int bx, const int by,
+                                                const int z, const int gdy) {
   if (nrows_dev) nrows = min(nrows, *nrows_dev);
-  if ((int)blockIdx.y * mrows >= nrows) return;
+  if (by * mrows >= nrows) return;
   constexpr int KP = (KT + 15) / 16 * 16, NS = KP / 16, CT = GH ? DDP_SAH_CT_GH : DDP_SAH_CT;
   constexpr int XS = KP + 8;
   constexpr int NV = (32 * KT / 4 + DDP_GEMM_THREADS - 1) / DDP_GEMM_THREADS;
@@ -419,9 +417,9 @@
   __shared__ __attribute__((aligned(16))) _Float16 xt[2][2][32 * XS];
   __shared__ __attribute__((aligned(16))) float st[G3 ? 1 : 4][2][G3 ? 4 : 32 * TS];
   __shared__ __attribute__((aligned(16))) char g3t[G3 ? 4 : 1][G3 ? 32 * RS3 : 16];
-  const int z = (int)blockIdx.z, tid = (int)threadIdx.x;
+  const int tid = (int)threadIdx.x;
   const int wave = tid >> 6, lane = tid & 63, r = lane & 31, hh = lane >> 5;
-  const int col0 = ((int)blockIdx.x * 4 + wave) * (32 * CT);
+  const int col0 = (bx * 4 + wave) * (32 * CT);
   h8 wr[CT][2][NS];
 #pragma unroll
   for (int t = 0; t < CT; ++t) {
@@ -438,7 +436,7 @@
       xt[bp / 2][bp % 2][rr * XS + KT + kk] = (_Float16)0.f;
     }
   }
-  const float* __restrict__ xb = x + offs.off[z];
+  const float* __restrict__ xb = x + off_z;
   float* __restrict__ ob = out + (size_t)z * out_rows * ldo;
   int cq[CT];
 #pragma unroll
@@ -469,9 +467,9 @@
       g3_pc[j] = (64 * j + lane) % 24;
     }
   }
-  for (int R0 = (int)blockIdx.y * mrows; R0 < nrows; R0 += (int)gridDim.y * mrows) {
+  for (int R0 = by * mrows; R0 < nrows; R0 += gdy * mrows) {
   const int R1 = min(nrows, R0 + mrows);
-  const bool al4 = ((ldx | offs.off[z]) & 3) == 0 && (reinterpret_cast<size_t>(x) & 15) == 0;
+  const bool al4 = ((ldx | off_z) & 3) == 0 && (reinterpret_cast<size_t>(x) & 15) == 0;
   f32x4 xv[NV];
   auto fetch = [&](int row0) {
 #pragma unroll
@@ -710,6 +708,66 @@
   if constexpr (GH) {
     if (!(gh_max <= 65504.f) && range_flag) *range_flag = 1;
   }
+}
+
+template <int KT, bool GH = false, bool G3 = false>
+__global__ __launch_bounds__(DDP_GEMM_THREADS, 2) void ddp_stage_a_h2_kernel(const float* __restrict__ x, int ldx, int nrows,
+                                                                              const int32_t* __restrict__ rows,
+                                                                              const int32_t* __restrict__ nrows_dev, int out_rows,
+                                                                              int mrows, const GemmOffs offs,
+                                                                              const _Float16* __restrict__ wh, int ncols,
+                                                                              float* __restrict__ out, int ldo, int32_t* range_flag,
+                                                                              const int32_t* __restrict__ gh_dest = nullptr) {
+  stage_a_h2_body<KT, GH, G3>(x, ldx, nrows, rows, nrows_dev, out_rows, mrows, offs.off[blockIdx.z], wh, ncols, out, ldo, range_flag, gh_dest,
+                              (int)blockIdx.x, (int)blockIdx.y, (int)blockIdx.z, (int)gridDim.y);
+}
+
+struct StageAJob {
+  const float* x;
+  const int32_t* rows;
+  const int32_t* nrows_dev;
+  const _Float16* wh;
+  float* out;
+  const int32_t* gh_dest;
+  int ldx, nrows, out_rows, mrows, ncols, ldo, gx, gy;
+  int off[DDP_MAX_GEMM_BATCH];
+};
+struct StageAJobs {
+  int njobs;
+  int wg_start[DDP_MAX_STAGE_A_JOBS + 1];
+  StageAJob job[DDP_MAX_STAGE_A_JOBS];
+};
+static_assert(sizeof(StageAJobs) < 4096, "the job table travels as a kernel argument");
+
+template <int KT, bool GH, bool G3>
+__global__ __launch_bounds__(DDP_GEMM_THREADS, 2) void ddp_stage_a_h2_jobs_kernel(const StageAJobs T, int32_t* range_flag) {
+  const int wg = (int)blockIdx.x;
+  int j = 0;
+  while (j + 1 < T.njobs && wg >= T.wg_start[j + 1]) ++j;
+  const StageAJob& J = T.job[j];
+  const int local = wg - T.wg_start[j];
+  const int bx = local % J.gx, t = local / J.gx, by = t % J.gy, z = t / J.gy;
+  stage_a_h2_body<KT, GH, G3>(J.x, J.ldx, J.nrows, J.rows, J.nrows_dev, J.out_rows, J.mrows, J.off[z], J.wh, J.ncols, J.out, J.ldo, range_flag,
+                              J.gh_dest, bx, by, z, J.gy);
+}
+
+struct StageATile {
+  int mrows, gy;
+};
+static StageATile stage_a_tile(int nrows, bool listed) {
+  int mrows = listed ? (nrows >= 16384 ? 256 : 128) : (nrows >= 8192 ? DDP_GEMM_MROWS : nrows >= 384 ? 256 : 64);
+  int gy = (nrows + mrows - 1) / mrows;
+  if (listed && gy > 96) gy = 96;
+#ifdef DDP_SA_TUNE
+  if (nrows < 8192 || listed) {
+    if (const char* e = getenv("DDP_SA_MROWS")) mrows = atoi(e);
+    gy = (nrows + mrows - 1) / mrows;
+    const char* c = getenv("DDP_SA_GYCAP");
+    const int cap = c ? atoi(c) : 96;
+    if (listed && gy > cap) gy = cap;
+  }
+#endif
+  return StageATile{mrows, gy};
 }
 
 static int stage_a_impl(const float* x, int ldx, int nrows, const int32_t* rows, const int32_t* nrows_dev, int out_rows,
@@ -739,21 +797,12 @@
   hipLaunchKernelGGL((ddp_stage_a_mfma_kernel<KT>), dim3((ncols + 128 * DDP_SA_CT - 1) / (128 * DDP_SA_CT), gy, nbatch), \
                      dim3(DDP_GEMM_THREADS), 0, s, x, ldx, nrows, rows, nrows_dev, out_rows, mrows, O, w, ncols, out, ldo)
   const bool listed = rows && nrows_dev;
-  int mrows = listed ? (nrows >= 16384 ? 256 : 128) : (nrows >= 8192 ? DDP_GEMM_MROWS : nrows >= 384 ? 256 : 64);
-  int gy = (nrows + mrows - 1) / mrows;
-  if (listed && gy > 96) gy = 96;
-#ifdef DDP_SA_TUNE
-  if (nrows < 8192 || listed) {
-    if (const char* e = getenv("DDP_SA_MROWS")) mrows = atoi(e);
-    gy = (nrows + mrows - 1) / mrows;
-    const char* c = getenv("DDP_SA_GYCAP");
-    const int cap = c ? atoi(c) : 96;
-    if (listed && gy > cap) gy = cap;
-  }
-#endif
+  const StageATile tile = stage_a_tile(nrows, listed);
+  const int mrows = tile.mrows, gy = tile.gy;
   static const bool no_mfma = getenv("DDP_STAGE_A_VALU") != nullptr;
   if (gh_dest) {
-    if (!(w_h2 && wide && (k == 60 || k == 32 || k == 24 || k == 16) && (reinterpret_cast<size_t>(w_h2) & 15) == 0 && (ncols & 31) == 0 &&
+    const bool al16 = ((ncols | ldo) & 3) == 0 && (reinterpret_cast<size_t>(out) & 15) == 0;
+    if (!(w_h2 && al16 && (k == 60 || k == 32 || k == 24 || k == 16) && (reinterpret_cast<size_t>(w_h2) & 15) == 0 && (ncols & 31) == 0 &&
           (reinterpret_cast<size_t>(gh_dest) & 7) == 0))
       return ddp_fail(DDP_EINVAL, "ddp_stage_a_gh: plane output needs the h2 path (w_h2, k in {60, 32, 24, 16}) and ncols % 32 == 0");
     const dim3 grid((ncols + 128 * DDP_SAH_CT_GH - 1) / (128 * DDP_SAH_CT_GH), gy, nbatch);
@@ -860,3 +909,113 @@
   if (!dest) return ddp_fail(DDP_EINVAL, "ddp_stage_a_gh3: dest");
   return stage_a_impl(x, ldx, nrows, rows, nrows_dev, out_rows, offs, nbatch, w, nullptr, w_h2, k, ncols, out, ldo, range_flag, stream, dest, 1);
 }
+
+static bool stage_a_job_empty(const ddp_stage_a_job_t& J) { return J.nrows == 0 || J.nbatch == 0; }
+
+static int stage_a_jobs_table(const ddp_stage_a_job_t* jobs, int njobs, StageAJobs* T, int32_t* plan, int* k_out, int* fmt_out) {
+  if (njobs < 0 || njobs > DDP_MAX_STAGE_A_JOBS) return ddp_fail(DDP_ELIMIT, "ddp_stage_a_jobs: njobs > DDP_MAX_STAGE_A_JOBS");
+  if (njobs > 0 && !jobs) return ddp_fail(DDP_EINVAL, "ddp_stage_a_jobs: null jobs");
+  int k = 0, fmt = 0, wg = 0;
+  T->njobs = 0;
+  T->wg_start[0] = 0;
+  for (int i = 0; i < njobs; ++i) {
+    const ddp_stage_a_job_t& J = jobs[i];
+    if (J.nbatch < 0 || J.nbatch > DDP_MAX_GEMM_BATCH) return ddp_fail(DDP_ELIMIT, "ddp_stage_a_jobs: nbatch > DDP_MAX_GEMM_BATCH");
+    if (J.nrows < 0 || J.ncols < 1) return ddp_fail(DDP_EINVAL, "ddp_stage_a_jobs: ncols / nrows");
+    if (!J.dest || !(J.k == 60 || J.k == 32 || J.k == 24 || J.k == 16) || (J.gh_fmt != 0 && J.gh_fmt != 1) || (J.ncols & 31) != 0 ||
+        (J.gh_fmt == 1 && (J.ncols & 127) != 0))
+      return ddp_fail(DDP_EINVAL, "ddp_stage_a_jobs: every job runs the plane path (dest, k in {60, 32, 24, 16}, ncols as ddp_stage_a_gh / _gh3 need it)");
+    int32_t* pl = plan ? plan + 5 * i : nullptr;
+    if (stage_a_job_empty(J)) {
+      if (pl) { pl[0] = pl[1] = pl[2] = pl[3] = 0; pl[4] = wg; }
+      continue;
+    }
+    if (T->njobs == 0) {
+      k = J.k;
+      fmt = J.gh_fmt;
+    } else if (J.k != k || J.gh_fmt != fmt) {
+      return ddp_fail(DDP_EINVAL, "ddp_stage_a_jobs: the jobs of a call share one k and one gh_fmt");
+    }
+    const StageATile tile = stage_a_tile(J.nrows, J.rows && J.nrows_dev);
+    const int gx = (J.ncols + 128 * DDP_SAH_CT_GH - 1) / (128 * DDP_SAH_CT_GH);
+    const long long n = (long long)gx * tile.gy * J.nbatch;
+    if (wg + n > 0x7fffffffLL) return ddp_fail(DDP_ELIMIT, "ddp_stage_a_jobs: grid");
+    StageAJob& D = T->job[T->njobs];
+    D.gx = gx;
+    D.gy = tile.gy;
+    D.mrows = tile.mrows;
+    if (pl) { pl[0] = gx; pl[1] = tile.gy; pl[2] = J.nbatch; pl[3] = tile.mrows; pl[4] = wg; }
+    wg += (int)n;
+    T->wg_start[++T->njobs] = wg;
+  }
+  for (int i = T->njobs + 1; i <= DDP_MAX_STAGE_A_JOBS; ++i) T->wg_start[i] = wg;
+  if (k_out) *k_out = k;
+  if (fmt_out) *fmt_out = fmt;
+  return 0;
+}
+
+extern "C" int ddp_stage_a_jobs_plan(const ddp_stage_a_job_t* jobs, int njobs, int32_t* plan, int32_t* n_workgroups) {
+  if (!plan && njobs > 0) return ddp_fail(DDP_EINVAL, "ddp_stage_a_jobs_plan: null plan");
+  StageAJobs T;
+  if (int rc = stage_a_jobs_table(jobs, njobs, &T, plan, nullptr, nullptr)) return rc;
+  if (n_workgroups) *n_workgroups = T.wg_start[T.njobs];
+  return 0;
+}
+
+extern "C" int ddp_stage_a_jobs(const ddp_stage_a_job_t* jobs, int njobs, int32_t* range_flag, void* stream) {
+  StageAJobs T;
+  int k = 0, fmt = 0;
+  if (int rc = stage_a_jobs_table(jobs, njobs, &T, nullptr, &k, &fmt)) return rc;
+  if (T.njobs == 0) return 0;
+  for (int i = 0, n = 0; i < njobs; ++i) {
+    const ddp_stage_a_job_t& J = jobs[i];
+    if (stage_a_job_empty(J)) continue;
+    StageAJob& D = T.job[n++];
+    const int out_rows = J.rows ? J.out_rows : J.nrows;
+    if (out_rows < 1) return ddp_fail(DDP_EINVAL, "ddp_stage_a_jobs: out_rows");
+    if (J.gh_fmt == 1 ? (J.ldo < (J.ncols / 8) * 6 || (J.ldo & 31) != 0) : (J.ldo < J.ncols || (J.ldo & 3) != 0))
+      return ddp_fail(DDP_EINVAL, "ddp_stage_a_jobs: ldo");
+    if (!J.x || !J.w || !J.w_h2 || !J.out) return ddp_fail(DDP_EINVAL, "ddp_stage_a_jobs: null argument");
+    if ((reinterpret_cast<size_t>(J.x) & 3) || (reinterpret_cast<size_t>(J.out) & 15) || (reinterpret_cast<size_t>(J.w_h2) & 15) ||
+        (reinterpret_cast<size_t>(J.dest) & 7))
+      return ddp_fail(DDP_EINVAL, "ddp_stage_a_jobs: x must be 4-byte aligned, out and w_h2 16-byte aligned, dest 8-byte aligned");
+    D.x = J.x;
+    D.rows = J.rows;
+    D.nrows_dev = J.nrows_dev;
+    D.wh = reinterpret_cast<const _Float16*>(J.w_h2);
+    D.out = J.out;
+    D.gh_dest = J.dest;
+    D.ldx = J.ldx;
+    D.nrows = J.nrows;
+    D.out_rows = out_rows;
+    D.ncols = J.ncols;
+    D.ldo = J.ldo;
+    for (int b = 0; b < DDP_MAX_GEMM_BATCH; ++b) D.off[b] = (b < J.nbatch) ? J.offs[b] : 0;
+  }
+  hipStream_t s = (hipStream_t)stream;
+  const dim3 grid(T.wg_start[T.njobs]);
+  const int pad = ddp_shape_stage_a_pad;
+  static int pad_have[8] = {0, 0, 0, 0, 0, 0, 0, 0};
+#define DDP_GEMM_JOBS(KT, I)                                                                                     \
+  {                                                                                                              \
+    if (pad > 0) {                                                                                               \
+      const hipError_t ep = (fmt == 1) ? ddp_need_lds(reinterpret_cast<const void*>(ddp_stage_a_h2_jobs_kernel<KT, true, true>), pad, &pad_have[4 + I]) \
+                                       : ddp_need_lds(reinterpret_cast<const void*>(ddp_stage_a_h2_jobs_kernel<KT, true, false>), pad, &pad_have[I]); \
+      if (ep != hipSuccess) return ddp_fail_hip(ep, "hipFuncSetAttribute(stage A jobs)");                        \
+    }                                                                                                            \
+    if (fmt == 1)                                                                                                \
+      hipLaunchKernelGGL((ddp_stage_a_h2_jobs_kernel<KT, true, true>), grid, dim3(DDP_GEMM_THREADS), pad, s, T, range_flag); \
+    else                                                                                                         \
+      hipLaunchKernelGGL((ddp_stage_a_h2_jobs_kernel<KT, true, false>), grid, dim3(DDP_GEMM_THREADS), pad, s, T, range_flag); \
+  }
+  switch (k) {
+    case 60: DDP_GEMM_JOBS(60, 0); break;
+    case 32: DDP_GEMM_JOBS(32, 1); break;
+    case 24: DDP_GEMM_JOBS(24, 2); break;
+    default: DDP_GEMM_JOBS(16, 3); break;
+  }
+#undef DDP_GEMM_JOBS
+  const hipError_t e = hipGetLastError();
+  if (e != hipSuccess) return ddp_fail_hip(e, "ddp_stage_a_jobs launch");
+  return 0;
+}
diff --git a/diffdock_pocket_amd/csrc/ddp_misc.hip b/diffdock_pocket_amd/csrc/ddp_misc.hip
--- a/diffdock_pocket_amd/csrc/ddp_misc.hip
+++ b/diffdock_pocket_amd/csrc/ddp_misc.hip
@@ -7,6 +7,8 @@
 
 typedef float f32x4 __attribute__((ext_vector_type(4)));
 
+#define DDP_REDUCE_REP_SPLIT 8
+#define DDP_REDUCE_REP_BATCH 8
 struct ReduceLaunch {
   ddp_reduce_src_t src[3];
   int nsrc;
@@ -55,22 +57,34 @@
   if (n_rep <= 1) {
     *dst = total;
   } else {
-    for (int g = 0; g < n_rep; ++g) {
-      float* d = dst + (size_t)g * rep_stride * ldx;
-      *d = *d + total;
-    }
-  }
-}
-
-typedef float red4 __attribute__((ext_vector_type(4)));
-__global__ __launch_bounds__(256) void ddp_segment_reduce4_kernel(float* __restrict__ x, int ldx, int n_nodes, int d_out, ReduceLaunch L,
-                                                                  int accumulate, int n_rep, int rep_stride) {
-  const int nq = d_out >> 2;
+    const int g0 = (int)blockIdx.y, gs = (int)gridDim.y;
+    for (int gb = g0; gb < n_rep; gb += DDP_REDUCE_REP_BATCH * gs) {
+      float v[DDP_REDUCE_REP_BATCH];
+#pragma unroll
+      for (int i = 0; i < DDP_REDUCE_REP_BATCH; ++i) {
+        const int g = gb + i * gs;
+        v[i] = g < n_rep ? dst[(size_t)g * rep_stride * ldx] : 0.f;
+      }
+#pragma unroll
+      for (int i = 0; i < DDP_REDUCE_REP_BATCH; ++i) {
+        const int g = gb + i * gs;
+        if (g < n_rep) dst[(size_t)g * rep_stride * ldx] = v[i] + total;
+      }
+    }
+  }
+}
+
+template <int V>
+__device__ __forceinline__ void segment_reduce_vec(float* __restrict__ x, int ldx, int n_nodes, int d_out, const ReduceLaunch& L,
+                                                   int accumulate, int n_rep, int rep_stride) {
+  typedef float redv __attribute__((ext_vector_type(V)));
+  const int nq = d_out / V;
   const long long item = (long long)blockIdx.x * 256 + threadIdx.x;
-  const int node = (int)(item / nq), ch = 4 * (int)(item - (long long)node * nq);
+  const int node = (int)(item / nq), ch = V * (int)(item - (long long)node * nq);
   if (node >= n_nodes) return;
   float* dst = x + (size_t)node * ldx + ch;
-  red4 total = (accumulate && n_rep <= 1) ? *reinterpret_cast<const red4*>(dst) : red4{0.f, 0.f, 0.f, 0.f};
+  redv total = 0.f;
+  if (accumulate && n_rep <= 1) total = *reinterpret_cast<const redv*>(dst);
   int p0[3], p1[3];
 #pragma unroll
   for (int k = 0; k < 3; ++k) {
@@ -84,9 +98,9 @@
       const ddp_reduce_src_t& s = L.src[k];
       const float* __restrict__ m = s.msg + ch;
       const int32_t* __restrict__ rm = s.rowmap;
-      red4 sum = {0.f, 0.f, 0.f, 0.f};
+      redv sum = 0.f;
       for (int p = p0[k]; p < p1[k]; p += 8) {
-        red4 v[8];
+        redv v[8];
         int row[8];
 #pragma unroll
         for (int i = 0; i < 8; ++i) {
@@ -94,26 +108,46 @@
           row[i] = rm ? rm[q] : q;
         }
 #pragma unroll
-        for (int i = 0; i < 8; ++i) v[i] = *reinterpret_cast<const red4*>(m + (size_t)row[i] * d_out);
+        for (int i = 0; i < 8; ++i) v[i] = *reinterpret_cast<const redv*>(m + (size_t)row[i] * d_out);
 #pragma unroll
         for (int i = 0; i < 8; ++i)
           if (p + i < p1[k]) sum += v[i];
       }
       const int cnt = p1[k] - p0[k];
       const float den = (float)(cnt > 1 ? cnt : 1);
-      const red4 sc = *reinterpret_cast<const red4*>(s.bn_scale + ch), sh = *reinterpret_cast<const red4*>(s.bn_shift + ch);
-#pragma unroll
-      for (int c = 0; c < 4; ++c) total[c] += (sum[c] / den) * sc[c] + sh[c];
+      const redv sc = *reinterpret_cast<const redv*>(s.bn_scale + ch), sh = *reinterpret_cast<const redv*>(s.bn_shift + ch);
+#pragma unroll
+      for (int c = 0; c < V; ++c) total[c] += (sum[c] / den) * sc[c] + sh[c];
     }
   }
   if (n_rep <= 1) {
-    *reinterpret_cast<red4*>(dst) = total;
+    *reinterpret_cast<redv*>(dst) = total;
   } else {
-    for (int g = 0; g < n_rep; ++g) {
-      red4* d = reinterpret_cast<red4*>(dst + (size_t)g * rep_stride * ldx);
-      *d = *d + total;
-    }
-  }
+    const int g0 = (int)blockIdx.y, gs = (int)gridDim.y;
+    for (int gb = g0; gb < n_rep; gb += DDP_REDUCE_REP_BATCH * gs) {
+      redv v[DDP_REDUCE_REP_BATCH];
+#pragma unroll
+      for (int i = 0; i < DDP_REDUCE_REP_BATCH; ++i) {
+        const int g = gb + i * gs;
+        v[i] = 0.f;
+        if (g < n_rep) v[i] = *reinterpret_cast<const redv*>(dst + (size_t)g * rep_stride * ldx);
+      }
+#pragma unroll
+      for (int i = 0; i < DDP_REDUCE_REP_BATCH; ++i) {
+        const int g = gb + i * gs;
+        if (g < n_rep) *reinterpret_cast<redv*>(dst + (size_t)g * rep_stride * ldx) = v[i] + total;
+      }
+    }
+  }
+}
+
+__global__ __launch_bounds__(256) void ddp_segment_reduce4_kernel(float* __restrict__ x, int ldx, int n_nodes, int d_out, ReduceLaunch L,
+                                                                  int accumulate, int n_rep, int rep_stride) {
+  segment_reduce_vec<4>(x, ldx, n_nodes, d_out, L, accumulate, n_rep, rep_stride);
+}
+__global__ __launch_bounds__(256) void ddp_segment_reduce2_kernel(float* __restrict__ x, int ldx, int n_nodes, int d_out, ReduceLaunch L,
+                                                                  int accumulate, int n_rep, int rep_stride) {
+  segment_reduce_vec<2>(x, ldx, n_nodes, d_out, L, accumulate, n_rep, rep_stride);
 }
 
 extern "C" int ddp_segment_reduce(float* x, int ldx, int n_nodes, int d_out, const ddp_reduce_src_t* srcs, int nsrc,
@@ -128,17 +162,24 @@
     if (srcs[i].n_edges > 0) L.src[L.nsrc++] = srcs[i];
   if (L.nsrc == 0 && (accumulate || n_rep > 1)) return 0;
   if (n_rep > 1 && rep_stride < n_nodes) return ddp_fail(DDP_EINVAL, "ddp_segment_reduce: rep_stride < n_nodes");
-  bool wide = ((d_out | ldx) & 3) == 0 && (reinterpret_cast<size_t>(x) & 15) == 0;
+  size_t al = reinterpret_cast<size_t>(x) | (size_t)(4 * (d_out | ldx));
   for (int i = 0; i < L.nsrc; ++i)
-    wide = wide && ((reinterpret_cast<size_t>(L.src[i].msg) | reinterpret_cast<size_t>(L.src[i].bn_scale) | reinterpret_cast<size_t>(L.src[i].bn_shift)) & 15) == 0;
+    al |= reinterpret_cast<size_t>(L.src[i].msg) | reinterpret_cast<size_t>(L.src[i].bn_scale) | reinterpret_cast<size_t>(L.src[i].bn_shift);
   static const bool narrow_only = getenv("DDP_REDUCE_NARROW") != nullptr;
-  if (wide && !narrow_only) {
-    const long long items = (long long)n_nodes * (d_out >> 2);
-    hipLaunchKernelGGL(ddp_segment_reduce4_kernel, dim3((unsigned)((items + 255) / 256)), dim3(256), 0, (hipStream_t)stream, x, ldx, n_nodes,
-                       d_out, L, accumulate, n_rep, rep_stride);
+  const int vec = narrow_only ? 1 : (al & 15) == 0 ? 4 : (al & 7) == 0 ? 2 : 1;
+  const unsigned rep = n_rep > 1 ? (unsigned)(n_rep < DDP_REDUCE_REP_SPLIT ? n_rep : DDP_REDUCE_REP_SPLIT) : 1u;
+  if (vec > 1) {
+    const long long items = (long long)n_nodes * (d_out / vec);
+    const dim3 grid((unsigned)((items + 255) / 256), rep);
+    if (vec == 4)
+      hipLaunchKernelGGL(ddp_segment_reduce4_kernel, grid, dim3(256), 0, (hipStream_t)stream, x, ldx, n_nodes, d_out, L, accumulate, n_rep,
+                         rep_stride);
+    else
+      hipLaunchKernelGGL(ddp_segment_reduce2_kernel, grid, dim3(256), 0, (hipStream_t)stream, x, ldx, n_nodes, d_out, L, accumulate, n_rep,
+                         rep_stride);
   } else {
     const int threads = ((d_out + 63) / 64) * 64;
-    hipLaunchKernelGGL(ddp_segment_reduce_kernel, dim3(n_nodes), dim3(threads), 0, (hipStream_t)stream, x, ldx, n_nodes,
+    hipLaunchKernelGGL(ddp_segment_reduce_kernel, dim3(n_nodes, rep), dim3(threads), 0, (hipStream_t)stream, x, ldx, n_nodes,
                        d_out, L, accumulate, n_rep, rep_stride);
   }
   hipError_t err = hipGetLastError();
diff --git a/diffdock_pocket_amd/engine.py b/diffdock_pocket_amd/engine.py
--- a/diffdock_pocket_amd/engine.py
+++ b/diffdock_pocket_amd/engine.py
@@ -656,33 +656,45 @@
         return K.conv_path(conv.packed_g(dev), self.m.rows_all_or_none(dev))
 
     def _stage_a(self, l, convs, x, n_rows, rows=None, rows_cnt=None, dense_rows=None):
+        return self._stage_a_many(l, [(convs, x, n_rows, rows, rows_cnt)])[0]
+
+    def _stage_a_many(self, l, items):
         m = self.m
-        paths = {self._conv_path(conv, x.device) for _, conv in convs}
-        if len(paths) != 1:
-            raise L.DdpError("the convs of one stage-A launch run through different conv paths")
-        path = paths.pop()
-        key = (l, tuple(k for k, _ in convs), path.rows)
-        st = m._stage_a_stacks.get(key)
-        if st is None or st.W.device != x.device:
-            st = m._stage_a_stacks[key] = K.stage_a_stack([(k, conv.packed_g(x.device)) for k, conv in convs], convs[0][1].spec_g.hid, path)
         h2 = m.stage_a_h2 and K.CONV_H2 and not m.stage_a_bf16x3
-        st.prepare(m.stage_a_h2, m.stage_a_bf16x3)
-        Gall = torch.empty((len(st.meta), n_rows, st.ld), device=x.device, dtype=torch.float32)
         prof = K.profiler(hbm=True)
-        if prof is not None:
-            e0, e1 = torch.cuda.Event(enable_timing=True), torch.cuda.Event(enable_timing=True)
-            e0.record()
-        n_list = n_rows if rows is None else int(rows.shape[0])
-        K.stage_a(x, n_list, st, Gall, rows=rows, rows_cnt=rows_cnt, out_rows=n_rows, h2=h2, x3=m.stage_a_bf16x3)
-        if prof is not None:
-            e1.record()
-            row_bytes = 4.0 * len(st.meta) * (st.ld + st.W.shape[1])
-
-            def nbytes(n_list=n_list, rows_cnt=rows_cnt, row_bytes=row_bytes, wn=st.W.numel()):
-                n = n_list if rows_cnt is None else min(n_list, int(rows_cnt.item()))
-                return row_bytes * n + 4.0 * wn
-            prof.hbm.setdefault("ddp_stage_a_h2_kernel" if (st.path.rows or h2) else "ddp_stage_a_mfma_kernel", []).append((e0, e1, nbytes))
-        return {(k, slot): Gall[i] for i, (k, slot, _) in enumerate(st.meta)}
+        calls, outs = [], []
+        for convs, x, n_rows, rows, rows_cnt in items:
+            paths = {self._conv_path(conv, x.device) for _, conv in convs}
+            if len(paths) != 1:
+                raise L.DdpError("the convs of one stage-A launch run through different conv paths")
+            path = paths.pop()
+            key = (l, tuple(k for k, _ in convs), path.rows)
+            st = m._stage_a_stacks.get(key)
+            if st is None or st.W.device != x.device:
+                st = m._stage_a_stacks[key] = K.stage_a_stack([(k, conv.packed_g(x.device)) for k, conv in convs], convs[0][1].spec_g.hid, path)
+            st.prepare(m.stage_a_h2, m.stage_a_bf16x3)
+            Gall = torch.empty((len(st.meta), n_rows, st.ld), device=x.device, dtype=torch.float32)
+            n_list = n_rows if rows is None else int(rows.shape[0])
+            calls.append(dict(x=x, n_rows=n_list, st=st, out=Gall, rows=rows, rows_cnt=rows_cnt, out_rows=n_rows, h2=h2, x3=m.stage_a_bf16x3))
+            outs.append({(k, slot): Gall[i] for i, (k, slot, _) in enumerate(st.meta)})
+        if prof is None and getattr(m, "stage_a_jobs", True) and len(calls) > 1:
+            K.stage_a_jobs(sorted(calls, key=lambda c: (c["rows_cnt"] is not None, -c["n_rows"] * len(c["st"].meta) * c["st"].ld)))
+            return outs
+        for c in calls:
+            st, n_list, rows_cnt = c["st"], c["n_rows"], c["rows_cnt"]
+            if prof is not None:
+                e0, e1 = torch.cuda.Event(enable_timing=True), torch.cuda.Event(enable_timing=True)
+                e0.record()
+            K.stage_a(**c)
+            if prof is not None:
+                e1.record()
+                row_bytes = 4.0 * len(st.meta) * (st.ld + st.W.shape[1])
+
+                def nbytes(n_list=n_list, rows_cnt=rows_cnt, row_bytes=row_bytes, wn=st.W.numel()):
+                    n = n_list if rows_cnt is None else min(n_list, int(rows_cnt.item()))
+                    return row_bytes * n + 4.0 * wn
+                prof.hbm.setdefault("ddp_stage_a_h2_kernel" if (st.path.rows or h2) else "ddp_stage_a_mfma_kernel", []).append((e0, e1, nbytes))
+        return outs
 
     def _layers(self, S, F, dev, mark):
         m = self.m
@@ -758,23 +770,37 @@
 
         def stage_a(P, which, forked=None):
             l = P.l
-            for gi, ((st_, gid), (x_src, rows, convs)) in enumerate(P.groups.items()):
-                if st_ not in which:
-                    continue
-                if forked is not None and gi > 0:
-                    P.gmap.update(forked.run((gi - 1) % 3, lambda: self._stage_a(l, convs, x_src, rows[3], rows=rows[1], rows_cnt=rows[2])))
-                else:
-                    P.gmap.update(self._stage_a(l, convs, x_src, rows[3], rows=rows[1], rows_cnt=rows[2]))
-            if forked is not None:
-                for i_ in range(3):
-                    forked.join(only=i_)
-            c1 = P.c1
-            if c1 is not None and "a" in which:
+            c1 = P.c1 if (P.c1 is not None and "a" in which) else None
+            groups = [(x_src, rows, convs) for (st_, gid), (x_src, rows, convs) in P.groups.items() if st_ in which]
+            if c1 is not None:
                 conv3 = m.conv_layers[9 * l + 3]
                 rows_d, rows_dc = c1.rows_d, c1.rows_d_cnt
                 if exact is not None:
                     rows_d, rows_dc = rows_d[:exact[rows_dc.data_ptr()]], None
-                P.g_d = self._stage_a(l, [(3, conv3)], xa, Na, rows=rows_d, rows_cnt=rows_dc)
+            every = [conv for _, _, convs in groups for _, conv in convs] + ([conv3] if c1 is not None else [])
+            jobs = (bool(getattr(m, "stage_a_jobs", True)) and K.profiler(hbm=True) is None and len(groups) + (c1 is not None) > 1
+                    and all(self._conv_path(conv, dev).rows for conv in every))
+            if jobs:
+                items = [(convs, x_src, rows[3], rows[1], rows[2]) for x_src, rows, convs in groups]
+                if c1 is not None:
+                    items.append(([(3, conv3)], xa, Na, rows_d, rows_dc))
+                res = self._stage_a_many(l, items) if items else []
+                for g_ in res[:len(groups)]:
+                    P.gmap.update(g_)
+                if c1 is not None:
+                    P.g_d = res[-1]
+            else:
+                for gi, (x_src, rows, convs) in enumerate(groups):
+                    if forked is not None and gi > 0:
+                        P.gmap.update(forked.run((gi - 1) % 3, lambda: self._stage_a(l, convs, x_src, rows[3], rows=rows[1], rows_cnt=rows[2])))
+                    else:
+                        P.gmap.update(self._stage_a(l, convs, x_src, rows[3], rows=rows[1], rows_cnt=rows[2]))
+                if forked is not None:
+                    for i_ in range(3):
+                        forked.join(only=i_)
+                if c1 is not None:
+                    P.g_d = self._stage_a(l, [(3, conv3)], xa, Na, rows=rows_d, rows_cnt=rows_dc)
+            if c1 is not None:
                 P.x_clean = torch.empty((c1.n0, ldx), device=dev)
                 K.gather_rows(xa, c1.rows_v, c1.n0, P.x_clean, ldx)
                 P.g_v = self._stage_a(l, [(3, conv3)], P.x_clean, c1.n0)
diff --git a/diffdock_pocket_amd/launch.py b/diffdock_pocket_amd/launch.py
--- a/diffdock_pocket_amd/launch.py
+++ b/diffdock_pocket_amd/launch.py
@@ -403,6 +403,28 @@
         L.check(lib.ddp_stage_a_h2(*args, ptr(st.Wh), n_in, ncols, out.data_ptr(), ncols, ptr(_RANGE_FLAG), stream()), "ddp_stage_a_h2")
     else:
         L.check(lib.ddp_stage_a(*args, ptr(st.W3 if x3 else None), n_in, ncols, out.data_ptr(), ncols, stream()), "ddp_stage_a")
+
+
+def stage_a_jobs(calls):
+    calls = [c for c in calls if c["n_rows"] > 0]
+    kinds = {(c["st"].path.rows, c["st"].W.shape[1], c["st"].path.gh_fmt) for c in calls}
+    if len(calls) < 2 or len(calls) > L.DDP_MAX_STAGE_A_JOBS or len(kinds) != 1 or not calls[0]["st"].path.rows:
+        for c in calls:
+            stage_a(**c)
+        return
+    arr = (L.StageAJob * len(calls))()
+    for j, c in zip(arr, calls):
+        x, st, out = c["x"], c["st"], c["out"]
+        nb, n_in, ncols = st.W.shape
+        if nb > L.DDP_MAX_GEMM_BATCH:
+            raise L.DdpError("more (conv, slot) pairs per source array than DDP_MAX_GEMM_BATCH")
+        j.x, j.ldx, j.nrows = x.data_ptr(), x.stride(0), c["n_rows"]
+        j.rows, j.nrows_dev = ptr(c.get("rows")), ptr(c.get("rows_cnt"))
+        j.out_rows = c["out_rows"] if c.get("out_rows") is not None else c["n_rows"]
+        j.offs[:nb] = st.offs[:nb]
+        j.nbatch, j.w, j.w_h2, j.k, j.ncols = nb, st.W.data_ptr(), ptr(st.Wh), n_in, ncols
+        j.out, j.ldo, j.dest, j.gh_fmt = out.data_ptr(), st.ld, st.gh.data_ptr(), 1 if st.path.gh_fmt == 1 else 0
+    L.check(L.load().ddp_stage_a_jobs(arr, len(calls), ptr(_RANGE_FLAG), stream()), "ddp_stage_a_jobs")
 
 
 def _hold(j, *objs):
diff --git a/diffdock_pocket_amd/score_model.py b/diffdock_pocket_amd/score_model.py
--- a/diffdock_pocket_amd/score_model.py
+++ b/diffdock_pocket_amd/score_model.py
@@ -443,6 +443,7 @@
         self.concurrent_heads = True
         self.stage_a_bf16x3 = False
         self.stage_a_h2 = True
+        self.stage_a_jobs = True
         self._overflow_flag = None
         self.exact_sizes = False
         self.debug_conv_outputs = None
diff --git a/include/ddp_hip.h b/include/ddp_hip.h
--- a/include/ddp_hip.h
+++ b/include/ddp_hip.h
@@ -233,6 +233,26 @@
                     int nbatch, const float* w, const void* w_h2, int k, int ncols, float* out, int ldo, int32_t* range_flag,
                     const int32_t* dest, void* stream);
 
+#define DDP_MAX_STAGE_A_JOBS 8
+typedef struct {
+  const float* x;
+  int32_t ldx, nrows;
+  const int32_t* rows;
+  const int32_t* nrows_dev;
+  int32_t out_rows;
+  int32_t offs[DDP_MAX_GEMM_BATCH];
+  int32_t nbatch;
+  const float* w;
+  const void* w_h2;
+  int32_t k, ncols;
+  float* out;
+  int32_t ldo;
+  const int32_t* dest;
+  int32_t gh_fmt;
+} ddp_stage_a_job_t;
+int ddp_stage_a_jobs(const ddp_stage_a_job_t* jobs, int njobs, int32_t* range_flag, void* stream);
+int ddp_stage_a_jobs_plan(const ddp_stage_a_job_t* jobs, int njobs, int32_t* plan, int32_t* n_workgroups);
+
 #define DDP_GH_SX 2
 
 int ddp_set_occupancy_shaping(int rows_min_lds_bytes, int stage_a_lds_pad_bytes);
```

After: 173.5 (median of 6 runs). No clear change (+0.7%).
